# retir/Style-Big-GAN

Hardware: AMD Instinct MI355X
Metric: images/sec (G+D step) StyleGAN2-ADA 256x256 bf16 (higher is better)
Workload: dtype bf16; 1 GPU; configs/sg2ada.yaml @ 256x256: sg2_classic G (skip) + D (orig), softplus + R1(0.01)/4, idle Greg slot /16 (G lr x 16/17), global batch 64 = 1 rank(s) x 2 round(s) x batch_gpu 32 (the rounds of a phase evaluated in one pass, minibatch-std groups and loss those of the separate rounds), bf16 from 8x8 up (num_fp16_res 6; the reference recipe defaults to 4), conv_clamp 256, ADA off; global_batch=64, per_rank_batch=64, parallelism=dp1

## Files before the change

### include/sbg_hip.h

```cpp
#ifndef SBG_HIP_H
#define SBG_HIP_H

#include <stdint.h>

#ifdef __cplusplus
extern "C" {
#endif

typedef void* sbg_stream_t;

enum sbg_status {
    SBG_OK = 0,
    SBG_ERR_INVALID = 1,
    SBG_ERR_UNSUPPORTED = 2,
    SBG_ERR_LAUNCH = 3
};

enum sbg_dtype { SBG_F32 = 0, SBG_F16 = 1, SBG_BF16 = 2 };

enum sbg_act {
    SBG_ACT_LINEAR = 1, SBG_ACT_RELU = 2, SBG_ACT_LRELU = 3, SBG_ACT_TANH = 4, SBG_ACT_SIGMOID = 5,
    SBG_ACT_ELU = 6, SBG_ACT_SELU = 7, SBG_ACT_SOFTPLUS = 8, SBG_ACT_SWISH = 9
};

int         sbg_version(void);
const char* sbg_last_error(void);

int sbg_bias_act(const void* x, const void* b, const void* xref, const void* yref, const void* dy,
                 void* y, int dtype, int grad, int act, float alpha, float gain, float clamp,
                 int64_t sizeX, int sizeB, int64_t stepB, sbg_stream_t stream);

typedef struct sbg_upfirdn2d_params {
    const void*  x;
    const float* f;
    void*        y;
    int dtype;
    int upx, upy, downx, downy, padx0, pady0;
    int flip;
    float gain;
    int     inSize[4];      int64_t inStride[4];
    int     filterSize[2];  int     filterStride[2];
    int     outSize[4];     int64_t outStride[4];
    const float* oscale; const float* noise; int64_t noise_stride_n; const float* bias;
    int act; float alpha, act_gain, clamp;
    int     filter_exact16;
    const void* dact_y; float* dact_partial; int dact_act; float dact_alpha, dact_gain, dact_clamp;
    const float* post_scale;
} sbg_upfirdn2d_params;
int sbg_upfirdn2d_tail_supported(const sbg_upfirdn2d_params* p);
int64_t sbg_upfirdn2d_dact_rows(const sbg_upfirdn2d_params* p);
int sbg_upfirdn2d(const sbg_upfirdn2d_params* p, sbg_stream_t stream);

int sbg_upfirdn2d_separable_supported(int up, int down, int taps);
int sbg_upfirdn2d_separable(const float* x, const float* f, float* y, int M, int IH, int IW, int OH, int OW, int taps,
                            int up, int down, int padx0, int pady0, int flip, float gain, sbg_stream_t stream);

#define SBG_MAX_TAPS 16
typedef struct sbg_conv_params {
    const void* x; const void* w; void* y;
    const float* oscale;
    int xdtype, ydtype;
    int N, IH, IW, Cin, Cout, OH, OW;
    int64_t xs_n, xs_h, xs_w;
    int64_t ys_n, ys_h, ys_w;
    int64_t ws_slab, ws_co;
    int stride;
    int ntaps;
    int tap_dy[SBG_MAX_TAPS], tap_dx[SBG_MAX_TAPS], tap_slab[SBG_MAX_TAPS];
    int accumulate;
    const float* bias; const float* noise; int64_t noise_stride_n;
    int act; float alpha, gain, clamp;
    void* workspace; int ksplit;
    int nphase; int ph_ntaps[4], ph_oh[4], ph_ow[4]; int64_t ph_yoff[4];
} sbg_conv_params;
int64_t sbg_conv2d_igemm_workspace(const sbg_conv_params* p);
int     sbg_conv2d_igemm(const sbg_conv_params* p, sbg_stream_t stream);
typedef struct sbg_conv_launch_info {
    int dims[7]; double flops, bytes;
    int64_t grid_x; int grid_y, block, lds;
} sbg_conv_launch_info;
int     sbg_conv2d_igemm_plan(const sbg_conv_params* p, sbg_conv_launch_info* out, int max);


typedef struct sbg_wgrad_params {
    const void* a; const void* b; float* out; void* workspace;
    int dtype;
    int N, PH, PW, Ca, BH, BW, Cb;
    int64_t as_n, as_h, as_w;
    int64_t bs_n, bs_h, bs_w;
    int stride;
    int ntaps;
    int tap_dy[SBG_MAX_TAPS], tap_dx[SBG_MAX_TAPS];
    int accumulate;
} sbg_wgrad_params;
int64_t sbg_conv2d_wgrad_workspace(const sbg_wgrad_params* p);
int     sbg_conv2d_wgrad(const sbg_wgrad_params* p, sbg_stream_t stream);


int sbg_scale_nc(const void* x, const float* a, const float* z, void* y, int dtype, int layout,
                 int N, int C, int64_t HW, int64_t z_stride_n, sbg_stream_t stream);
int sbg_scale_shift_nc(const void* x, const float* a, const float* b, void* y, int dtype, int layout,
                       int N, int C, int64_t HW, sbg_stream_t stream);

int sbg_dot_hw_splits(int layout, int N, int C, int64_t HW);
int sbg_dot_hw(const void* u, const void* v, float* partial, int dtype, int layout,
               int N, int C, int64_t HW, sbg_stream_t stream);
int sbg_moments_hw(const void* x, float* r, int dtype, int N, int C, int64_t HW, sbg_stream_t stream);

typedef struct sbg_gg_problem {
    const float *a0, *b0, *a1, *b1;
    float* c; const float* bias; float* rowsum;
    int64_t a0_rs, a0_cs, b0_rs, b0_cs, a1_rs, a1_cs, b1_rs, b1_cs, c_rs, c_cs;
    int M, N, K0, K1, nterms;
    float alpha0, alpha1, bias_scale, rowsum_scale;
} sbg_gg_problem;
int sbg_grouped_gemm(const sbg_gg_problem* problems, int count, sbg_stream_t stream);

int sbg_dot_hw_scale_supported(int C);
int sbg_dot_hw_scale(const void* u, const void* v, const float* scale, void* y, float* partial, int dtype,
                     int N, int C, int64_t HW, sbg_stream_t stream);


int sbg_modconv_bwd_supported(int C);
int sbg_modconv_bwd(const void* dy, const void* y, const float* dcoef, const float* noise, const float* bias,
                    void* d2, float* partial, float* dnoise, int dtype, int N, int C, int64_t HW, int64_t noise_stride_n,
                    int act, float alpha, float gain, float clamp, sbg_stream_t stream);
int sbg_modconv_bwd_prescaled(const void* dy, const void* y, const float* prescale, const float* dcoef, const float* noise, const float* bias,
                              void* d2, float* partial, float* partial3, float* dnoise, int dtype, int N, int C, int64_t HW,
                              int64_t noise_stride_n, int act, float alpha, float gain, float clamp, sbg_stream_t stream);

int64_t sbg_sn_workspace(int rows, int cols);
int sbg_sn_power_iteration(const float* W, const float* u, float* v, float* u_new, float* sigma, void* workspace,
                           int rows, int cols, float eps, sbg_stream_t stream);

int64_t sbg_mbstd_workspace(int N, int C, int HW, int G, int F);
int sbg_mbstd_fwd(const float* x, float* y, void* workspace, int N, int C, int HW, int G, int F, sbg_stream_t stream);
int sbg_mbstd_bwd(const float* x, const float* dy, float* dx, int N, int C, int HW, int G, int F, sbg_stream_t stream);

int sbg_split_bf16_cat(const float* x, void* y, int64_t outer, int64_t C, int64_t inner, int nseg, const int* order, sbg_stream_t stream);
int sbg_split_bf16_cat_nd(const float* x, const int64_t* shape, const int64_t* xstrides, int cat_dim, void* y, int nseg, const int* order, sbg_stream_t stream);

int sbg_attention_supported(int Q, int M, int D, int DV);
int sbg_attention_fwd(const float* theta, const float* phi, const float* g, float* out, int N, int Q, int M, int D, int DV,
                      sbg_stream_t stream);
int sbg_attention_bwd_supported(int Q, int M, int D, int DV);
int64_t sbg_attention_bwd_workspace(int N, int Q);
int sbg_attention_bwd(const float* theta, const float* phi, const float* g, const float* dout, float* dtheta, float* dphi, float* dg,
                      void* workspace, int N, int Q, int M, int D, int DV, sbg_stream_t stream);

int sbg_pack_weight(const float* w, void* out, int out_dtype, int A, int B, int KH, int KW,
                    int64_t sA, int64_t sB, int64_t sKH, int64_t sKW, int Bp, float gain, float* w2, sbg_stream_t stream);
int sbg_unpack_wgrad(const float* dwp, int64_t dwp_tap_stride, int64_t dwp_row_stride, float* dw, const float* w, const float* dw2,
                     int A, int B, int KH, int KW, int64_t sA, int64_t sB, int64_t sKH, int64_t sKW, float gain, sbg_stream_t stream);

int sbg_demod_coefs(const float* styles, const float* w2, float* dcoefs, int N, int O, int I, float eps, sbg_stream_t stream);
int sbg_demod_coefs_bwd(const float* g, const float* dcoefs, const float* styles, const float* w2, float* dstyles, float* dw2,
                        int N, int O, int I, sbg_stream_t stream);

// ... 163 lines not shown
```

### style-big-gan_amd/_lib.py

```python
import ctypes
import os
import threading

import torch

_HERE = os.path.dirname(os.path.abspath(__file__))
LIB_PATH = os.environ.get("SBG_HIP_LIBRARY") or os.path.join(_HERE, "libsbg_hip.so")

SBG_F32, SBG_F16, SBG_BF16 = 0, 1, 2
SBG_MAX_TAPS = 16

_DTYPES = {torch.float32: SBG_F32, torch.float16: SBG_F16, torch.bfloat16: SBG_BF16}


def dtype_code(dtype):
    try:
        return _DTYPES[dtype]
    except KeyError:
        raise RuntimeError(f"style_big_gan_amd: unsupported dtype {dtype} (float32 / float16 / bfloat16 only)")


class UpfirdnParams(ctypes.Structure):
    _fields_ = [
        ("x", ctypes.c_void_p), ("f", ctypes.c_void_p), ("y", ctypes.c_void_p),
        ("dtype", ctypes.c_int),
        ("upx", ctypes.c_int), ("upy", ctypes.c_int), ("downx", ctypes.c_int), ("downy", ctypes.c_int),
        ("padx0", ctypes.c_int), ("pady0", ctypes.c_int),
        ("flip", ctypes.c_int), ("gain", ctypes.c_float),
        ("inSize", ctypes.c_int * 4), ("inStride", ctypes.c_int64 * 4),
        ("filterSize", ctypes.c_int * 2), ("filterStride", ctypes.c_int * 2),
        ("outSize", ctypes.c_int * 4), ("outStride", ctypes.c_int64 * 4),
        ("oscale", ctypes.c_void_p), ("noise", ctypes.c_void_p), ("noise_stride_n", ctypes.c_int64), ("bias", ctypes.c_void_p),
        ("act", ctypes.c_int), ("alpha", ctypes.c_float), ("act_gain", ctypes.c_float), ("clamp", ctypes.c_float),
        ("filter_exact16", ctypes.c_int),
        ("dact_y", ctypes.c_void_p), ("dact_partial", ctypes.c_void_p), ("dact_act", ctypes.c_int),
        ("dact_alpha", ctypes.c_float), ("dact_gain", ctypes.c_float), ("dact_clamp", ctypes.c_float),
        ("post_scale", ctypes.c_void_p),
    ]


class ConvParams(ctypes.Structure):
    _fields_ = [
        ("x", ctypes.c_void_p), ("w", ctypes.c_void_p), ("y", ctypes.c_void_p), ("oscale", ctypes.c_void_p),
        ("xdtype", ctypes.c_int), ("ydtype", ctypes.c_int),
        ("N", ctypes.c_int), ("IH", ctypes.c_int), ("IW", ctypes.c_int), ("Cin", ctypes.c_int), ("Cout", ctypes.c_int),
        ("OH", ctypes.c_int), ("OW", ctypes.c_int),
        ("xs_n", ctypes.c_int64), ("xs_h", ctypes.c_int64), ("xs_w", ctypes.c_int64),
        ("ys_n", ctypes.c_int64), ("ys_h", ctypes.c_int64), ("ys_w", ctypes.c_int64),
        ("ws_slab", ctypes.c_int64), ("ws_co", ctypes.c_int64),
        ("stride", ctypes.c_int), ("ntaps", ctypes.c_int),
        ("tap_dy", ctypes.c_int * SBG_MAX_TAPS), ("tap_dx", ctypes.c_int * SBG_MAX_TAPS), ("tap_slab", ctypes.c_int * SBG_MAX_TAPS),
        ("accumulate", ctypes.c_int),
        ("bias", ctypes.c_void_p), ("noise", ctypes.c_void_p), ("noise_stride_n", ctypes.c_int64),
        ("act", ctypes.c_int), ("alpha", ctypes.c_float), ("gain", ctypes.c_float), ("clamp", ctypes.c_float),
        ("workspace", ctypes.c_void_p), ("ksplit", ctypes.c_int),
        ("nphase", ctypes.c_int), ("ph_ntaps", ctypes.c_int * 4), ("ph_oh", ctypes.c_int * 4), ("ph_ow", ctypes.c_int * 4), ("ph_yoff", ctypes.c_int64 * 4),
    ]


class ConvLaunchInfo(ctypes.Structure):
    _fields_ = [("dims", ctypes.c_int * 7), ("flops", ctypes.c_double), ("bytes", ctypes.c_double),
                ("grid_x", ctypes.c_int64), ("grid_y", ctypes.c_int), ("block", ctypes.c_int), ("lds", ctypes.c_int)]


class WgradParams(ctypes.Structure):
    _fields_ = [
        ("a", ctypes.c_void_p), ("b", ctypes.c_void_p), ("out", ctypes.c_void_p), ("workspace", ctypes.c_void_p),
        ("dtype", ctypes.c_int),
        ("N", ctypes.c_int), ("PH", ctypes.c_int), ("PW", ctypes.c_int), ("Ca", ctypes.c_int),
        ("BH", ctypes.c_int), ("BW", ctypes.c_int), ("Cb", ctypes.c_int),
        ("as_n", ctypes.c_int64), ("as_h", ctypes.c_int64), ("as_w", ctypes.c_int64),
        ("bs_n", ctypes.c_int64), ("bs_h", ctypes.c_int64), ("bs_w", ctypes.c_int64),
        ("stride", ctypes.c_int), ("ntaps", ctypes.c_int),
        ("tap_dy", ctypes.c_int * SBG_MAX_TAPS), ("tap_dx", ctypes.c_int * SBG_MAX_TAPS),
        ("accumulate", ctypes.c_int),
    ]


class GridSampleParams(ctypes.Structure):
    _fields_ = [
        ("x", ctypes.c_void_p), ("grid", ctypes.c_void_p), ("theta", ctypes.c_void_p), ("dy", ctypes.c_void_p),
        ("y", ctypes.c_void_p), ("dx", ctypes.c_void_p), ("dgrid", ctypes.c_void_p),
        ("N", ctypes.c_int), ("C", ctypes.c_int), ("IH", ctypes.c_int), ("IW", ctypes.c_int), ("OH", ctypes.c_int), ("OW", ctypes.c_int),
        ("xs_n", ctypes.c_int64), ("xs_c", ctypes.c_int64), ("xs_h", ctypes.c_int64), ("xs_w", ctypes.c_int64),
        ("ys_n", ctypes.c_int64), ("ys_c", ctypes.c_int64), ("ys_h", ctypes.c_int64), ("ys_w", ctypes.c_int64),
        ("theta_host", ctypes.c_void_p),
    ]


class GgProblem(ctypes.Structure):
    _fields_ = [("a0", ctypes.c_void_p), ("b0", ctypes.c_void_p), ("a1", ctypes.c_void_p), ("b1", ctypes.c_void_p),
                ("c", ctypes.c_void_p), ("bias", ctypes.c_void_p), ("rowsum", ctypes.c_void_p),
                ("a0_rs", ctypes.c_int64), ("a0_cs", ctypes.c_int64), ("b0_rs", ctypes.c_int64), ("b0_cs", ctypes.c_int64),
                ("a1_rs", ctypes.c_int64), ("a1_cs", ctypes.c_int64), ("b1_rs", ctypes.c_int64), ("b1_cs", ctypes.c_int64),
                ("c_rs", ctypes.c_int64), ("c_cs", ctypes.c_int64),
                ("M", ctypes.c_int), ("N", ctypes.c_int), ("K0", ctypes.c_int), ("K1", ctypes.c_int), ("nterms", ctypes.c_int),
                ("alpha0", ctypes.c_float), ("alpha1", ctypes.c_float), ("bias_scale", ctypes.c_float), ("rowsum_scale", ctypes.c_float)]


class ProfRecord(ctypes.Structure):
    _fields_ = [("kind", ctypes.c_int), ("dims", ctypes.c_int * 7), ("flops", ctypes.c_double), ("bytes", ctypes.c_double),
                ("ms", ctypes.c_float), ("pad", ctypes.c_int)]


KERNEL_KINDS = {1: "bias_act", 2: "upfirdn2d", 3: "conv_igemm", 4: "conv_wgrad", 5: "wgrad_reduce", 6: "scale_nc", 7: "dot_hw", 9: "sn_power", 10: "attention",
                11: "grid_sample", 12: "filter1d", 13: "color", 14: "weight_prep", 15: "torgb", 16: "fromrgb", 17: "grouped_gemm", 18: "ppl",
                19: "projector", 20: "image_export", 21: "resample", 22: "pr", 23: "grad_finish", 24: "resident", 25: "diffaug", 26: "nn_u8", 27: "swd", 28: "spectrum",
                29: "msssim", 30: "directions", 31: "kmeans_u8", 32: "walk"}
WALK_VARIANTS = {0: "blend", 1: "sqdiff", 2: "merge"}
KMEANS_VARIANTS = {0: "accumulate", 1: "finish"}
DIRECTIONS_VARIANTS = {0: "mean", 1: "gram", 2: "merge", 3: "edit"}
MSSSIM_VARIANTS = {0: "level", 1: "down", 2: "merge"}
SWD_VARIANTS = {0: "pyr_down", 1: "pyr_lap", 2: "gather", 3: "moments", 4: "project", 5: "l1", 6: "merge"}
SPECTRUM_VARIANTS = {0: "rows", 1: "cols"}
NN_VARIANTS = {0: "norms", 1: "single", 2: "split", 3: "merge"}
RESIDENT_PATHS = {1: "dword", 2: "byte"}
PPL_VARIANTS = {0: "slerp", 1: "lerp", 2: "prep", 3: "dist"}
PROJ_VARIANTS = {0: "reg", 1: "reg_bwd", 2: "normalize", 3: "sqdist", 4: "sqdist_bwd"}
IMG_VARIANTS = {0: "quantize_tile", 1: "truncate_mix"}
QUANT_RULES = {"grid": 0, "clamp": 1}
RESAMPLE_VARIANTS = {0: "h", 1: "v"}
PR_VARIANTS = {0: "single", 1: "split", 2: "merge", 3: "norms"}
GRAD_FINISH_VARIANTS = {0: "sweep", 1: "merge"}
DIFFAUG_VARIANTS = {0: "sum", 1: "apply", 2: "adj_sum", 3: "adj_apply", 4: "single", 5: "adj_single"}
DIFFAUG_WORDS = 12
ATT_VARIANTS = {0: "single", 1: "stream", 2: "stream_stats", 3: "stream_dq", 4: "stream_dkv"}

_lib = None
_lock = threading.Lock()

_c = ctypes
SYMBOLS = [
    ("sbg_version", _c.c_int, []),
    ("sbg_last_error", _c.c_char_p, []),
    ("sbg_bias_act", _c.c_int, [_c.c_void_p] * 6 + [_c.c_int, _c.c_int, _c.c_int, _c.c_float, _c.c_float, _c.c_float,
                                                   _c.c_int64, _c.c_int, _c.c_int64, _c.c_void_p]),
    ("sbg_upfirdn2d_tail_supported", _c.c_int, [_c.POINTER(UpfirdnParams)]),
    ("sbg_upfirdn2d", _c.c_int, [_c.POINTER(UpfirdnParams), _c.c_void_p]),
    ("sbg_upfirdn2d_dact_rows", _c.c_int64, [_c.POINTER(UpfirdnParams)]),
    ("sbg_upfirdn2d_separable_supported", _c.c_int, [_c.c_int] * 3),
    ("sbg_upfirdn2d_separable", _c.c_int, [_c.c_void_p] * 3 + [_c.c_int] * 11 + [_c.c_float, _c.c_void_p]),
    ("sbg_conv2d_igemm_workspace", _c.c_int64, [_c.POINTER(ConvParams)]),
    ("sbg_conv2d_igemm", _c.c_int, [_c.POINTER(ConvParams), _c.c_void_p]),
    ("sbg_conv2d_igemm_plan", _c.c_int, [_c.POINTER(ConvParams), _c.POINTER(ConvLaunchInfo), _c.c_int]),
    ("sbg_conv2d_wgrad_workspace", _c.c_int64, [_c.POINTER(WgradParams)]),
    ("sbg_conv2d_wgrad", _c.c_int, [_c.POINTER(WgradParams), _c.c_void_p]),
    ("sbg_scale_nc", _c.c_int, [_c.c_void_p] * 4 + [_c.c_int, _c.c_int, _c.c_int, _c.c_int, _c.c_int64, _c.c_int64, _c.c_void_p]),
    ("sbg_scale_shift_nc", _c.c_int, [_c.c_void_p] * 4 + [_c.c_int, _c.c_int, _c.c_int, _c.c_int, _c.c_int64, _c.c_void_p]),
    ("sbg_sn_workspace", _c.c_int64, [_c.c_int, _c.c_int]),
    ("sbg_sn_power_iteration", _c.c_int, [_c.c_void_p] * 6 + [_c.c_int, _c.c_int, _c.c_float, _c.c_void_p]),
    ("sbg_mbstd_workspace", _c.c_int64, [_c.c_int] * 5),
    ("sbg_mbstd_fwd", _c.c_int, [_c.c_void_p] * 3 + [_c.c_int] * 5 + [_c.c_void_p]),
    ("sbg_mbstd_bwd", _c.c_int, [_c.c_void_p] * 3 + [_c.c_int] * 5 + [_c.c_void_p]),
    ("sbg_split_bf16_cat", _c.c_int, [_c.c_void_p, _c.c_void_p, _c.c_int64, _c.c_int64, _c.c_int64, _c.c_int, _c.POINTER(_c.c_int), _c.c_void_p]),
    ("sbg_split_bf16_cat_nd", _c.c_int, [_c.c_void_p, _c.POINTER(_c.c_int64), _c.POINTER(_c.c_int64), _c.c_int, _c.c_void_p, _c.c_int, _c.POINTER(_c.c_int), _c.c_void_p]),
    ("sbg_attention_supported", _c.c_int, [_c.c_int] * 4),
    ("sbg_attention_fwd", _c.c_int, [_c.c_void_p] * 4 + [_c.c_int] * 5 + [_c.c_void_p]),
    ("sbg_attention_bwd_supported", _c.c_int, [_c.c_int] * 4),
    ("sbg_attention_bwd_workspace", _c.c_int64, [_c.c_int, _c.c_int]),
    ("sbg_attention_bwd", _c.c_int, [_c.c_void_p] * 8 + [_c.c_int] * 5 + [_c.c_void_p]),
    ("sbg_dot_hw_splits", _c.c_int, [_c.c_int, _c.c_int, _c.c_int, _c.c_int64]),
    ("sbg_dot_hw", _c.c_int, [_c.c_void_p] * 3 + [_c.c_int, _c.c_int, _c.c_int, _c.c_int, _c.c_int64, _c.c_void_p]),
    ("sbg_moments_hw", _c.c_int, [_c.c_void_p, _c.c_void_p, _c.c_int, _c.c_int, _c.c_int, _c.c_int64, _c.c_void_p]),
    ("sbg_grouped_gemm", _c.c_int, [_c.c_void_p, _c.c_int, _c.c_void_p]),
    ("sbg_dot_hw_scale_supported", _c.c_int, [_c.c_int]),
    ("sbg_dot_hw_scale", _c.c_int, [_c.c_void_p] * 5 + [_c.c_int, _c.c_int, _c.c_int, _c.c_int64, _c.c_void_p]),
    ("sbg_modconv_bwd_supported", _c.c_int, [_c.c_int]),
    ("sbg_modconv_bwd", _c.c_int, [_c.c_void_p] * 8 + [_c.c_int, _c.c_int, _c.c_int, _c.c_int64, _c.c_int64, _c.c_int, _c.c_float, _c.c_float, _c.c_float, _c.c_void_p]),
    ("sbg_modconv_bwd_prescaled", _c.c_int, [_c.c_void_p] * 10 + [_c.c_int, _c.c_int, _c.c_int, _c.c_int64, _c.c_int64, _c.c_int, _c.c_float, _c.c_float, _c.c_float, _c.c_void_p]),
    ("sbg_pack_weight", _c.c_int, [_c.c_void_p, _c.c_void_p, _c.c_int, _c.c_int, _c.c_int, _c.c_int, _c.c_int] + [_c.c_int64] * 4
     + [_c.c_int, _c.c_float, _c.c_void_p, _c.c_void_p]),
    ("sbg_unpack_wgrad", _c.c_int, [_c.c_void_p, _c.c_int64, _c.c_int64, _c.c_void_p, _c.c_void_p, _c.c_void_p] + [_c.c_int] * 4
     + [_c.c_int64] * 4 + [_c.c_float, _c.c_void_p]),
    ("sbg_demod_coefs", _c.c_int, [_c.c_void_p] * 3 + [_c.c_int] * 3 + [_c.c_float, _c.c_void_p]),
    ("sbg_demod_coefs_bwd", _c.c_int, [_c.c_void_p] * 6 + [_c.c_int] * 3 + [_c.c_void_p]),
    ("sbg_torgb_supported", _c.c_int, [_c.c_int, _c.c_int]),
    ("sbg_torgb_bwd_blocks", _c.c_int, [_c.c_int, _c.c_int, _c.c_int64]),
    ("sbg_torgb_fwd", _c.c_int, [_c.c_void_p] * 4 + [_c.c_int] * 4 + [_c.c_int64, _c.c_float, _c.c_void_p]),
    ("sbg_torgb_bwd", _c.c_int, [_c.c_void_p] * 6 + [_c.c_int] * 4 + [_c.c_int64, _c.c_float, _c.c_void_p]),
    ("sbg_fromrgb_supported", _c.c_int, [_c.c_int] * 3),
    ("sbg_fromrgb_bwd_blocks", _c.c_int, [_c.c_int, _c.c_int64]),
    ("sbg_fromrgb_fwd", _c.c_int, [_c.c_void_p] * 4 + [_c.c_int] * 4 + [_c.c_int64, _c.c_int, _c.c_float, _c.c_float, _c.c_float, _c.c_void_p]),
    ("sbg_fromrgb_bwd", _c.c_int, [_c.c_void_p] * 6 + [_c.c_int] * 4 + [_c.c_int64, _c.c_int, _c.c_float, _c.c_float, _c.c_float, _c.c_void_p]),
    ("sbg_grid_sample2d", _c.c_int, [_c.POINTER(GridSampleParams), _c.c_void_p]),
    ("sbg_grid_sample2d_bwd", _c.c_int, [_c.POINTER(GridSampleParams), _c.c_void_p]),
    ("sbg_grid_sample2d_bwd_overwrites", _c.c_int, [_c.POINTER(GridSampleParams)]),
    ("sbg_color_transform", _c.c_int, [_c.c_void_p] * 3 + [_c.c_int, _c.c_int64, _c.c_void_p]),
    ("sbg_filter1d_batch", _c.c_int, [_c.c_void_p] * 3 + [_c.c_int] * 8 + [_c.c_void_p]),
    ("sbg_ppl_slerp_endpoints", _c.c_int, [_c.c_void_p] * 3 + [_c.c_float, _c.c_void_p, _c.c_int, _c.c_int, _c.c_void_p]),
    ("sbg_ppl_lerp_endpoints", _c.c_int, [_c.c_void_p] * 3 + [_c.c_float, _c.c_void_p, _c.c_int, _c.c_int64, _c.c_void_p]),
    ("sbg_ppl_prep_images", _c.c_int, [_c.c_void_p] * 2 + [_c.c_int] * 4 + [_c.c_int64] * 4 + [_c.c_int, _c.c_int, _c.c_void_p]),
    ("sbg_ppl_dist_workspace", _c.c_int64, [_c.c_int, _c.c_int64]),
    ("sbg_ppl_dist", _c.c_int, [_c.c_void_p] * 3 + [_c.c_int, _c.c_int64, _c.c_float, _c.c_void_p]),
    ("sbg_proj_noise_reg_workspace", _c.c_int64, [_c.c_void_p, _c.c_int]),
    ("sbg_proj_noise_reg", _c.c_int, [_c.c_void_p] * 2 + [_c.c_int] + [_c.c_void_p] * 4),
    ("sbg_proj_noise_reg_bwd", _c.c_int, [_c.c_void_p] * 3 + [_c.c_int] + [_c.c_void_p] * 4),
    ("sbg_proj_noise_normalize_workspace", _c.c_int64, [_c.c_void_p, _c.c_int]),
    ("sbg_proj_noise_normalize", _c.c_int, [_c.c_void_p] * 2 + [_c.c_int] + [_c.c_void_p] * 2),
    ("sbg_proj_sqdist_workspace", _c.c_int64, [_c.c_int64]),
    ("sbg_proj_sqdist", _c.c_int, [_c.c_void_p] * 4 + [_c.c_int64, _c.c_void_p]),
    ("sbg_proj_sqdist_bwd", _c.c_int, [_c.c_void_p] * 4 + [_c.c_int64, _c.c_void_p]),
    ("sbg_img_quantize_tile", _c.c_int, [_c.c_void_p] * 2 + [_c.c_int] * 4 + [_c.c_int64] * 4 + [_c.c_int] * 4 + [_c.c_float] * 2 + [_c.c_void_p]),
    ("sbg_ws_truncate_mix", _c.c_int, [_c.c_void_p] * 2 + [_c.c_float] + [_c.c_void_p] * 4 + [_c.c_int] * 5 + [_c.c_void_p]),
    ("sbg_u8_resample_h", _c.c_int, [_c.c_void_p, _c.c_int64, _c.c_int64] * 2 + [_c.c_int] * 5 + [_c.c_void_p] * 2 + [_c.c_int] * 3 + [_c.c_void_p]),
    ("sbg_u8_resample_v", _c.c_int, [_c.c_void_p, _c.c_int64, _c.c_int64] * 2 + [_c.c_int] * 4 + [_c.c_void_p] * 2 + [_c.c_int, _c.c_void_p]),
    ("sbg_knn_workspace", _c.c_int64, [_c.c_int] * 4),
    ("sbg_knn_kth_radius", _c.c_int, [_c.c_void_p] * 2 + [_c.c_int, _c.c_int, _c.c_int64, _c.c_int] + [_c.c_void_p] * 3),
    ("sbg_knn_in_manifold", _c.c_int, [_c.c_void_p] * 3 + [_c.c_int, _c.c_int, _c.c_int64] + [_c.c_void_p] * 3),
    ("sbg_knn_probe_workspace", _c.c_int64, [_c.c_int] * 2),
    ("sbg_knn_probe", _c.c_int, [_c.c_void_p] * 3 + [_c.c_int, _c.c_int, _c.c_int64] + [_c.c_void_p] * 4),
    ("sbg_knn_topk_workspace", _c.c_int64, [_c.c_int] * 3),
    ("sbg_knn_topk", _c.c_int, [_c.c_void_p] * 2 + [_c.c_int, _c.c_int, _c.c_int64, _c.c_int] + [_c.c_void_p] * 5),
    ("sbg_knn_realism_workspace", _c.c_int64, [_c.c_int] * 2),
    ("sbg_knn_realism", _c.c_int, [_c.c_void_p] * 3 + [_c.c_int, _c.c_int, _c.c_int64] + [_c.c_void_p] * 5),
    ("sbg_grad_finish_records", _c.c_int64, [_c.c_int64]),
    ("sbg_grad_finish_sweep", _c.c_int, [_c.c_void_p, _c.c_int64, _c.c_float, _c.c_void_p, _c.c_void_p]),
    ("sbg_grad_finish_merge", _c.c_int, [_c.c_void_p, _c.c_int64, _c.c_void_p, _c.c_void_p]),
    ("sbg_u8_gather_images", _c.c_int, [_c.c_void_p, _c.c_int64, _c.c_int, _c.c_int, _c.c_int, _c.c_void_p, _c.c_void_p, _c.c_int, _c.c_void_p, _c.c_int,
                                        _c.c_void_p, _c.c_void_p]),
    ("sbg_u8_nn_workspace", _c.c_int64, [_c.c_int] * 3),
    ("sbg_u8_nn_topk", _c.c_int, [_c.c_void_p] * 2 + [_c.c_int, _c.c_int, _c.c_int64, _c.c_int] + [_c.c_void_p] * 5),
    ("sbg_diffaug_workspace", _c.c_int64, [_c.c_int] * 4),
    ("sbg_diffaug_fwd", _c.c_int, [_c.c_void_p] * 4 + [_c.c_int] * 5 + [_c.c_void_p]),
    ("sbg_diffaug_adj", _c.c_int, [_c.c_void_p] * 4 + [_c.c_int] * 4 + [_c.c_void_p]),
    ("sbg_swd_pyr_down", _c.c_int, [_c.c_void_p] * 2 + [_c.c_int] * 3 + [_c.c_void_p]),
# ... 98 lines not shown
```

### style-big-gan_amd/csrc/conv_common.h

```cpp
#pragma once
#include "sbg_common.h"
#include <cstdlib>

#define SBG_OOB_OFFSET 0x80000000u

namespace sbgconv {

typedef __attribute__((address_space(3))) void* lds_void_ptr;

struct bf16_mfma { static constexpr int dtype = SBG_BF16; };
struct f16_mfma  { static constexpr int dtype = SBG_F16;  };

template <class MF> struct Mfma;
template <> struct Mfma<bf16_mfma> {
    static __device__ __forceinline__ float4_t run(short8_t a, short8_t b, float4_t c) {
        return __builtin_amdgcn_mfma_f32_16x16x32_bf16(__builtin_bit_cast(bf16x8_t, a), __builtin_bit_cast(bf16x8_t, b), c, 0, 0, 0);
    }
    static __device__ __forceinline__ unsigned short cvt(float v) { return f32_to_bf16_bits(v); }
};
template <> struct Mfma<f16_mfma> {
    static __device__ __forceinline__ float4_t run(short8_t a, short8_t b, float4_t c) {
        return __builtin_amdgcn_mfma_f32_16x16x32_f16(__builtin_bit_cast(f16x8_t, a), __builtin_bit_cast(f16x8_t, b), c, 0, 0, 0);
    }
    static __device__ __forceinline__ unsigned short cvt(float v) { return f32_to_f16_bits(v); }
};

struct ConvArgs {
    const unsigned short* x; const unsigned short* w; void* y; const float* oscale;
    const float* bias; const float* noise; int64_t noise_sn; int act; float alpha, gain, clamp;
    int ydtype;
    int N, IH, IW, Cin, Cout, OH, OW;
    int64_t xs_n, xs_h, xs_w, ys_n, ys_h, ys_w, ws_slab, ws_co;
    int stride, ntaps;
    int tap_dy[SBG_MAX_TAPS], tap_dx[SBG_MAX_TAPS], tap_slab[SBG_MAX_TAPS];
    int accumulate;
    int P;
    int ptiles, ctiles;
    int nphase, ph_rot_div;
    int ph_tap0[4], ph_ntaps[4], ph_OH[4], ph_OW[4], ph_P[4];
    int64_t ph_yoff[4];
    int ksplit;
    int64_t y_split_stride;
    int lds_params;
};

#define SBG_CONV_IS_PLAIN(a) (((a).act <= SBG_ACT_LINEAR) && (a).gain == 1.f && (a).clamp < 0.f && !(a).bias && !(a).noise && !(a).oscale)
static __host__ __device__ __forceinline__ bool conv_is_plain(const ConvArgs& a) { return SBG_CONV_IS_PLAIN(a); }
static inline bool conv_is_plain(const sbg_conv_params& q)
{
    return (q.act == 0 || q.act == SBG_ACT_LINEAR) && (q.gain == 1.f || q.gain == 0.f) && q.clamp < 0.f && !q.bias && !q.noise && !q.oscale;
}

template <auto Kern, class... Args>
static int launch_as(int kind, const char* who, int64_t nblk, unsigned grid_y, unsigned block, int lds, hipStream_t stream, double flops,
                     double bytes, std::initializer_list<int> dims, const Args&... args)
{
    if (nblk > INT32_MAX || nblk < 1) return sbg_fail(SBG_ERR_INVALID, "%s: grid too large", who);
    if (lds > 64 * 1024 && !SBG_RAISE_LDS_ONCE(Kern, lds))
        return sbg_fail(SBG_ERR_LAUNCH, "%s: cannot raise the dynamic LDS limit to %d bytes", who, lds);
    SbgProfScope prof(stream, kind, flops, bytes, dims);
    SBG_LAUNCH(Kern, dim3((unsigned)nblk, grid_y), dim3(block), lds, stream, args...);
    SBG_HIP_LAUNCH_CHECK();
    return SBG_OK;
}

enum ConvFamily { CONV_THIN, CONV_UP2, CONV_GATHER, CONV_HALO, CONV_K64, CONV_GENERIC };
struct ConvLaunch {
    ConvFamily family;
    int bc, bp;
    int64_t grid_x; unsigned grid_y, block; int lds;
    ConvArgs a;
    unsigned x_bytes, w_bytes;
    int pitch;
    int tiles_y, tiles_x, dymin, dxmin;
    double flops, bytes; int dims[7];
};
struct ConvPlan {
    int nlaunch; ConvLaunch launch[5];
    ConvArgs call;
    int ksplit; bool reduce_epi;
    int64_t workspace_bytes;
};

static inline void conv_prof(ConvLaunch& l, double macs, double outpix, int ntaps, int stride, int rows, int code)
{
    const ConvArgs& a = l.a;
    const double ys = a.ydtype == SBG_F32 ? 4.0 : 2.0;
    l.flops = 2.0 * macs * a.Cout * (double)a.Cin;
    l.bytes = 2.0 * a.N * a.IH * a.IW * (double)a.Cin + 2.0 * ntaps * a.Cout * (double)a.Cin + ys * outpix * (double)a.Cout * (a.accumulate ? 2 : 1);
    const int dims[7] = {(int)outpix, a.Cout, a.Cin, ntaps, stride, rows, code};
    for (int i = 0; i < 7; i++) l.dims[i] = dims[i];
}
static inline void conv_prof_phases(ConvLaunch& l, int code)
{
    const ConvArgs& a = l.a;
    double macs = (double)a.P * a.ntaps, outpix = a.P;
    if (a.nphase > 1) {
        macs = outpix = 0.0;
        for (int i = 0; i < a.nphase; i++) { macs += (double)a.ph_P[i] * a.ph_ntaps[i]; outpix += a.ph_P[i]; }
    }
    conv_prof(l, macs, outpix, a.ntaps, a.stride, a.OH, code);
}

template <auto Kern, class... Extra>
static int conv_launch(const ConvLaunch& l, hipStream_t stream, const Extra&... extra)
{
    const int* d = l.dims;
    return launch_as<Kern>(SBG_K_CONV_IGEMM, "conv2d_igemm", l.grid_x, l.grid_y, l.block, l.lds, stream, l.flops, l.bytes,
                           {d[0], d[1], d[2], d[3], d[4], d[5], d[6]}, l.a, extra...);
}

}

bool sbg_conv_thin_fit(sbgconv::ConvLaunch& l);
int  sbg_conv_thin_launch(const sbgconv::ConvLaunch& l, bool bf16, hipStream_t stream);
enum Up2Fit { UP2_OTHER_FORM, UP2_ORDERED, UP2_FITS };
Up2Fit sbg_conv_up2_fit(sbgconv::ConvLaunch& l, const sbg_conv_params& q, sbg_conv_params& border);
int    sbg_conv_up2_launch(const sbgconv::ConvLaunch& l, bool bf16, hipStream_t stream);
void sbg_conv_k64_fit(sbgconv::ConvLaunch& l);
int  sbg_conv_k64_launch(const sbgconv::ConvLaunch& l, bool bf16, hipStream_t stream);
int  sbg_conv_ksplit_reduce(const sbgconv::ConvArgs& call, const void* workspace, int ksplit, bool reduce_epi, hipStream_t stream);
```

### style-big-gan_amd/csrc/conv_device.h

```cpp
#pragma once
#include "conv_common.h"
#include "lds_asm.h"

namespace sbgconv {

static __device__ __forceinline__ int chmap(int R) { return (R & ~31) + 8 * ((R & 15) >> 2) + 4 * ((R >> 4) & 1) + (R & 3); }

template <int N> static __device__ __forceinline__ void wait_vmcnt_const() { asm volatile("s_waitcnt vmcnt(%0)" :: "n"(N) : "memory"); }

static __device__ __forceinline__ int xcd_tile_order(int bid, int nwg)
{
    const int q = nwg >> 3, r = nwg & 7, xcd = bid & 7, k = bid >> 3;
    return (xcd < r ? xcd * (q + 1) : r * (q + 1) + (xcd - r) * q) + k;
}

static __device__ __forceinline__ int dma_lrow(int lane)  { return lane >> 3; }
static __device__ __forceinline__ int dma_src_k(int lane, int lrow) { return ((lane & 7) ^ lrow) * 8; }

static __device__ __forceinline__ int frag_off(int fr, int fg) { return fr * 128 + ((fg ^ (fr & 7)) << 4); }

template <class MF, int TC, int TP>
static __device__ __forceinline__ void mma_step(float4_t (&acc)[TC][TP], const short8_t (&fa)[2][TC], const short8_t (&fb)[2][TP])
{
#pragma unroll
    for (int ks = 0; ks < 2; ks++)
#pragma unroll
        for (int i = 0; i < TC; i++)
#pragma unroll
            for (int j = 0; j < TP; j++) acc[i][j] = Mfma<MF>::run(fa[ks][i], fb[ks][j], acc[i][j]);
}

static __device__ __forceinline__ float tail(const ConvArgs& p, float u, int64_t si, float add)
{
    if (p.oscale) u *= p.oscale[si];
    u += add;
    if (p.act == SBG_ACT_LRELU) u = (u > 0.f) ? u : u * p.alpha;
    else if (p.act == SBG_ACT_RELU) u = (u > 0.f) ? u : 0.f;
    u *= p.gain;
    if (p.clamp >= 0.f) u = (u > -p.clamp && u < p.clamp) ? u : (u >= 0.f ? p.clamp : -p.clamp);
    return u;
}

typedef __attribute__((address_space(3))) const float lds_cfloat;
typedef __attribute__((address_space(3))) const float4_t lds_cfloat4;
struct LdsParams { lds_cfloat* base; int c; int tw; };
template <int TC, int TP, int YDT, bool PLAIN, bool NUNI, bool LP = false, class PixFn>
static __device__ __forceinline__ void conv_epilogue_fast(const ConvArgs& p, float4_t (&acc)[TC][TP], int cbase, int fg, PixFn pix, int64_t ybase,
                                                          const LdsParams* lp = nullptr, int y0 = 0, int x0 = 0)
{
    constexpr int TH2 = TC / 2;
    const float alpha = (p.act == SBG_ACT_LRELU) ? p.alpha : (p.act == SBG_ACT_RELU ? 0.f : 1.f);
    const float lsel = alpha <= 1.f ? __builtin_inff() : -__builtin_inff();
    const float cl = p.clamp >= 0.f ? p.clamp : __builtin_inff();
    const float gain = p.gain;
    const float* const dummy = reinterpret_cast<const float*>(p.x);
    const bool has_nz = !PLAIN && p.noise != nullptr, has_b = !PLAIN && p.bias != nullptr, has_s = !PLAIN && p.oscale != nullptr;
    int64_t yoff[TP]; float nz[TP]; bool ok[TP]; int nn[TP];
#pragma unroll
    for (int j = 0; j < TP; j++) {
        int n, oy, ox;
        ok[j] = pix(j, n, oy, ox);
        nn[j] = n;
        yoff[j] = ybase + (int64_t)blockIdx.y * p.y_split_stride + (int64_t)n * p.ys_n + (int64_t)oy * p.ys_h + (int64_t)ox * p.ys_w + cbase + 8 * fg;
        nz[j] = 0.f;
        if (!PLAIN) {
            if constexpr (LP) nz[j] = lp->base[(oy - y0) * lp->tw + (ox - x0)];
            else              nz[j] = *(has_nz ? p.noise + ((int64_t)n * p.noise_sn + (int64_t)oy * p.OW + ox) : dummy);
        }
    }
    float4_t b_lo[TH2], b_hi[TH2], s_lo[TH2], s_hi[TH2];
#pragma unroll
    for (int h = 0; h < TH2; h++) {
        b_lo[h] = b_hi[h] = float4_t{0.f, 0.f, 0.f, 0.f};
        s_lo[h] = s_hi[h] = float4_t{1.f, 1.f, 1.f, 1.f};
        if (!PLAIN) {
            if constexpr (LP) {
                lds_cfloat* b = lp->base + 256 + lp->c + 32 * h + 8 * fg;
                b_lo[h] = *(lds_cfloat4*)b; b_hi[h] = *(lds_cfloat4*)(b + 4);
                if (NUNI) { s_lo[h] = *(lds_cfloat4*)(b + 256); s_hi[h] = *(lds_cfloat4*)(b + 260); }
            } else {
            const float* b = has_b ? p.bias + cbase + 32 * h + 8 * fg : dummy;
            b_lo[h] = *reinterpret_cast<const float4_t*>(b); b_hi[h] = *reinterpret_cast<const float4_t*>(has_b ? b + 4 : dummy);
            if (NUNI) {
                const float* sc = has_s ? p.oscale + (int64_t)nn[0] * p.Cout + cbase + 32 * h + 8 * fg : dummy;
                s_lo[h] = *reinterpret_cast<const float4_t*>(sc); s_hi[h] = *reinterpret_cast<const float4_t*>(has_s ? sc + 4 : dummy);
            }
            }
        }
    }
    if (!PLAIN) {
#pragma unroll
        for (int j = 0; j < TP; j++) nz[j] = has_nz ? nz[j] : 0.f;
#pragma unroll
        for (int h = 0; h < TH2; h++) {
            if (!has_b) { b_lo[h] = float4_t{0.f, 0.f, 0.f, 0.f}; b_hi[h] = b_lo[h]; }
            if (!NUNI || !has_s) { s_lo[h] = float4_t{1.f, 1.f, 1.f, 1.f}; s_hi[h] = s_lo[h]; }
        }
    }
#pragma unroll
    for (int h = 0; h < TH2; h++) {
#pragma unroll
        for (int j = 0; j < TP; j++) {
            if (!ok[j]) continue;
            float4_t lo = acc[2 * h][j], hi = acc[2 * h + 1][j];
            if (!PLAIN) {
                float4_t sl = s_lo[h], sh = s_hi[h];
                if (!NUNI && has_s) {
                    const float* sc = p.oscale + (int64_t)nn[j] * p.Cout + cbase + 32 * h + 8 * fg;
                    sl = *reinterpret_cast<const float4_t*>(sc); sh = *reinterpret_cast<const float4_t*>(sc + 4);
                }
                lo = lo * sl + (nz[j] + b_lo[h]);
                hi = hi * sh + (nz[j] + b_hi[h]);
                const float4_t tl = lo * alpha, th = hi * alpha;
#pragma unroll
                for (int e = 0; e < 4; e++) { lo[e] = __builtin_amdgcn_fmed3f(lo[e], tl[e], lsel); hi[e] = __builtin_amdgcn_fmed3f(hi[e], th[e], lsel); }
                lo = lo * gain; hi = hi * gain;
#pragma unroll
                for (int e = 0; e < 4; e++) { lo[e] = __builtin_amdgcn_fmed3f(lo[e], -cl, cl); hi[e] = __builtin_amdgcn_fmed3f(hi[e], -cl, cl); }
            }
            if (YDT == SBG_F32) {
                float* dst = (float*)p.y + yoff[j] + 32 * h;
                if (p.accumulate) { lo += *reinterpret_cast<float4_t*>(dst); hi += *reinterpret_cast<float4_t*>(dst + 4); }
                *reinterpret_cast<float4_t*>(dst) = lo;
                *reinterpret_cast<float4_t*>(dst + 4) = hi;
            } else {
                short8_t o;
#pragma unroll
                for (int e = 0; e < 4; e++) { o[e] = (short)f32_to_bf16_bits(lo[e]); o[4 + e] = (short)f32_to_bf16_bits(hi[e]); }
                *reinterpret_cast<short8_t*>((unsigned short*)p.y + yoff[j] + 32 * h) = o;
            }
        }
    }
}


template <int TC, int TP, bool NUNI = false, class PixFn>
static __device__ __forceinline__ void conv_epilogue8(const ConvArgs& p, float4_t (&acc)[TC][TP], int cbase, int fg, PixFn pix, int64_t ybase = 0,
                                                      const LdsParams* lp = nullptr, int y0 = 0, int x0 = 0)
{
    constexpr int TH2 = TC / 2;
    const bool plain = conv_is_plain(p);
    const bool fast = (cbase + 16 * TC <= p.Cout) && ((p.Cout & 7) == 0) && ((((uintptr_t)p.y) & 15) == 0) && (((p.ys_n | p.ys_h | p.ys_w) & 7) == 0)
                      && ((((uintptr_t)p.oscale) & 15) == 0) && ((((uintptr_t)p.bias) & 15) == 0) && p.ydtype != SBG_F16;
    if (fast) {
        if (p.ydtype == SBG_BF16) {
            if (plain) conv_epilogue_fast<TC, TP, SBG_BF16, true, NUNI>(p, acc, cbase, fg, pix, ybase);
            else if (lp) conv_epilogue_fast<TC, TP, SBG_BF16, false, NUNI, true>(p, acc, cbase, fg, pix, ybase, lp, y0, x0);
            else       conv_epilogue_fast<TC, TP, SBG_BF16, false, NUNI>(p, acc, cbase, fg, pix, ybase);
        } else {
            if (plain) conv_epilogue_fast<TC, TP, SBG_F32, true, NUNI>(p, acc, cbase, fg, pix, ybase);
            else if (lp) conv_epilogue_fast<TC, TP, SBG_F32, false, NUNI, true>(p, acc, cbase, fg, pix, ybase, lp, y0, x0);
            else       conv_epilogue_fast<TC, TP, SBG_F32, false, NUNI>(p, acc, cbase, fg, pix, ybase);
        }
        return;
    }
    float bias8[TH2][8];
#pragma unroll
    for (int h = 0; h < TH2; h++) {
        const int co = cbase + 32 * h + 8 * fg;
#pragma unroll
        for (int e = 0; e < 8; e++) bias8[h][e] = (p.bias && co + e < p.Cout) ? p.bias[co + e] : 0.f;
    }
#pragma unroll
    for (int j = 0; j < TP; j++) {
        int n, oy, ox;
        if (!pix(j, n, oy, ox)) continue;
        const int64_t yoff = ybase + (int64_t)blockIdx.y * p.y_split_stride + (int64_t)n * p.ys_n + (int64_t)oy * p.ys_h + (int64_t)ox * p.ys_w;
        const float nz = (!plain && p.noise) ? p.noise[(int64_t)n * p.noise_sn + (int64_t)oy * p.OW + ox] : 0.f;
#pragma unroll
        for (int h = 0; h < TH2; h++) {
            const int co = cbase + 32 * h + 8 * fg;
            if (co >= p.Cout) continue;
            float v[8];
#pragma unroll
            for (int e = 0; e < 4; e++) { v[e] = acc[2 * h][j][e]; v[4 + e] = acc[2 * h + 1][j][e]; }
#pragma unroll 1
            for (int e = 0; e < 8; e++) {
                if (co + e >= p.Cout) break;
                float u = v[e];
                if (!plain) {
                    if (p.oscale) u *= p.oscale[(int64_t)n * p.Cout + co + e];
                    u += nz + bias8[h][e];
                    if (p.act == SBG_ACT_LRELU) u = (u > 0.f) ? u : u * p.alpha;
                    else if (p.act == SBG_ACT_RELU) u = (u > 0.f) ? u : 0.f;
                    u *= p.gain;
                    if (p.clamp >= 0.f) u = (u > -p.clamp && u < p.clamp) ? u : (u >= 0.f ? p.clamp : -p.clamp);
                }
                if (p.ydtype == SBG_F32) {
                    float* dst = (float*)p.y + yoff + co + e;
                    *dst = p.accumulate ? *dst + u : u;
                } else {
                    ((unsigned short*)p.y)[yoff + co + e] = (p.ydtype == SBG_BF16) ? f32_to_bf16_bits(u) : f32_to_f16_bits(u);
                }
            }
        }
    }
}

}
```

### style-big-gan_amd/csrc/conv_igemm.hip

```cpp
#include "conv_device.h"

using namespace sbgconv;

namespace {

static __device__ __forceinline__ int stage_row16(int lane) { return (lane & 7) | ((lane >> 5) << 3); }
static __device__ __forceinline__ int stage_kgrp(int lane)  { return (lane >> 3) & 3; }

template <int TC, int TP>
static __device__ __forceinline__ void conv_epilogue(const ConvArgs& p, float4_t (&acc)[TC][TP], int c0, int p0, int wc, int wp, int fr, int fg)
{
    float4_t bias4[TC];
    bool full4[TC];
#pragma unroll
    for (int i = 0; i < TC; i++) {
        const int co = c0 + wc + 16 * i + 4 * fg;
        full4[i] = (co + 4 <= p.Cout);
        bias4[i] = float4_t{0.f, 0.f, 0.f, 0.f};
        if (p.bias) {
#pragma unroll
            for (int e = 0; e < 4; e++) if (co + e < p.Cout) bias4[i][e] = p.bias[co + e];
        }
    }
    const bool plain = conv_is_plain(p);
// ... 125 lines not shown
        if (s + 1 < nsteps) issue_loads(s + 1);
        const unsigned char* sa = smem + buf * STAGE;
        const unsigned char* sb = sa + A_BYTES;
        short8_t fa[TC], fb[TP];
#pragma unroll
        for (int i = 0; i < TC; i++) fa[i] = *reinterpret_cast<const short8_t*>(sa + (fg * BC + wc + 16 * i + fr) * 16);
#pragma unroll
        for (int j = 0; j < TP; j++) fb[j] = *reinterpret_cast<const short8_t*>(sb + (fg * BP + wp + 16 * j + fr) * 16);
#pragma unroll
        for (int i = 0; i < TC; i++)
#pragma unroll
            for (int j = 0; j < TP; j++) acc[i][j] = Mfma<MF>::run(fa[i], fb[j], acc[i][j]);
        if (s + 1 < nsteps) write_stage(buf ^ 1);
        __syncthreads();
    }

    conv_epilogue<TC, TP>(p, acc, c0, p0, wc, wp, fr, fg);
}

template <class MF>
static int launch_generic(const ConvLaunch& l, hipStream_t stream)
{
    if (l.bc == 64) return conv_launch<conv_igemm_kernel<MF, 64, 256, 1, 4>>(l, stream);
    return conv_launch<conv_igemm_kernel<MF, 128, 128, 2, 2>>(l, stream);
}

static void fit_generic(ConvLaunch& l)
{
    ConvArgs& a = l.a;
    l.family = CONV_GENERIC; l.bc = a.Cout <= 64 ? 64 : 128; l.bp = a.Cout <= 64 ? 256 : 128;
    a.ptiles = (a.P + l.bp - 1) / l.bp;
    a.ctiles = (a.Cout + l.bc - 1) / l.bc;
    l.grid_x = (int64_t)a.ptiles * a.ctiles; l.grid_y = 1; l.block = 256; l.lds = 2 * (4 * l.bc * 16 + 4 * l.bp * 16);
    conv_prof_phases(l, l.bc * 1000 + l.bp);
}

constexpr int kPhaseMinTiles = 16;

int conv_validate(const sbg_conv_params* q)
{
    SBG_CHECK(q && q->x && q->w && q->y, "conv2d_igemm: null pointer");
    SBG_CHECK(q->xdtype == SBG_BF16 || q->xdtype == SBG_F16, "conv2d_igemm: x/w must be bf16 or f16 (fp32 inputs are split by the host)");
    SBG_CHECK(q->ydtype == SBG_F32 || q->ydtype == SBG_BF16 || q->ydtype == SBG_F16, "conv2d_igemm: bad output dtype");
    SBG_CHECK(q->N >= 0 && q->IH >= 1 && q->IW >= 1 && q->OH >= 1 && q->OW >= 1 && q->Cin >= 8 && q->Cout >= 1, "conv2d_igemm: bad sizes");
    SBG_CHECK((q->Cin % 8) == 0, "conv2d_igemm: Cin must be a multiple of 8 (pad on the host)");
    SBG_CHECK(q->ntaps >= 1 && q->ntaps <= SBG_MAX_TAPS, "conv2d_igemm: 1..%d taps", SBG_MAX_TAPS);
    SBG_CHECK(q->stride >= 1, "conv2d_igemm: stride must be >= 1");
    SBG_CHECK(!q->accumulate || q->ydtype == SBG_F32, "conv2d_igemm: accumulate needs an fp32 output");
    SBG_CHECK(q->ksplit >= 0, "conv2d_igemm: ksplit must be 0 (the library chooses), 1 (never) or a cap");
    SBG_CHECK(q->act == 0 || q->act == SBG_ACT_LINEAR || q->act == SBG_ACT_RELU || q->act == SBG_ACT_LRELU, "conv2d_igemm: fused activation must be linear, relu or lrelu");
    SBG_CHECK(sbg_aligned16(q->x) && sbg_aligned16(q->w), "conv2d_igemm: x and w must be 16-byte aligned");
    SBG_CHECK((q->xs_n % 8) == 0 && (q->xs_h % 8) == 0 && (q->xs_w % 8) == 0 && (q->ws_slab % 8) == 0 && (q->ws_co % 8) == 0,
              "conv2d_igemm: pixel / row strides must be multiples of 8 elements");
    const int64_t P = (int64_t)q->N * q->OH * q->OW;
    SBG_CHECK(P <= INT32_MAX, "conv2d_igemm: too many output pixels");
    if (P == 0) return SBG_OK;
    for (int t = 0; t < q->ntaps; t++) SBG_CHECK(q->tap_slab[t] >= 0, "conv2d_igemm: negative weight slab");
    if (q->nphase > 1) {
        SBG_CHECK(q->nphase <= 4, "conv2d_igemm: at most 4 phases");
        SBG_CHECK(conv_is_plain(*q) && (q->ksplit <= 1), "conv2d_igemm: phases exclude the fused epilogue and the K split");
        int t0 = 0;
        for (int i = 0; i < q->nphase; i++) {
            SBG_CHECK(q->ph_ntaps[i] >= 1 && q->ph_oh[i] >= 1 && q->ph_ow[i] >= 1, "conv2d_igemm: bad phase %d", i);
            t0 += q->ph_ntaps[i];
        }
        SBG_CHECK(t0 <= q->ntaps, "conv2d_igemm: phases use %d taps, %d given", t0, q->ntaps);
    }
    return SBG_OK;
}

void conv_fill(const sbg_conv_params& q, ConvArgs& a)
{
    a.x = (const unsigned short*)q.x; a.w = (const unsigned short*)q.w; a.y = q.y; a.oscale = q.oscale;
    a.bias = q.bias; a.noise = q.noise; a.noise_sn = q.noise_stride_n;
    a.act = q.act; a.alpha = q.alpha; a.gain = (q.act == 0 && q.gain == 0.f) ? 1.f : q.gain; a.clamp = (q.act == 0 && q.clamp == 0.f && q.gain == 0.f) ? -1.f : q.clamp;
    a.ydtype = q.ydtype;
    a.N = q.N; a.IH = q.IH; a.IW = q.IW; a.Cin = q.Cin; a.Cout = q.Cout; a.OH = q.OH; a.OW = q.OW;
    a.xs_n = q.xs_n; a.xs_h = q.xs_h; a.xs_w = q.xs_w; a.ys_n = q.ys_n; a.ys_h = q.ys_h; a.ys_w = q.ys_w;
    a.ws_slab = q.ws_slab; a.ws_co = q.ws_co;
    a.stride = q.stride; a.ntaps = q.ntaps;
    for (int t = 0; t < SBG_MAX_TAPS; t++) { a.tap_dy[t] = q.tap_dy[t]; a.tap_dx[t] = q.tap_dx[t]; a.tap_slab[t] = q.tap_slab[t]; }
    a.accumulate = q.accumulate;
    a.P = q.N * q.OH * q.OW; a.ptiles = a.ctiles = 0; a.lds_params = 0; a.ksplit = 1; a.y_split_stride = 0;
    a.nphase = q.nphase > 1 ? q.nphase : 1; a.ph_rot_div = 1;
    for (int i = 0, t0 = 0; i < 4; i++) {
        const bool on = q.nphase > 1 && i < q.nphase;
        a.ph_tap0[i] = on ? t0 : 0; a.ph_ntaps[i] = on ? q.ph_ntaps[i] : 0; a.ph_OH[i] = on ? q.ph_oh[i] : 0; a.ph_OW[i] = on ? q.ph_ow[i] : 0;
        a.ph_P[i] = on ? q.N * q.ph_oh[i] * q.ph_ow[i] : 0; a.ph_yoff[i] = on ? q.ph_yoff[i] : 0;
        if (on) t0 += q.ph_ntaps[i];
    }
}

int conv_ksplit(const sbg_conv_params& q, const ConvArgs& a, bool have_ws, bool& reduce_epi)
{
    const bool dense_y = a.ys_w == a.Cout && a.ys_h == (int64_t)a.OW * a.Cout && a.ys_n == (int64_t)a.OH * a.OW * a.Cout;
    const bool simple = a.ydtype == SBG_F32 && conv_is_plain(a);
    const bool epi_ok = !a.accumulate && (a.Cout & 7) == 0 && sbg_aligned16(a.y);
    reduce_epi = !simple;
    if (!have_ws || q.ksplit == 1 || a.Cout <= 64 || !dense_y || !(simple || epi_ok)) return 1;
    const int64_t tiles = (int64_t)((a.P + 127) / 128) * ((a.Cout + 127) / 128);
    const int ksteps = a.ntaps * ((a.Cin + 63) >> 6);
    if (tiles >= 128 || ksteps < 16) return 1;
    int k = (int)((256 + tiles - 1) / tiles);
    if (k > ksteps / 4) k = ksteps / 4;
    if (q.ksplit > 1 && k > q.ksplit) k = q.ksplit;
    return k < 2 ? 1 : k;
}

int push(ConvPlan& pl, const ConvLaunch& l)
{
    if (pl.nlaunch >= 5) return sbg_fail(SBG_ERR_INVALID, "conv2d_igemm: more than five launches");
    pl.launch[pl.nlaunch++] = l;
    return SBG_OK;
}

int conv_plan_add(const sbg_conv_params& q, bool have_ws, ConvPlan& pl)
{
    if ((int64_t)q.N * q.OH * q.OW == 0) return SBG_OK;
    ConvLaunch l = {};
    ConvArgs& a = l.a;
    conv_fill(q, a);
    if (pl.nlaunch == 0) pl.call = a;
    int maxslab = 0;
    for (int t = 0; t < q.ntaps; t++) if (q.tap_slab[t] > maxslab) maxslab = q.tap_slab[t];
    const int64_t x_bytes = 2 * ((int64_t)(q.N - 1) * q.xs_n + (int64_t)(q.IH - 1) * q.xs_h + (int64_t)(q.IW - 1) * q.xs_w + q.Cin);
    const int64_t w_bytes = 2 * ((int64_t)maxslab * q.ws_slab + (int64_t)(q.Cout - 1) * q.ws_co + q.Cin);
    const bool fwd_strides = q.xs_n >= 0 && q.xs_h >= 0 && q.xs_w >= 0 && q.ws_slab >= 0 && q.ws_co >= 0;
    const bool dma = fwd_strides && x_bytes < (int64_t)SBG_OOB_OFFSET && w_bytes < (int64_t)SBG_OOB_OFFSET;
    l.x_bytes = (unsigned)x_bytes; l.w_bytes = (unsigned)w_bytes;
    if (q.nphase > 1) {
        if (fwd_strides && sbg_conv_thin_fit(l)) return push(pl, l);
        if (dma && q.nphase == 4) {
            sbg_conv_params border;
            if (sbg_conv_up2_fit(l, q, border) == UP2_FITS) {
                const int rc = push(pl, l);
                return rc != SBG_OK || border.nphase == 0 ? rc : conv_plan_add(border, false, pl);
            }
        }
        int64_t ptot = 0;
        for (int i = 0; i < q.nphase; i++) ptot += a.ph_P[i];
        const int64_t tiles = ((ptot / q.nphase + 255) / 256) * q.nphase * ((q.Cout + 127) / 128);
        if (dma && q.Cout > 64 && tiles >= kPhaseMinTiles) { sbg_conv_k64_fit(l); return push(pl, l); }
        for (int i = 0; i < q.nphase; i++) {
            sbg_conv_params one = q;
            one.nphase = 0; one.ksplit = 1; one.OH = q.ph_oh[i]; one.OW = q.ph_ow[i]; one.ntaps = q.ph_ntaps[i];
            one.y = (char*)q.y + q.ph_yoff[i] * (q.ydtype == SBG_F32 ? 4 : 2);
            for (int t = 0; t < one.ntaps; t++) { one.tap_dy[t] = q.tap_dy[a.ph_tap0[i] + t]; one.tap_dx[t] = q.tap_dx[a.ph_tap0[i] + t]; one.tap_slab[t] = q.tap_slab[a.ph_tap0[i] + t]; }
            const int rc = conv_plan_add(one, false, pl);
            if (rc != SBG_OK) return rc;
        }
        return SBG_OK;
    }
    if (q.ksplit <= 1 && fwd_strides && sbg_conv_thin_fit(l)) return push(pl, l);
    if (!dma) { fit_generic(l); return push(pl, l); }
    const int k = conv_ksplit(q, a, have_ws, pl.reduce_epi);
    if (k > 1) {
        pl.ksplit = k; pl.workspace_bytes = (int64_t)k * a.P * a.Cout * (int64_t)sizeof(float);
        a.y = q.workspace; a.accumulate = 0; a.ksplit = k; a.y_split_stride = (int64_t)a.P * a.Cout;
        a.ydtype = SBG_F32; a.act = SBG_ACT_LINEAR; a.gain = 1.f; a.clamp = -1.f; a.bias = nullptr; a.noise = nullptr; a.oscale = nullptr;
    }
    sbg_conv_k64_fit(l);
    return push(pl, l);
}

int conv_plan(const sbg_conv_params* q, bool have_ws, ConvPlan& pl)
{
    const int rc = conv_validate(q);
    if (rc != SBG_OK) return rc;
    pl.nlaunch = 0; pl.ksplit = 1; pl.reduce_epi = false; pl.workspace_bytes = 0;
    return conv_plan_add(*q, have_ws, pl);
}

}

extern "C" int64_t sbg_conv2d_igemm_workspace(const sbg_conv_params* q)
{
    ConvPlan pl;
    return conv_plan(q, true, pl) == SBG_OK ? pl.workspace_bytes : -1;
}

extern "C" int sbg_conv2d_igemm_plan(const sbg_conv_params* q, sbg_conv_launch_info* out, int max)
{
    ConvPlan pl;
    if (conv_plan(q, q && q->workspace, pl) != SBG_OK) return -1;
    for (int i = 0; i < pl.nlaunch && i < max && out; i++) {
        const ConvLaunch& l = pl.launch[i];
        for (int d = 0; d < 7; d++) out[i].dims[d] = l.dims[d];
        out[i].flops = l.flops; out[i].bytes = l.bytes;
        out[i].grid_x = l.grid_x; out[i].grid_y = (int)l.grid_y; out[i].block = (int)l.block; out[i].lds = l.lds;
    }
    return pl.nlaunch;
}

extern "C" int sbg_conv2d_igemm(const sbg_conv_params* q, sbg_stream_t stream)
{
    ConvPlan pl;
    int rc = conv_plan(q, q && q->workspace, pl);
    if (rc != SBG_OK) return rc;
    SBG_CHECK(q->ksplit <= 1 || q->workspace != nullptr, "conv2d_igemm: ksplit > 1 needs a workspace");
    hipStream_t s = (hipStream_t)stream;
    const bool bf16 = q->xdtype == SBG_BF16;
    for (int i = 0; i < pl.nlaunch && rc == SBG_OK; i++) {
        const ConvLaunch& l = pl.launch[i];
        switch (l.family) {
        case CONV_THIN:    rc = sbg_conv_thin_launch(l, bf16, s); break;
        case CONV_UP2:     rc = sbg_conv_up2_launch(l, bf16, s); break;
        case CONV_GENERIC: rc = bf16 ? launch_generic<bf16_mfma>(l, s) : launch_generic<f16_mfma>(l, s); break;
        default:           rc = sbg_conv_k64_launch(l, bf16, s); break;
        }
    }
    return rc != SBG_OK || pl.ksplit == 1 ? rc : sbg_conv_ksplit_reduce(pl.call, q->workspace, pl.ksplit, pl.reduce_epi, s);
}
```

### style-big-gan_amd/csrc/conv_k64.hip

```cpp
#include "conv_device.h"
#include <type_traits>

using namespace sbgconv;

namespace {


template <class MF, int BC, int BP, int WGC, int WGP, int NSTAGE = 3>
__global__ __launch_bounds__(512, 2) void conv_k64_kernel(ConvArgs p, unsigned x_bytes, unsigned w_bytes)
{
    constexpr int NW = 8;
    static_assert(WGC * WGP == NW, "8 waves per workgroup");
    constexpr int WC = BC / WGC, WP = BP / WGP;
    constexpr int TC = WC / 16,  TP = WP / 16;
    static_assert(WC % 32 == 0 && WP % 16 == 0 && BC % 64 == 0 && BP % 64 == 0, "tile shape");
    constexpr int IA = BC / 64;
    constexpr int IB = BP / 64;
    constexpr int LEAD = NSTAGE - 1;
    static_assert(NSTAGE == 2 || NSTAGE == 3, "gather pipeline: one or two steps of loads in flight");
    constexpr int A_BYTES = BC * 128, B_BYTES = BP * 128, STAGE = A_BYTES + B_BYTES;

    extern __shared__ __attribute__((aligned(16))) unsigned char smem[];

    const int tid = threadIdx.x, lane = tid & 63;
    const int wave = __builtin_amdgcn_readfirstlane(tid >> 6);
    const bool grpY = wave >= 4;
    const int bid = xcd_tile_order(blockIdx.x, gridDim.x);
    const int c0 = (bid % p.ctiles) * BC, p0 = (bid / p.ctiles) * BP;

    __amdgpu_buffer_rsrc_t xr = __builtin_amdgcn_make_buffer_rsrc((void*)p.x, 0, (int)x_bytes, 0x00020000);
    __amdgpu_buffer_rsrc_t wr = __builtin_amdgcn_make_buffer_rsrc((void*)p.w, 0, (int)w_bytes, 0x00020000);

    const int lrow = dma_lrow(lane);
    const int src_k = dma_src_k(lane, lrow);
    unsigned a_base[IA];
#pragma unroll
    for (int i = 0; i < IA; i++) {
        const int co = c0 + chmap((wave * IA + i) * 8 + lrow);
        a_base[i] = (co < p.Cout) ? (unsigned)(co * (int)p.ws_co + src_k) * 2u : SBG_OOB_OFFSET;
    }
    const int kchunks = (p.Cin + 63) >> 6;
    const int nsteps_all = p.ntaps * kchunks;
    int nsteps = nsteps_all;
    const int tl = lane < p.ntaps ? lane : 0;
    const int tbl_dy = p.tap_dy[tl], tbl_dx = p.tap_dx[tl];
    const int tbl_wtap = p.tap_slab[tl] * (int)p.ws_slab * 2;

    auto issue_w = [&](int t, int chunk, int stage) {
        unsigned char* st = smem + stage * STAGE;
        const int wtap = __builtin_amdgcn_readlane(tbl_wtap, t) + chunk * 128;
        const bool ragged = chunk * 64 + 64 > p.Cin;
#pragma unroll
        for (int i = 0; i < IA; i++) {
            unsigned off = a_base[i];
            if (ragged) off = (chunk * 64 + src_k < p.Cin) ? off : SBG_OOB_OFFSET;
            __builtin_amdgcn_raw_ptr_buffer_load_lds(wr, (lds_void_ptr)(st + (wave * IA + i) * 1024), 16, off, wtap, 0, 0);
        }
    };

    const int wci = wave / WGP, wpi = wave % WGP;
    const int wc = wci * WC, wp = wpi * WP;
    const int fr = lane & 15, fg = lane >> 4;
    const int foff = frag_off(fr, fg);
    float4_t acc[TC][TP];
#pragma unroll
    for (int i = 0; i < TC; i++)
#pragma unroll
        for (int j = 0; j < TP; j++) acc[i][j] = float4_t{0.f, 0.f, 0.f, 0.f};
    short8_t fa[2][TC], fb[2][TP];

    auto read_a = [&](int stage) {
        const unsigned char* sa = smem + stage * STAGE + wc * 128;
#pragma unroll
        for (int ks = 0; ks < 2; ks++)
#pragma unroll
            for (int i = 0; i < TC; i++) fa[ks][i] = *reinterpret_cast<const short8_t*>(sa + i * 16 * 128 + (foff ^ (ks * 64)));
    };
    auto mma = [&]() {
#pragma unroll
        for (int ks = 0; ks < 2; ks++)
#pragma unroll
            for (int i = 0; i < TC; i++)
#pragma unroll
                for (int j = 0; j < TP; j++) acc[i][j] = Mfma<MF>::run(fa[ks][i], fb[ks][j], acc[i][j]);
    };


    {
        int b_iy0[IB], b_ix0[IB]; unsigned b_base[IB];
#pragma unroll
        for (int i = 0; i < IB; i++) {
// ... 92 lines not shown
                    x_off[i] = ok ? b_org[i] + shift : SBG_OOB_OFFSET;
                }
            }
        };
        auto issue_piece = [&](auto k_tag, int t, int chunk, int stg) {
            constexpr int k = decltype(k_tag)::value;
            unsigned char* st = smem + stg * STAGE;
            const bool ragged = chunk * 64 + 64 > p.Cin;
            if constexpr (k < IA) {
                const int wtap = __builtin_amdgcn_readlane(tbl_wtap, t) + chunk * 128 + (16 * (k & 1) + 4 * (k >> 1)) * (int)p.ws_co * 2;
                unsigned off = a_base[0];
                if (ragged) off = (chunk * 64 + src_k < p.Cin) ? off : SBG_OOB_OFFSET;
                __builtin_amdgcn_raw_ptr_buffer_load_lds(wr, (lds_void_ptr)(st + (wave * IA + k) * 1024), 16, off, wtap, 0, 0);
            } else {
                constexpr int i = k - IA;
                unsigned off = x_off[i];
                if (ragged) off = (chunk * 64 + src_k < p.Cin) ? off : SBG_OOB_OFFSET;
                __builtin_amdgcn_raw_ptr_buffer_load_lds(xr, (lds_void_ptr)(st + A_BYTES + (wave * IB + i) * 1024), 16, off, chunk * 128, 0, 0);
            }
        };
        auto issue_advance = [&]() {
            wstage ^= 1;
            if (++ic == kchunks) { ic = 0; it++; }
        };
        auto issue_all = [&]() {
            tap_prep(it);
            sbg_static_for<C>([&](auto k_tag) { issue_piece(k_tag, it, ic, wstage); });
            issue_advance();
        };
        constexpr int NG = 2 * TC, GPP = NG / C;
        static_assert(NG % C == 0, "pieces spread evenly over the MFMA groups");
        auto mma_issue = [&]() {
            tap_prep(it);
            sbg_static_for<NG>([&](auto q_tag) {
                constexpr int q = decltype(q_tag)::value, ks = q / TC, i = q % TC;
#pragma unroll
                for (int j = 0; j < TP; j++) acc[i][j] = Mfma<MF>::run(fa[ks][i], fb[ks][j], acc[i][j]);
                if constexpr ((q + 1) % GPP == 0) {
                    __builtin_amdgcn_sched_barrier(0);
                    issue_piece(std::integral_constant<int, (q + 1) / GPP - 1>{}, it, ic, wstage);
                    __builtin_amdgcn_sched_barrier(0);
                }
            });
            issue_advance();
        };
        if (nsteps > 0) issue_all();
        int stage = 0;
        if (!grpY) {
            for (int s = 0; s < nsteps; s++) {
                wait_vmcnt_const<0>();
                __builtin_amdgcn_s_barrier();
                read_a(stage); read_b(stage);
                if (s + 1 < nsteps) issue_all();
                __builtin_amdgcn_s_waitcnt(0xC07F);
                __builtin_amdgcn_s_barrier();
                __builtin_amdgcn_sched_barrier(0);
                mma();
                __builtin_amdgcn_sched_barrier(0);
                stage ^= 1;
            }
            __builtin_amdgcn_s_barrier();
        } else {
            if (nsteps > 1) { issue_all(); wait_vmcnt_const<C>(); } else wait_vmcnt_const<0>();
            __builtin_amdgcn_s_barrier();
            auto y_step = [&](auto more_tag) {
                constexpr bool more = decltype(more_tag)::value;
                __builtin_amdgcn_s_barrier();
                read_a(stage); read_b(stage);
                wait_vmcnt_const<0>();
                __builtin_amdgcn_s_waitcnt(0xC07F);
                __builtin_amdgcn_s_barrier();
                __builtin_amdgcn_sched_barrier(0);
                if constexpr (more) mma_issue(); else mma();
                __builtin_amdgcn_sched_barrier(0);
                stage ^= 1;
            };
            int s = 0;
            for (; s + 2 < nsteps; s++) y_step(std::true_type{});
            for (; s < nsteps; s++) y_step(std::false_type{});
        }
        }
    }

    conv_epilogue8<TC, TP>(p, acc, c0 + wc, fg, [&](int j, int& n, int& oy, int& ox) {
        const int pix = p0 + wp + 16 * j + fr;
        const int pp = pix < p.P ? pix : 0;
        ox = pp % p.OW; const int t = pp / p.OW; oy = t % p.OH; n = t / p.OH;
        return pix < p.P;
    });
}

template <class MF, int TH, int TW>
__global__ __launch_bounds__(768, 3) void conv_halo_ld_kernel(ConvArgs p, unsigned x_bytes, unsigned w_bytes)
{
    constexpr int BC = 128, BP = 256, WGP = 4;
    constexpr int WC = 64, WP = 64, TC = 4, TP = 4;
    static_assert(TH * TW == BP, "halo tile = TH x TW pixels");
    constexpr int NSTAGE = 4, STAGE = BC * 128;
    constexpr int PW = TW + 2, PH = TH + 2, NPIX = PW * PH;
    constexpr int HPIECES = (NPIX + 7) / 8, HALO_BYTES = HPIECES * 1024;
    constexpr int NT = 9, SEG = TW / 16;
    constexpr int WPIECES = BC / 8 / 2;
    constexpr int HPL = (HPIECES + 1) / 2;

    extern __shared__ __attribute__((aligned(16))) unsigned char smem[];
    unsigned char* const sH = smem + NSTAGE * STAGE;
    unsigned char* const sP = sH + 2 * HALO_BYTES;
    constexpr int PARAM_BYTES = 3072;

    const int tid = threadIdx.x, lane = tid & 63;
    const int wave = __builtin_amdgcn_readfirstlane(tid >> 6);
    const int bid = xcd_tile_order(blockIdx.x, gridDim.x);
    const int tiles_x = p.OW / TW, tiles_y = p.OH / TH;
    const int ntiles = p.ptiles * p.ctiles, G = gridDim.x;
    const int my_tiles = (ntiles - bid + G - 1) / G;
    const int kchunks = (p.Cin + 63) >> 6;
    const int nslices = my_tiles * kchunks;
    struct TileC { int c0, tn, y0, x0; };
    auto decode = [&](int tile) -> TileC {
        TileC r;
        const int ct_ = tile % p.ctiles; int pt_ = tile / p.ctiles;
        const int tx = pt_ % tiles_x; pt_ /= tiles_x;
        const int ty = pt_ % tiles_y;
        r.c0 = ct_ * BC; r.tn = pt_ / tiles_y; r.y0 = ty * TH; r.x0 = tx * TW;
        return r;
    };
    const TileC gstep = decode(G);
    auto advance = [&](TileC t_) -> TileC {
        t_.c0 += gstep.c0; int carry = t_.c0 >= p.ctiles * BC; t_.c0 -= carry ? p.ctiles * BC : 0;
        t_.x0 += gstep.x0 + (carry ? TW : 0); carry = t_.x0 >= tiles_x * TW; t_.x0 -= carry ? tiles_x * TW : 0;
        t_.y0 += gstep.y0 + (carry ? TH : 0); carry = t_.y0 >= tiles_y * TH; t_.y0 -= carry ? tiles_y * TH : 0;
        t_.tn += gstep.tn + carry;
        return t_;
    };
    const int lrow = dma_lrow(lane);
    const int src_k = dma_src_k(lane, lrow);

    if (wave >= 10) {
        const int lh = wave - 10;
        __amdgpu_buffer_rsrc_t xr = __builtin_amdgcn_make_buffer_rsrc((void*)p.x, 0, (int)x_bytes, 0x00020000);
        auto issue_params = [&](int t_, int buf) {
            const TileC pc = decode(t_);
            unsigned char* dst = sP + buf * PARAM_BYTES;
            if (p.noise) {
                __amdgpu_buffer_rsrc_t nr = __builtin_amdgcn_make_buffer_rsrc((void*)p.noise, 0, 0x7fffffff, 0x00020000);
                constexpr int LPR = TW / 4;
                const int r = lane / LPR, cx = (lane - r * LPR) * 4;
                const unsigned off = (unsigned)(pc.tn * (int)p.noise_sn + (pc.y0 + r) * p.OW + pc.x0 + cx) * 4u;
                __builtin_amdgcn_raw_ptr_buffer_load_lds(nr, (lds_void_ptr)dst, 16, off, 0, 0, 0);
            }
            const int co = pc.c0 + 4 * lane;
            const unsigned okm = 0u - (unsigned)((lane < 32) & (co < p.Cout));
            if (p.bias) {
                __amdgpu_buffer_rsrc_t br_ = __builtin_amdgcn_make_buffer_rsrc((void*)p.bias, 0, 0x7fffffff, 0x00020000);
                __builtin_amdgcn_raw_ptr_buffer_load_lds(br_, (lds_void_ptr)(dst + 1024), 16, (((unsigned)co * 4u) & okm) | (SBG_OOB_OFFSET & ~okm), 0, 0, 0);
            }
            if (p.oscale) {
                __amdgpu_buffer_rsrc_t sr = __builtin_amdgcn_make_buffer_rsrc((void*)p.oscale, 0, 0x7fffffff, 0x00020000);
                __builtin_amdgcn_raw_ptr_buffer_load_lds(sr, (lds_void_ptr)(dst + 2048), 16, (((unsigned)(pc.tn * p.Cout + co) * 4u) & okm) | (SBG_OOB_OFFSET & ~okm), 0, 0, 0);
            }
        };
        int rel[HPL]; unsigned ef[(HPL + 5) / 6];
#pragma unroll
        for (int w_ = 0; w_ < (HPL + 5) / 6; w_++) ef[w_] = 0;
#pragma unroll
        for (int i = 0; i < HPL; i++) {
            const int piece = lh * HPL + i, pp = piece * 8 + lrow;
            const int py = pp / PW, px = pp - py * PW;
            rel[i] = (py * (int)p.xs_h + px * (int)p.xs_w + src_k) * 2;
            const unsigned f = (unsigned)(py == 0) | ((unsigned)(py == PH - 1) << 1) | ((unsigned)(px == 0) << 2) | ((unsigned)(px == PW - 1) << 3)
                             | ((unsigned)((piece >= HPIECES) | (pp >= NPIX)) << 4);
            ef[i / 6] |= f << (5 * (i % 6));
        }
        auto issue_halo = [&](auto i_tag, int hbase, unsigned emask, bool kok, int buf) {
            constexpr int i = decltype(i_tag)::value;
// ... 52 lines not shown
                const int co = c0_ + chmap((lw * WPIECES + i) * 8 + lrow);
                a_base[i] = (co < p.Cout) ? (unsigned)(co * (int)p.ws_co + src_k) * 2u : SBG_OOB_OFFSET;
            }
        };
        int it = 0, ichunk = 0, itile = bid, istage = 0;
        weight_rows(decode(itile).c0);
        unsigned char* st = nullptr; unsigned kokm = 0, wtap = 0;
        auto issue_prep = [&]() {
            st = smem + istage * STAGE + lw * WPIECES * 1024;
            kokm = 0u - (unsigned)(ichunk * 64 + src_k < p.Cin);
            wtap = (unsigned)(__builtin_amdgcn_readlane(tbl_wtap, it) + ichunk * 128);
        };
        const bool whole_k = (p.Cin & 63) == 0;
        auto issue_part = [&](int lo, int hi) {
            if (whole_k) {
#pragma unroll
                for (int i = 0; i < WPIECES; i++)
                    if (i >= lo && i < hi) __builtin_amdgcn_raw_ptr_buffer_load_lds(wr, (lds_void_ptr)(st + i * 1024), 16, a_base[i], wtap, 0, 0);
                return;
            }
#pragma unroll
            for (int i = 0; i < WPIECES; i++) {
                if (i < lo || i >= hi) continue;
                const unsigned okm = kokm & (0u - (unsigned)(a_base[i] != SBG_OOB_OFFSET));
                const unsigned off = ((a_base[i] + wtap) & okm) | (SBG_OOB_OFFSET & ~okm);
                __builtin_amdgcn_raw_ptr_buffer_load_lds(wr, (lds_void_ptr)(st + i * 1024), 16, off, 0, 0, 0);
            }
        };
        auto issue_done = [&]() {
            istage = (istage + 1) & (NSTAGE - 1);
            if (++it == NT) {
                it = 0;
                if (++ichunk == kchunks) { ichunk = 0; itile += G; if (itile < ntiles) weight_rows(decode(itile).c0); }
            }
        };
        auto issue_next = [&]() { issue_prep(); issue_part(0, WPIECES); issue_done(); };
        constexpr bool split = false;
        const int S = nslices * NT;
        int issued = 0;
        for (; issued < 4 && issued < S; issued++) issue_next();
        for (int s = 0; s < S; s++) {
            const int newer = issued - 1 - s;
            if (newer >= 3) wait_vmcnt_const<3 * WPIECES>();
            else if (newer == 2) wait_vmcnt_const<2 * WPIECES>();
            else if (newer == 1) wait_vmcnt_const<1 * WPIECES>();
            else wait_vmcnt_const<0>();
            __builtin_amdgcn_s_barrier();
            const bool go = s >= 1 && issued < S;
            if (go) { issue_prep(); issue_part(0, split ? WPIECES / 2 : WPIECES); }
            __builtin_amdgcn_s_barrier();
            if (go) { if (split) issue_part(WPIECES / 2, WPIECES); issue_done(); issued++; }
            else if (s >= 1 && issued < S) issued++;
        }
        __builtin_amdgcn_s_barrier();
        return;
    }

    const bool grpY = wave >= 4;
    const int wci = wave >> 2, wpi = wave & 3;
    const int wc = wci * WC;
    const int fr = lane & 15, fg = lane >> 4;
    const int foff = frag_off(fr, fg);
    const int tl = lane < p.ntaps ? lane : 0;
    const int tbl_shift = p.tap_dy[tl] * PW + p.tap_dx[tl];
    float4_t acc[TC][TP];
#pragma unroll
    for (int i = 0; i < TC; i++)
#pragma unroll
        for (int j = 0; j < TP; j++) acc[i][j] = float4_t{0.f, 0.f, 0.f, 0.f};
    short8_t fa[2][TC], fb[2][TP];
    int seg_pp[TP];
#pragma unroll
    for (int j = 0; j < TP; j++) {
        const int sg = wpi * TP + j, r = sg / SEG, cseg = (sg - r * SEG) * 16;
        seg_pp[j] = (r + 1) * PW + cseg + fr + 1;
    }
    int stage = 0, par = 0, chunk = 0, tile = bid;
    TileC cur = decode(tile);
    bool pend = false;
    TileC done = cur;
    int tpar = 0, done_par = 0;
    auto epilogue = [&](const TileC& tc) __attribute__((always_inline)) {
        const LdsParams lp{(lds_cfloat*)(sP + done_par * PARAM_BYTES), wc, TW};
        conv_epilogue8<TC, TP, true>(p, acc, tc.c0 + wc, fg, [&](int j, int& n, int& oy, int& ox) {
            const int sg = wpi * TP + j, r = sg / SEG, cseg = (sg - r * SEG) * 16;
            n = tc.tn; oy = tc.y0 + r; ox = tc.x0 + cseg + fr;
            return true;
        }, 0, p.lds_params ? &lp : nullptr, tc.y0, tc.x0);
#pragma unroll
        for (int i = 0; i < TC; i++)
#pragma unroll
            for (int j = 0; j < TP; j++) acc[i][j] = float4_t{0.f, 0.f, 0.f, 0.f};
    };
    if (grpY) __builtin_amdgcn_s_barrier();
    for (int c = 0; c < nslices; c++) {
        const unsigned char* hb = sH + par * HALO_BYTES;
        sbg_static_for<NT>([&](auto tap_tag) {
            constexpr int t = decltype(tap_tag)::value;
            const int shift = __builtin_amdgcn_readlane(tbl_shift, t);
            const unsigned char* sa = smem + stage * STAGE + wc * 128;
            __builtin_amdgcn_s_barrier();
            if (t == 0 && pend) { epilogue(done); pend = false; }
#pragma unroll
            for (int ks = 0; ks < 2; ks++)
#pragma unroll
                for (int i = 0; i < TC; i++) fa[ks][i] = *reinterpret_cast<const short8_t*>(sa + i * 16 * 128 + (foff ^ (ks * 64)));
#pragma unroll
            for (int j = 0; j < TP; j++) {
                const int pp = seg_pp[j] + shift;
                const int o = pp * 128 + ((fg ^ (pp & 7)) << 4);
#pragma unroll
                for (int ks = 0; ks < 2; ks++) fb[ks][j] = *reinterpret_cast<const short8_t*>(hb + (o ^ (ks * 64)));
            }
            __builtin_amdgcn_s_waitcnt(0xC07F);
            __builtin_amdgcn_s_barrier();
            __builtin_amdgcn_sched_barrier(0);
            mma_step<MF>(acc, fa, fb);
            __builtin_amdgcn_sched_barrier(0);
            stage = (stage + 1) & (NSTAGE - 1);
        });
        par ^= 1;
        if (++chunk < kchunks) continue;
        done = cur; done_par = tpar; tpar ^= 1;
        if (grpY && p.lds_params) epilogue(done); else pend = true;
        chunk = 0; tile += G;
        if (tile < ntiles) cur = advance(cur);
    }
    if (pend) epilogue(done);
    if (!grpY) __builtin_amdgcn_s_barrier();
}

template <class MF>
__global__ __launch_bounds__(768, 3) void conv_gather_ld_kernel(ConvArgs p, unsigned x_bytes, unsigned w_bytes)
{
    constexpr int BC = 128, BP = 256, WGP = 4;
    constexpr int WC = 64, WP = 64, TC = 4, TP = 4;
    constexpr int NSTAGE = 3, A_BYTES = BC * 128, B_BYTES = BP * 128, STAGE = A_BYTES + B_BYTES;
    constexpr int WPIECES = BC / 8 / 2;
    constexpr int XPIECES = BP / 8 / 2;

    extern __shared__ __attribute__((aligned(16))) unsigned char smem[];
    const int tid = threadIdx.x, lane = tid & 63;
    const int wave = __builtin_amdgcn_readfirstlane(tid >> 6);
    const int bid = xcd_tile_order(blockIdx.x, gridDim.x);
    const int ntiles = p.ptiles * p.ctiles, G = gridDim.x;
    const int my_tiles = (ntiles - bid + G - 1) / G;
    const int kchunks = (p.Cin + 63) >> 6;
    auto tile_phase = [&](int tile) { const int r = tile / p.ctiles; return (r % p.nphase + (r / p.nphase) / p.ph_rot_div) % p.nphase; };
    int S = 0;
    for (int t_ = bid; t_ < ntiles; t_ += G) S += p.ph_ntaps[tile_phase(t_)] * kchunks;
    const int lrow = dma_lrow(lane);
    const int src_k = dma_src_k(lane, lrow);
    const int tl = lane < p.ntaps ? lane : 0;

    if (wave >= 8) {
        const bool xload = wave >= 10;
        const int lw = (wave - 8) & 1;
        __amdgpu_buffer_rsrc_t xr = __builtin_amdgcn_make_buffer_rsrc((void*)p.x, 0, (int)x_bytes, 0x00020000);
        __amdgpu_buffer_rsrc_t wr = __builtin_amdgcn_make_buffer_rsrc((void*)p.w, 0, (int)w_bytes, 0x00020000);
        const int tbl_dy = p.tap_dy[tl], tbl_dx = p.tap_dx[tl];
        const int tbl_wtap = p.tap_slab[tl] * (int)p.ws_slab * 2;
        unsigned a_base[WPIECES];
        int b_iy0[XPIECES], b_ix0[XPIECES]; unsigned b_base[XPIECES];
        int ph_t0 = 0, ph_nt = 1;
        auto tile_state = [&](int tile) {
            const int ph = tile_phase(tile);
            const int c0 = (tile % p.ctiles) * BC, p0 = (tile / p.ctiles / p.nphase) * BP;
            const int OW_ = p.ph_OW[ph], OH_ = p.ph_OH[ph], P_ = p.ph_P[ph];
            ph_t0 = p.ph_tap0[ph]; ph_nt = p.ph_ntaps[ph];
            if (!xload) {
#pragma unroll
// ... 54 lines not shown
        int issued = 0;
        for (; issued < NSTAGE && issued < S; issued++) issue_next();
        for (int s = 0; s < S; s++) {
            const int newer = issued - 1 - s;
            if (xload) {
                if (newer >= 2) wait_vmcnt_const<2 * XPIECES>(); else if (newer == 1) wait_vmcnt_const<XPIECES>(); else wait_vmcnt_const<0>();
            } else {
                if (newer >= 2) wait_vmcnt_const<2 * WPIECES>(); else if (newer == 1) wait_vmcnt_const<WPIECES>(); else wait_vmcnt_const<0>();
            }
            __builtin_amdgcn_s_barrier();
            const bool go = s >= 1 && issued < S;
            if (go) issue_part(split ? 0 : -1);
            __builtin_amdgcn_s_barrier();
            if (go) { if (split) issue_part(1); issue_done(); issued++; }
        }
        __builtin_amdgcn_s_barrier();
        return;
    }

    const bool grpY = wave >= 4;
    const int wci = wave >> 2, wpi = wave & 3;
    const int wc = wci * WC, wp = wpi * WP;
    const int fr = lane & 15, fg = lane >> 4;
    const int foff = frag_off(fr, fg);
    float4_t acc[TC][TP];
#pragma unroll
    for (int i = 0; i < TC; i++)
#pragma unroll
        for (int j = 0; j < TP; j++) acc[i][j] = float4_t{0.f, 0.f, 0.f, 0.f};
    short8_t fa[2][TC], fb[2][TP];
    int stage = 0, tile = bid, left = p.ph_ntaps[tile_phase(bid)] * kchunks;
    bool pend = false;
    int done_tile = tile;
    auto epilogue = [&](int t_) __attribute__((always_inline)) {
        const int ph = tile_phase(t_);
        const int c0 = (t_ % p.ctiles) * BC, p0 = (t_ / p.ctiles / p.nphase) * BP;
        const int OW_ = p.ph_OW[ph], OH_ = p.ph_OH[ph], P_ = p.ph_P[ph];
        conv_epilogue8<TC, TP>(p, acc, c0 + wc, fg, [&](int j, int& n, int& oy, int& ox) {
            const int pix = p0 + wp + 16 * j + fr;
            const int pp = pix < P_ ? pix : 0;
            ox = pp % OW_; const int t = pp / OW_; oy = t % OH_; n = t / OH_;
            return pix < P_;
        }, p.ph_yoff[ph]);
#pragma unroll
        for (int i = 0; i < TC; i++)
#pragma unroll
            for (int j = 0; j < TP; j++) acc[i][j] = float4_t{0.f, 0.f, 0.f, 0.f};
    };
    if (grpY) __builtin_amdgcn_s_barrier();
    for (int s = 0; s < S; s++) {
        const unsigned char* sa = smem + stage * STAGE + wc * 128;
        const unsigned char* sb = smem + stage * STAGE + A_BYTES + wp * 128;
        __builtin_amdgcn_s_barrier();
        if (pend) { epilogue(done_tile); pend = false; }
#pragma unroll
        for (int ks = 0; ks < 2; ks++)
#pragma unroll
            for (int i = 0; i < TC; i++) fa[ks][i] = *reinterpret_cast<const short8_t*>(sa + i * 16 * 128 + (foff ^ (ks * 64)));
#pragma unroll
        for (int ks = 0; ks < 2; ks++)
#pragma unroll
            for (int j = 0; j < TP; j++) fb[ks][j] = *reinterpret_cast<const short8_t*>(sb + j * 16 * 128 + (foff ^ (ks * 64)));
        __builtin_amdgcn_s_waitcnt(0xC07F);
        __builtin_amdgcn_s_barrier();
        __builtin_amdgcn_sched_barrier(0);
        mma_step<MF>(acc, fa, fb);
        __builtin_amdgcn_sched_barrier(0);
        stage = stage == NSTAGE - 1 ? 0 : stage + 1;
        if (--left == 0) { pend = true; done_tile = tile; tile += G; if (tile < ntiles) left = p.ph_ntaps[tile_phase(tile)] * kchunks; }
    }
    if (pend) epilogue(done_tile);
    if (!grpY) __builtin_amdgcn_s_barrier();
}

constexpr int kGatherLds = 3 * (128 * 128 + 256 * 128);
constexpr int halo_lds(int TH, int TW) { return 4 * 128 * 128 + 2 * (((TH + 2) * (TW + 2) + 7) / 8) * 1024 + 2 * 3072; }
constexpr int k64_lds(int BC, int BP, int NSTAGE) { return NSTAGE * (BC * 128 + BP * 128); }
static_assert(kGatherLds <= 160 * 1024 && halo_lds(8, 32) <= 160 * 1024 && halo_lds(16, 16) <= 160 * 1024 && k64_lds(256, 256, 2) <= 160 * 1024
              && k64_lds(128, 256, 3) <= 160 * 1024, "LDS budget");

template <class MF>
static int launch_leaf(const ConvLaunch& l, hipStream_t stream)
{
    if (l.family == CONV_GATHER) return conv_launch<conv_gather_ld_kernel<MF>>(l, stream, l.x_bytes, l.w_bytes);
    if (l.family == CONV_HALO)
        return l.bc == 8 ? conv_launch<conv_halo_ld_kernel<MF, 8, 32>>(l, stream, l.x_bytes, l.w_bytes)
                         : conv_launch<conv_halo_ld_kernel<MF, 16, 16>>(l, stream, l.x_bytes, l.w_bytes);
    if (l.bc == 64)  return conv_launch<conv_k64_kernel<MF, 64, 256, 1, 8>>(l, stream, l.x_bytes, l.w_bytes);
    if (l.bp == 128) return conv_launch<conv_k64_kernel<MF, 128, 128, 2, 4>>(l, stream, l.x_bytes, l.w_bytes);
    if (l.bc == 256) return conv_launch<conv_k64_kernel<MF, 256, 256, 2, 4, 2>>(l, stream, l.x_bytes, l.w_bytes);
    return conv_launch<conv_k64_kernel<MF, 128, 256, 2, 4>>(l, stream, l.x_bytes, l.w_bytes);
}

static int64_t persistent_grid(int64_t tiles) { return tiles <= INT32_MAX && tiles > sbg_cu_count() ? sbg_cu_count() : tiles; }

static void fit_gather(ConvLaunch& l)
{
    ConvArgs& a = l.a;
    a.ctiles = (a.Cout + 127) / 128;
    if (a.nphase <= 1) {
        a.nphase = 1; a.ph_tap0[0] = 0; a.ph_ntaps[0] = a.ntaps; a.ph_OH[0] = a.OH; a.ph_OW[0] = a.OW; a.ph_P[0] = a.P; a.ph_yoff[0] = 0;
    }
    int pmax = 0;
    for (int i = 0; i < a.nphase; i++) if (a.ph_P[i] > pmax) pmax = a.ph_P[i];
    a.ptiles = ((pmax + 255) / 256) * a.nphase;
    l.family = CONV_GATHER; l.bc = 128; l.bp = 256;
    l.grid_x = persistent_grid((int64_t)a.ptiles * a.ctiles); l.grid_y = 1; l.block = 768; l.lds = kGatherLds;
    a.ph_rot_div = (int)(l.grid_x / ((int64_t)a.ctiles * a.nphase)); if (a.ph_rot_div < 1) a.ph_rot_div = 1;
    conv_prof_phases(l, 4128256 + (a.nphase > 1 ? 1000000 * a.nphase : 0));
}

static void fit_halo(ConvLaunch& l, int TH, int TW)
{
    ConvArgs& a = l.a;
    {
        const bool plain = conv_is_plain(a);
        const bool fast = ((a.Cout & 7) == 0) && ((((uintptr_t)a.y) & 15) == 0) && (((a.ys_n | a.ys_h | a.ys_w) & 7) == 0)
                          && ((((uintptr_t)a.oscale) & 15) == 0) && ((((uintptr_t)a.bias) & 15) == 0) && a.ydtype != SBG_F16;
        const bool nz_ok = !a.noise || (((((uintptr_t)a.noise) & 15) == 0) && (a.noise_sn & 3) == 0 && (a.OW & 3) == 0
                                        && (int64_t)a.N * (a.noise_sn > 0 ? a.noise_sn : 0) + (int64_t)a.OH * a.OW < (1ll << 28));
        a.lds_params = !plain && fast && nz_ok && (int64_t)a.N * a.Cout < (1ll << 28);
    }
    a.ctiles = (a.Cout + 127) / 128;
    a.ptiles = a.N * (a.OH / TH) * (a.OW / TW);
    l.family = CONV_HALO; l.bc = TH; l.bp = TW;
    l.grid_x = persistent_grid((int64_t)a.ptiles * a.ctiles); l.grid_y = 1; l.block = 768; l.lds = halo_lds(TH, TW);
    conv_prof_phases(l, 3128256);
}

static void fit_tile(ConvLaunch& l, int BC, int BP, int NSTAGE = 3)
{
    ConvArgs& a = l.a;
    a.ctiles = (a.Cout + BC - 1) / BC;
    a.ptiles = (a.P + BP - 1) / BP;
    l.family = CONV_K64; l.bc = BC; l.bp = BP;
    l.grid_x = (int64_t)a.ptiles * a.ctiles; l.grid_y = (unsigned)(a.ksplit > 1 ? a.ksplit : 1); l.block = 512; l.lds = k64_lds(BC, BP, NSTAGE);
    conv_prof_phases(l, 1000000 + BC * 1000 + BP);
}

__global__ __launch_bounds__(256) void conv_ksplit_reduce_kernel(const float* ws, float* y, int64_t n, int ksplit, int accumulate)
{
    const int sub = threadIdx.x & 15;
    const int64_t step = (int64_t)gridDim.x * 16;
    for (int64_t i = (int64_t)blockIdx.x * 16 + (threadIdx.x >> 4); i < n; i += step) {
        float s = 0.f;
        for (int k = sub; k < ksplit; k += 16) s += ws[(int64_t)k * n + i];
        for (int m = 8; m >= 1; m >>= 1) s += __shfl_xor(s, m, 64);
        if (sub == 0) y[i] = accumulate ? y[i] + s : s;
    }
}

__global__ __launch_bounds__(256) void conv_ksplit_reduce_epi_kernel(const float* ws, ConvArgs p, int64_t n, int ksplit)
{
    const int64_t groups = n >> 3;
    const int hw = p.OH * p.OW;
    for (int64_t g = (int64_t)blockIdx.x * 256 + threadIdx.x; g < groups; g += (int64_t)gridDim.x * 256) {
        const int64_t i = g << 3;
        float acc[8] = {0.f, 0.f, 0.f, 0.f, 0.f, 0.f, 0.f, 0.f};
        for (int k = 0; k < ksplit; k++) {
            float v[8];
            Vec8<float>::ld(ws + (int64_t)k * n + i, v);
#pragma unroll
            for (int e = 0; e < 8; e++) acc[e] += v[e];
        }
        const int64_t pix = i / p.Cout; const int co = (int)(i - pix * p.Cout);
        const int img = (int)(pix / hw), pp = (int)(pix - (int64_t)img * hw);
// ... 51 lines not shown
```

### style-big-gan_amd/csrc/fromrgb.hip

```cpp
#include "sbg_common.h"

namespace {

constexpr int MAX_CI = 4;

struct FromArgs {
    const float* img; const float* w; const float* bias; const void* dy; const void* ysaved;
    void* y; float* dimg; float* partial;
    int N, Ci, Co; int64_t HW;
    int act; float alpha, gain, clamp;
    int blocks_per_n;
};

static __device__ __forceinline__ float act_fwd(float v, int act, float alpha)
{
    if (act == SBG_ACT_RELU) return fmaxf(v, 0.0f);
    if (act == SBG_ACT_LRELU) return v > 0.0f ? v : v * alpha;
    return v;
}
static __device__ __forceinline__ float act_grad_from_y(float y, int act, float alpha, float gain, float clamp)
{
    if (clamp >= 0.0f && !(fabsf(y) < clamp)) return 0.0f;
    if (act == SBG_ACT_RELU) return y > 0.0f ? gain : 0.0f;
    if (act == SBG_ACT_LRELU) return y > 0.0f ? gain : gain * alpha;
    return gain;
}

template <class T>
__global__ void __launch_bounds__(256) fromrgb_fwd_kernel(FromArgs p)
{
    __shared__ float4_t px[256];
    const int lpp = p.Co >> 3, ppw = 64 / lpp;
    const int n = blockIdx.x / p.blocks_per_n, blk = blockIdx.x % p.blocks_per_n;
    const int lane = threadIdx.x & 63, wave = threadIdx.x >> 6;
    const int cl = lane & (lpp - 1), pl = lane / lpp;
    float w[MAX_CI][8], b[8];
#pragma unroll
    for (int j = 0; j < 8; j++) {
        b[j] = p.bias ? p.bias[cl * 8 + j] : 0.0f;
#pragma unroll
        for (int c = 0; c < MAX_CI; c++) w[c][j] = c < p.Ci ? p.w[(int64_t)(cl * 8 + j) * p.Ci + c] : 0.0f;
    }
    const float* ib = p.img + (int64_t)n * p.Ci * p.HW;
    T* yb = (T*)p.y + (int64_t)n * p.HW * p.Co;
    for (int64_t chunk = (int64_t)blk * 256; chunk < p.HW; chunk += (int64_t)p.blocks_per_n * 256) {
        {
            const int64_t pix = chunk + threadIdx.x;
            float4_t v = {0.f, 0.f, 0.f, 0.f};
            if (pix < p.HW) {
#pragma unroll
                for (int c = 0; c < MAX_CI; c++)
                    if (c < p.Ci) v[c] = ib[(int64_t)c * p.HW + pix];
            }
            __syncthreads();
            px[threadIdx.x] = v;
            __syncthreads();
        }
        for (int q = 0; q < 64; q += ppw) {
            const int loc = wave * 64 + q + pl;
            const int64_t pix = chunk + loc;
            if (pix >= p.HW) continue;
            const float4_t v = px[loc];
            float o[8];
#pragma unroll
            for (int j = 0; j < 8; j++) {
                float a = b[j];
#pragma unroll
                for (int c = 0; c < MAX_CI; c++) a += v[c] * w[c][j];
                a = act_fwd(a, p.act, p.alpha) * p.gain;
                if (p.clamp >= 0.0f) a = fminf(fmaxf(a, -p.clamp), p.clamp);
                o[j] = a;
            }
            Vec8<T>::st(yb + pix * p.Co + cl * 8, o);
        }
    }
}

template <class T, int CI, bool DIMG>
__global__ void __launch_bounds__(256) fromrgb_bwd_kernel(FromArgs p)
{
    constexpr int RS = MAX_CI * 8 + 8 + 1;
    __shared__ float4_t px[256];
    extern __shared__ float red[];
    const int lpp = p.Co >> 3, ppw = 64 / lpp;
    const int n = blockIdx.x / p.blocks_per_n, blk = blockIdx.x % p.blocks_per_n;
    const int lane = threadIdx.x & 63, wave = threadIdx.x >> 6;
    const int cl = lane & (lpp - 1), pl = lane / lpp;
    float w[MAX_CI][8];
#pragma unroll
    for (int j = 0; j < 8; j++)
#pragma unroll
        for (int c = 0; c < MAX_CI; c++) w[c][j] = c < p.Ci ? p.w[(int64_t)(cl * 8 + j) * p.Ci + c] : 0.0f;
    float dw[MAX_CI][8], db[8];
#pragma unroll
    for (int j = 0; j < 8; j++) {
        db[j] = 0.0f;
#pragma unroll
        for (int c = 0; c < MAX_CI; c++) dw[c][j] = 0.0f;
    }
    const float* ib = p.img + (int64_t)n * p.Ci * p.HW;
    const T* dyb = (const T*)p.dy + (int64_t)n * p.HW * p.Co;
    const T* ysb = (const T*)p.ysaved + (int64_t)n * p.HW * p.Co;
    float* dib = DIMG ? p.dimg + (int64_t)n * p.Ci * p.HW : nullptr;
    const float gpos = p.gain, gneg = p.act == SBG_ACT_LRELU ? p.gain * p.alpha : (p.act == SBG_ACT_RELU ? 0.0f : p.gain);
    const float rail = p.clamp >= 0.0f ? p.clamp : __builtin_inff();
    for (int64_t chunk = (int64_t)blk * 256; chunk < p.HW; chunk += (int64_t)p.blocks_per_n * 256) {
        {
            const int64_t pix = chunk + threadIdx.x;
            float4_t v = {0.f, 0.f, 0.f, 0.f};
            if (pix < p.HW) {
#pragma unroll
                for (int c = 0; c < MAX_CI; c++)
                    if (c < p.Ci) v[c] = ib[(int64_t)c * p.HW + pix];
            }
            __syncthreads();
            px[threadIdx.x] = v;
            __syncthreads();
        }
        for (int q = 0; q < 64; q += ppw) {
            const int loc = wave * 64 + q + pl;
            const int64_t pix = chunk + loc;
            const bool ok = pix < p.HW;
            float g[8], yv[8];
            if (ok) {
                Vec8<T>::ld(dyb + pix * p.Co + cl * 8, g);
                Vec8<T>::ld(ysb + pix * p.Co + cl * 8, yv);
            }
            const float4_t v = px[loc & 255];
            float di[MAX_CI] = {0.f, 0.f, 0.f, 0.f};
#pragma unroll
            for (int j = 0; j < 8; j++) {
                const bool live = ok && (fabsf(yv[j]) < rail);
                const float d1 = live ? g[j] * (yv[j] > 0.0f ? gpos : gneg) : 0.0f;
                db[j] += d1;
#pragma unroll
                for (int c = 0; c < CI; c++) { dw[c][j] += d1 * v[c]; if (DIMG) di[c] += d1 * w[c][j]; }
            }
            if (DIMG) {
#pragma unroll
                for (int c = 0; c < CI; c++) {
                    float a = di[c];
                    for (int m = lpp >> 1; m >= 1; m >>= 1) a += __shfl_xor(a, m, 64);
                    if (ok && cl == (c & (lpp - 1)) && c < p.Ci) dib[(int64_t)c * p.HW + pix] = a;
                }
            }
        }
    }
#pragma unroll
    for (int j = 0; j < 8; j++) {
#pragma unroll
        for (int c = 0; c < MAX_CI; c++) {
            float a = c < CI ? dw[c][j] : 0.0f;
            for (int m = lpp; m < 64; m <<= 1) a += __shfl_xor(a, m, 64);
            if (pl == 0) red[(wave * lpp + cl) * RS + c * 8 + j] = a;
        }
        float a = db[j];
        for (int m = lpp; m < 64; m <<= 1) a += __shfl_xor(a, m, 64);
        if (pl == 0) red[(wave * lpp + cl) * RS + MAX_CI * 8 + j] = a;
    }
    __syncthreads();
    float* out = p.partial + ((int64_t)n * p.blocks_per_n + blk) * ((int64_t)p.Co * p.Ci + p.Co);
    for (int idx = threadIdx.x; idx < p.Co * (p.Ci + 1); idx += 256) {
        const bool is_b = idx >= p.Co * p.Ci;
        const int co = is_b ? idx - p.Co * p.Ci : idx / p.Ci, c = is_b ? 0 : idx % p.Ci;
        const int gq = co >> 3, j = co & 7;
        const int slot = is_b ? MAX_CI * 8 + j : c * 8 + j;
        float s = 0.0f;
        for (int wv = 0; wv < 4; wv++) s += red[(wv * lpp + gq) * RS + slot];
        out[idx] = s;
    }
}

static int check_shape(int N, int Ci, int Co, int64_t HW)
{
    const int lpp = Co >> 3;
    SBG_CHECK(N >= 1 && HW >= 1 && Ci >= 1 && Ci <= MAX_CI, "fromrgb: bad sizes (Cin <= %d)", MAX_CI);
    SBG_CHECK(Co >= 8 && Co <= 512 && (Co & 7) == 0 && (lpp & (lpp - 1)) == 0, "fromrgb: Cout must be 8 * 2^k <= 512");
    SBG_CHECK((int64_t)N * Co * HW <= INT32_MAX, "fromrgb: tensors are limited to INT_MAX elements");
    return 0;
}

static int blocks_for(int N, int64_t HW)
{
    int64_t want = (HW + 255) / 256;
    int64_t cap = (256 * 8 + N - 1) / N;
    if (want > cap) want = cap;
    if (want < 1) want = 1;
    return (int)want;
}

}

extern "C" int sbg_fromrgb_supported(int Ci, int Co, int act)
{
    const int lpp = Co >> 3;
    return (Ci >= 1 && Ci <= MAX_CI && Co >= 8 && Co <= 512 && (Co & 7) == 0 && (lpp & (lpp - 1)) == 0
            && (act == SBG_ACT_LINEAR || act == SBG_ACT_RELU || act == SBG_ACT_LRELU)) ? 1 : 0;
}

extern "C" int sbg_fromrgb_bwd_blocks(int N, int64_t HW) { return blocks_for(N, HW); }

extern "C" int sbg_fromrgb_fwd(const float* img, const float* w, const float* bias, void* y, int dtype, int N, int Ci, int Co, int64_t HW,
                               int act, float alpha, float gain, float clamp, sbg_stream_t stream_)
{
    SBG_CHECK(img && w && y, "fromrgb_fwd: null pointer");
    if (int rc = check_shape(N, Ci, Co, HW)) return rc;
    SBG_CHECK(sbg_fromrgb_supported(Ci, Co, act), "fromrgb_fwd: unsupported activation %d", act);
    SBG_CHECK(dtype == SBG_BF16 || dtype == SBG_F16, "fromrgb_fwd: 16-bit output only");
    FromArgs a = {};
    a.img = img; a.w = w; a.bias = bias; a.y = y; a.N = N; a.Ci = Ci; a.Co = Co; a.HW = HW; a.act = act; a.alpha = alpha; a.gain = gain; a.clamp = clamp;
    a.blocks_per_n = blocks_for(N, HW);
    hipStream_t stream = (hipStream_t)stream_;
    SbgProfScope prof(stream, SBG_K_FROMRGB, 2.0 * N * Co * (double)Ci * HW, (double)N * HW * (2.0 * Co + 4.0 * Ci), {N, Ci, Co, (int)HW, 0, 0, 0});
    dim3 grid((unsigned)(N * a.blocks_per_n)), block(256);
    if (dtype == SBG_BF16) SBG_LAUNCH(fromrgb_fwd_kernel<bf16_s>, grid, block, 0, stream, a);
    else                   SBG_LAUNCH(fromrgb_fwd_kernel<f16_s>, grid, block, 0, stream, a);
    SBG_HIP_LAUNCH_CHECK();
    return 0;
}

extern "C" int sbg_fromrgb_bwd(const float* img, const float* w, const void* dy, const void* y, float* dimg, float* partial, int dtype,
                               int N, int Ci, int Co, int64_t HW, int act, float alpha, float gain, float clamp, sbg_stream_t stream_)
{
    SBG_CHECK(img && w && dy && y && partial, "fromrgb_bwd: null pointer");
    if (int rc = check_shape(N, Ci, Co, HW)) return rc;
    SBG_CHECK(sbg_fromrgb_supported(Ci, Co, act), "fromrgb_bwd: unsupported activation %d", act);
    SBG_CHECK(dtype == SBG_BF16 || dtype == SBG_F16, "fromrgb_bwd: 16-bit activations only");
    FromArgs a = {};
    a.img = img; a.w = w; a.dy = dy; a.ysaved = y; a.dimg = dimg; a.partial = partial;
    a.N = N; a.Ci = Ci; a.Co = Co; a.HW = HW; a.act = act; a.alpha = alpha; a.gain = gain; a.clamp = clamp;
    a.blocks_per_n = blocks_for(N, HW);
    hipStream_t stream = (hipStream_t)stream_;
    SbgProfScope prof(stream, SBG_K_FROMRGB, 4.0 * N * Co * (double)Ci * HW, (double)N * HW * (4.0 * Co + 8.0 * Ci), {N, Ci, Co, (int)HW, 1, Ci == 3 ? 3 : MAX_CI, dimg ? 1 : 0});
    dim3 grid((unsigned)(N * a.blocks_per_n)), block(256);
    const int lds = 4 * (Co >> 3) * (MAX_CI * 8 + 8 + 1) * (int)sizeof(float);
#define SBG_FROMRGB_BWD(T_) do { \
        if (Ci == 3) { if (dimg) SBG_LAUNCH((fromrgb_bwd_kernel<T_, 3, true>), grid, block, lds, stream, a); else SBG_LAUNCH((fromrgb_bwd_kernel<T_, 3, false>), grid, block, lds, stream, a); } \
        else { if (dimg) SBG_LAUNCH((fromrgb_bwd_kernel<T_, MAX_CI, true>), grid, block, lds, stream, a); else SBG_LAUNCH((fromrgb_bwd_kernel<T_, MAX_CI, false>), grid, block, lds, stream, a); } } while (0)
    if (dtype == SBG_BF16) SBG_FROMRGB_BWD(bf16_s); else SBG_FROMRGB_BWD(f16_s);
#undef SBG_FROMRGB_BWD
    SBG_HIP_LAUNCH_CHECK();
    return 0;
}
```

### style-big-gan_amd/torch_utils/misc.py

```python
import contextlib
import re

import numpy as np
import torch


def assert_shape(tensor, ref_shape):
    if tensor.ndim != len(ref_shape):
        raise AssertionError(f"Wrong number of dimensions: got {tensor.ndim}, expected {len(ref_shape)}")
    for idx, (size, ref) in enumerate(zip(tensor.shape, ref_shape)):
        if ref is not None and int(size) != int(ref):
            raise AssertionError(f"Wrong size for dimension {idx}: got {size}, expected {ref}")


def profiled_function(fn):
    def wrapper(*args, **kwargs):
        with torch.autograd.profiler.record_function(fn.__name__):
            return fn(*args, **kwargs)
    wrapper.__name__ = fn.__name__
    return wrapper


class InfiniteSampler(torch.utils.data.Sampler):

# ... 6 lines not shown
    def __iter__(self):
        order = np.arange(len(self.dataset))
        rnd, window = None, 0
        if self.shuffle:
            rnd = np.random.RandomState(self.seed)
            rnd.shuffle(order)
            window = int(np.rint(order.size * self.window_size))
        idx = 0
        while True:
            i = idx % order.size
            if idx % self.num_replicas == self.rank:
                yield order[i]
            if window >= 2:
                j = (i - rnd.randint(window)) % order.size
                order[i], order[j] = order[j], order[i]
            idx += 1


def params_and_buffers(module):
    assert isinstance(module, torch.nn.Module)
    return list(module.parameters()) + list(module.buffers())


def named_params_and_buffers(module):
    assert isinstance(module, torch.nn.Module)
    return list(module.named_parameters()) + list(module.named_buffers())


def copy_params_and_buffers(src_module, dst_module, require_all=False):
    src = dict(named_params_and_buffers(src_module))
    for name, tensor in named_params_and_buffers(dst_module):
        assert (name in src) or (not require_all)
        if name in src:
            tensor.copy_(src[name].detach()).requires_grad_(tensor.requires_grad)


@contextlib.contextmanager
def ddp_sync(module, sync):
    assert isinstance(module, torch.nn.Module)
    if sync or not hasattr(module, "no_sync"):
        yield
    else:
        with module.no_sync():
            yield


def check_ddp_consistency(module, ignore_regex=None):
    assert isinstance(module, torch.nn.Module)
    for name, tensor in named_params_and_buffers(module):
        fullname = type(module).__name__ + "." + name
        if ignore_regex is not None and re.fullmatch(ignore_regex, fullname):
            continue
        tensor = tensor.detach()
        other = tensor.clone()
        torch.distributed.broadcast(tensor=other, src=0)
        assert (torch.nan_to_num(tensor) == torch.nan_to_num(other)).all(), fullname


class _Cat0(torch.autograd.Function):

    @staticmethod
    def forward(ctx, *tensors):
        ctx.sizes = [t.shape[0] for t in tensors]
        first = tensors[0]
        fmt = torch.channels_last if (first.ndim == 4 and first.is_contiguous(memory_format=torch.channels_last) and not first.is_contiguous()) else torch.contiguous_format
        out = torch.empty([sum(ctx.sizes), *first.shape[1:]], dtype=first.dtype, device=first.device, memory_format=fmt)
        i = 0
        for t in tensors:
            out.narrow(0, i, t.shape[0]).copy_(t)
            i += t.shape[0]
        return out

    @staticmethod
    def backward(ctx, dout):
        return tuple(dout.split(ctx.sizes))


def cat0(tensors):
    tensors = list(tensors)
    if len(tensors) == 1:
        return tensors[0]
    if any(t.dtype != tensors[0].dtype or t.shape[1:] != tensors[0].shape[1:] for t in tensors) or tensors[0].device.type != 'cuda':
        return torch.cat(tensors)
    return _Cat0.apply(*tensors)
```

### style-big-gan_amd/torch_utils/ops/conv2d_gradfix.py

```python
import contextlib
import ctypes
import typing
import weakref

import numpy as np
import torch

from ... import _lib
from . import bias_act
from ._tail import Tail

enabled = False
weight_gradients_disabled = False


@contextlib.contextmanager
def no_weight_gradients():
    global weight_gradients_disabled
    old = weight_gradients_disabled
    weight_gradients_disabled = True
    try:
        yield
    finally:
        weight_gradients_disabled = old
# ... 85 lines not shown
    if x_cat_dim == 1:
        a = a.contiguous(memory_format=torch.channels_last)
    return [(a, b)]



_pack_cache = {}
_ptr_epoch = {}


def _on_optimizer_step(optimizer, args, kwargs):
    for group in optimizer.param_groups:
        for q in group["params"]:
            if isinstance(q, torch.Tensor) and q.device.type == "cuda":
                k = q.data_ptr()
                _ptr_epoch[k] = _ptr_epoch.get(k, 0) + 1


from torch.optim.optimizer import register_optimizer_step_post_hook as _register_step_hook
_register_step_hook(_on_optimizer_step)


def invalidate_packed_weights():
    _pack_cache.clear()


def is_mixed(x, w):
    return w.dtype == torch.float32 and x.dtype in (torch.bfloat16, torch.float16)


def _packed_weight(w, rows_dim, dtype, bp, gain):
    assert w.dtype == torch.float32 and w.ndim == 4 and rows_dim in (0, 1)
    a_dim, b_dim = rows_dim, 1 - rows_dim
    A, B, kh, kw = w.shape[a_dim], w.shape[b_dim], w.shape[2], w.shape[3]
    base = w._base if w._base is not None else w
    cacheable = isinstance(base, torch.nn.Parameter)
    key = None
    if cacheable:
        key = (base.data_ptr(), w.storage_offset(), tuple(w.shape), tuple(w.stride()), rows_dim, dtype, bp, float(gain))
        hit = _pack_cache.get(key)
        stamp = (base._version, _ptr_epoch.get(base.data_ptr(), 0))
        if hit is not None and hit[0]() is base and hit[1] == stamp:
            return hit[2], hit[3]
    out = torch.empty([kh * kw, A, bp], dtype=dtype, device=w.device)
    w2 = torch.empty([A, B], dtype=torch.float32, device=w.device) if rows_dim == 0 else None
    wd = w.detach()
    _lib.check(_lib.load().sbg_pack_weight(wd.data_ptr(), out.data_ptr(), _lib.dtype_code(dtype), A, B, kh, kw, wd.stride(a_dim), wd.stride(b_dim),
                                           wd.stride(2), wd.stride(3), bp, float(gain), _lib.ptr(w2), _lib.stream_ptr(w.device)), "sbg_pack_weight")
    if cacheable:
        if len(_pack_cache) > 256:
            for k in [k for k, v in _pack_cache.items() if v[0]() is None]:
                del _pack_cache[k]
            if len(_pack_cache) > 2048:
                _pack_cache.clear()
        _pack_cache[key] = (weakref.ref(base), (base._version, _ptr_epoch.get(base.data_ptr(), 0)), out, w2)
    return out, w2


def _unpack_wgrad(out, ca, cb, wshape, wstride, rows_dim, gain, w=None, dw2=None):
    dev = out.device if out is not None else w.device
    dw = torch.empty_strided(wshape, wstride, dtype=torch.float32, device=dev)
    a_dim, b_dim = rows_dim, 1 - rows_dim
    assert wshape[a_dim] == ca and wshape[b_dim] == cb
    _lib.check(_lib.load().sbg_unpack_wgrad(_lib.ptr(out), out.stride(0) if out is not None else 0, out.stride(1) if out is not None else 0,
                                            dw.data_ptr(), _lib.ptr(w), _lib.ptr(dw2), ca, cb, wshape[2], wshape[3],
                                            wstride[a_dim], wstride[b_dim], wstride[2], wstride[3], float(gain), _lib.stream_ptr(dev)), "sbg_unpack_wgrad")
    return dw


def _conv_params(x, wp, y, y_step):
    p = _lib.ConvParams()
    n, cin, ih, iw = x.shape
    assert wp.shape[2] == cin and x.stride(1) == 1 and y.stride(1) == 1 and wp.is_contiguous() and x.dtype == wp.dtype
    p.x, p.w, p.y = x.data_ptr(), wp.data_ptr(), y.data_ptr()
    p.xdtype, p.ydtype = _lib.dtype_code(x.dtype), _lib.dtype_code(y.dtype)
    p.N, p.IH, p.IW, p.Cin, p.Cout = n, ih, iw, cin, wp.shape[1]
    p.xs_n, p.xs_h, p.xs_w = x.stride(0), x.stride(2), x.stride(3)
    p.ys_n, p.ys_h, p.ys_w = y.stride(0), y.stride(2) * y_step[0], y.stride(3) * y_step[1]
    p.ws_slab, p.ws_co = wp.stride(0), wp.stride(1)
    p.act, p.alpha, p.gain, p.clamp = 1, 0.0, 1.0, -1.0
    return p


def _igemm(x, wp, y, taps, stride, oh, ow, y_off=(0, 0), y_step=(1, 1), oscale=None, accumulate=False, epi=None):
    lib = _lib.load()
    p = _conv_params(x, wp, y, y_step)
    p.y = y.data_ptr() + (y_off[0] * y.stride(2) + y_off[1] * y.stride(3)) * y.element_size()
    p.oscale = oscale.data_ptr() if oscale is not None else None
    p.OH, p.OW = oh, ow
    p.stride, p.ntaps = stride, len(taps)
    assert 1 <= len(taps) <= _lib.SBG_MAX_TAPS
    for i, (dy, dx, slab) in enumerate(taps):
        p.tap_dy[i], p.tap_dx[i], p.tap_slab[i] = dy, dx, slab
    p.accumulate = int(accumulate)
    if epi is not None:
        assert not accumulate and y_step == (1, 1) and epi.act.fused and epi.post is None
        osc32, nz32, p.noise_stride_n, b32, _ = epi.operands(x.shape[0], wp.shape[1], oh, ow)
        if osc32 is not None:
            p.oscale = osc32.data_ptr()
        p.noise, p.bias = _lib.ptr(nz32), _lib.ptr(b32)
        p.act, p.alpha, p.gain, p.clamp = epi.act.code, epi.act.alpha, epi.act.gain, epi.act.clamp
    nbytes = lib.sbg_conv2d_igemm_workspace(p)
    if nbytes < 0:
        _lib.check(1, "sbg_conv2d_igemm_workspace")
    ws = torch.empty([nbytes // 4], dtype=torch.float32, device=x.device) if nbytes > 0 else None
    p.workspace = ws.data_ptr() if ws is not None else None
    _lib.check(lib.sbg_conv2d_igemm(p, _lib.stream_ptr(x.device)), "sbg_conv2d_igemm")


def _igemm_phases(x, wp, y, phases, s):
    lib = _lib.load()
    p = _conv_params(x, wp, y, (s, s))
    p.OH, p.OW = max(ph[2] for ph in phases), max(ph[3] for ph in phases)
    p.stride = 1
    t = 0
    for i, (a, b, goh, gow, taps) in enumerate(phases):
        p.ph_ntaps[i], p.ph_oh[i], p.ph_ow[i] = len(taps), goh, gow
        p.ph_yoff[i] = a * y.stride(2) + b * y.stride(3)
        for dy, dx, slab in taps:
            p.tap_dy[t], p.tap_dx[t], p.tap_slab[t] = dy, dx, slab
            t += 1
    p.ntaps, p.nphase = t, len(phases)
    _lib.check(lib.sbg_conv2d_igemm(p, _lib.stream_ptr(x.device)), "sbg_conv2d_igemm")


def _launch_groups(taps):
    m = _lib.SBG_MAX_TAPS
    return [taps[i:i + m] for i in range(0, len(taps), m)]


def epilogue_fusable(x):
    return x.dtype in (torch.bfloat16, torch.float16)


def _conv_forward(x, w, stride, padding, epi=None, wgain=1.0):
    n, cin, ih, iw = x.shape
    cout, cin_w, kh, kw = w.shape
    mixed = is_mixed(x, w)
    assert cin == cin_w and (x.dtype == w.dtype or mixed) and (mixed or wgain == 1.0)
    (sh, sw), (ph, pw) = stride, padding
    assert sh == sw, "conv2d: only square strides are implemented"
    oh = (ih + 2 * ph - kh) // sh + 1
    ow = (iw + 2 * pw - kw) // sw + 1
    assert oh >= 1 and ow >= 1
    xp = _pad_channels(x)
    taps = [(i - ph, j - pw, i * kw + j) for i in range(kh) for j in range(kw)]
    if mixed:
        passes = [(xp, _packed_weight(w, 0, x.dtype, xp.shape[1], wgain)[0])]
    else:
        wpk = w.permute(2, 3, 0, 1).reshape(kh * kw, cout, cin)
        if xp.shape[1] != cin:
            wpk = torch.nn.functional.pad(wpk, (0, xp.shape[1] - cin))
        passes = _mfma_operands(xp, wpk, 1, 2, b_dense=True)
    multi = len(passes) > 1 or len(taps) > _lib.SBG_MAX_TAPS
    y = torch.empty([n, cout, oh, ow], dtype=torch.float32 if multi else x.dtype, device=x.device, memory_format=torch.channels_last)
    assert epi is None or (not multi)
    first = True
    for xa, wa in passes:
        wa = wa.contiguous()
        for grp in _launch_groups(taps):
            _igemm(xa, wa, y, grp, sh, oh, ow, accumulate=not first, epi=epi)
            first = False
    return y.to(x.dtype) if y.dtype != x.dtype else y


def _conv_transpose_forward(x, w, stride, padding, output_padding, wgain=1.0):
    n, cin, ih, iw = x.shape
    cin_w, cout, kh, kw = w.shape
    mixed = is_mixed(x, w)
    assert cin == cin_w and (x.dtype == w.dtype or mixed) and (mixed or wgain == 1.0)
    (sh, sw), (ph, pw), (oph, opw) = stride, padding, output_padding
    assert sh == sw, "conv_transpose2d: only square strides are implemented"
    s = sh
    oh = (ih - 1) * s - 2 * ph + kh + oph
    ow = (iw - 1) * s - 2 * pw + kw + opw
    assert oh >= 1 and ow >= 1
    xp = _pad_channels(x)
    if mixed:
        passes = [(xp, _packed_weight(w, 1, x.dtype, xp.shape[1], wgain)[0])]
    else:
        wpk = w.permute(2, 3, 1, 0).reshape(kh * kw, cout, cin)
        if xp.shape[1] != cin:
            wpk = torch.nn.functional.pad(wpk, (0, xp.shape[1] - cin))
        passes = _mfma_operands(xp, wpk, 1, 2, b_dense=True)
    phases = []
    need_zero = False
    for a in range(s):
        for b in range(s):
            goh, gow = (oh - a + s - 1) // s, (ow - b + s - 1) // s
            if goh <= 0 or gow <= 0:
                continue
            taps = [((a + ph - i) // s, (b + pw - j) // s, i * kw + j)
                    for i in range(kh) if (a + ph - i) % s == 0
                    for j in range(kw) if (b + pw - j) % s == 0]
            if not taps:
                need_zero = True
                continue
            phases.append((a, b, goh, gow, taps))
    multi = len(passes) > 1 or any(len(t) > _lib.SBG_MAX_TAPS for *_, t in phases)
    y = torch.empty([n, cout, oh, ow], dtype=torch.float32 if multi else x.dtype, device=x.device, memory_format=torch.channels_last)
    if need_zero:
        y.zero_()
    first = True
    if (not multi and 2 <= len(phases) <= 4 and sum(len(t) for *_, t in phases) <= _lib.SBG_MAX_TAPS):
        xa, wa = passes[0]
        _igemm_phases(xa, wa.contiguous(), y, phases, s)
        return y
    for xa, wa in passes:
        wa = wa.contiguous()
        for a, b, goh, gow, taps in phases:
            for gi, grp in enumerate(_launch_groups(taps)):
                _igemm(xa, wa, y, grp, 1, goh, gow, y_off=(a, b), y_step=(s, s), accumulate=(not first) or gi > 0)
        first = False
    return y.to(x.dtype) if y.dtype != x.dtype else y


def _wgrad(a, b, stride, taps):
    lib = _lib.load()
    assert a.dtype == b.dtype and a.shape[0] == b.shape[0]
    ca, cb = a.shape[1], b.shape[1]
    pw = a.shape[3]
    if (len(taps) == 9 and stride in (1, 2) and pw in (8, 16)
            and all(taps[t] == (taps[0][0] + t // 3, taps[0][1] + t % 3) for t in range(9))):
        a = torch.nn.functional.pad(a, (0, 32 - pw))
    ap, bp = _pad_channels(a), _pad_channels(b)
    cap, cbp = ap.shape[1], bp.shape[1]
    out = torch.empty([len(taps), cap, cbp], dtype=torch.float32, device=a.device)
    first = True
    for aa, bb in _mfma_operands(ap, bp, 0, 0):
        aa, bb = _cl(aa), _cl(bb)
        for g0 in range(0, len(taps), _lib.SBG_MAX_TAPS):
            grp = taps[g0:g0 + _lib.SBG_MAX_TAPS]
            p = _lib.WgradParams()
            p.a, p.b, p.out = aa.data_ptr(), bb.data_ptr(), out[g0:].data_ptr()
            p.dtype = _lib.dtype_code(aa.dtype)
            p.N, p.PH, p.PW, p.Ca = aa.shape[0], aa.shape[2], aa.shape[3], cap
            p.BH, p.BW, p.Cb = bb.shape[2], bb.shape[3], cbp
            p.as_n, p.as_h, p.as_w = aa.stride(0), aa.stride(2), aa.stride(3)
            p.bs_n, p.bs_h, p.bs_w = bb.stride(0), bb.stride(2), bb.stride(3)
            p.stride, p.ntaps = stride, len(grp)
            for i, (dy, dx) in enumerate(grp):
                p.tap_dy[i], p.tap_dx[i] = dy, dx
            p.accumulate = int(not first)
            nbytes = lib.sbg_conv2d_wgrad_workspace(p)
            if nbytes < 0:
                _lib.check(1, "sbg_conv2d_wgrad_workspace")
            ws = torch.empty([max(nbytes, 4) // 4], dtype=torch.float32, device=a.device) if nbytes > 0 else None
            p.workspace = ws.data_ptr() if ws is not None else None
            _lib.check(lib.sbg_conv2d_wgrad(p, _lib.stream_ptr(a.device)), "sbg_conv2d_wgrad")
        first = False
    return out[:, :ca, :cb]



class ConvCfg(typing.NamedTuple):
    transpose: bool
    stride: tuple
    padding: tuple
    output_padding: tuple = (0, 0)
    wgain: float = 1.0

    @classmethod
    def make(cls, transpose, stride=1, padding=0, output_padding=0, wgain=1.0):
        return cls(bool(transpose), _pair(stride), _pair(padding), _pair(output_padding), float(wgain))

    def adjoint(self, x_hw, dy_hw, k_hw):
        op = (0, 0)
        if not self.transpose:
            op = tuple(x_hw[i] - (dy_hw[i] - 1) * self.stride[i] - (1 - 2 * self.padding[i]) - (k_hw[i] - 1) for i in range(2))
        return self._replace(transpose=not self.transpose, output_padding=op)


class _Conv(torch.autograd.Function):

    @staticmethod
    def forward(ctx, x, w, cfg):
        _lib.require_cuda(x, "conv2d")
        if x.dtype != w.dtype and not is_mixed(x, w):
            raise RuntimeError(f"conv2d: input ({x.dtype}) and weight ({w.dtype}) must have the same dtype (or an fp32 weight with 16-bit input)")
        if not cfg.transpose:
            y = _conv_forward(x, w, cfg.stride, cfg.padding, wgain=cfg.wgain)
        else:
            y = _conv_transpose_forward(x, w, cfg.stride, cfg.padding, cfg.output_padding, wgain=cfg.wgain)
        ctx.save_for_backward(x, w)
        ctx.cfg = cfg
        return y

    @staticmethod
    def backward(ctx, dy):
        x, w = ctx.saved_tensors
        dx = dw = None
        if ctx.needs_input_grad[0]:
            if dy.dtype != x.dtype:
                dy = dy.to(x.dtype)
            dx = _Conv.apply(dy, w, ctx.cfg.adjoint(x.shape[2:], dy.shape[2:], w.shape[2:]))
            assert dx.shape == x.shape
        if ctx.needs_input_grad[1] and not weight_gradients_disabled:
            dw = _ConvWgrad.apply(dy, x, ctx.cfg, tuple(w.shape), wmeta_of(x, w))
        return dx, dw, None
# ... 72 lines not shown
```

### style-big-gan_amd/torch_utils/ops/conv2d_resample.py

```python
import torch

from . import bias_act
from . import conv2d_gradfix
from . import conv_bias_act
from . import modulate
from . import upfirdn2d
from .upfirdn2d import _get_filter_size, _parse_padding


def _conv(x, w, stride=1, padding=0, groups=1, transpose=False, flip_weight=True, tail=None, wgain=1.0):
    if not flip_weight:
        w = w.flip([2, 3])
    if tail is not None and not transpose and conv_bias_act.fusable(x, w, tail.act.name, groups):
        return conv_bias_act.conv2d_bias_act(x, w, tail.bias, stride, padding, *tail.act, wgain=wgain)
    fn = conv2d_gradfix.conv_transpose2d if transpose else conv2d_gradfix.conv2d
    y = fn(x, w, stride=stride, padding=padding, groups=groups, wgain=wgain)
    return _tail(y, tail)


def _tail(y, tail):
    if tail is None:
        return y
    b = tail.bias
    if b is not None and b.dtype != y.dtype:
        b = b.to(y.dtype)
    return bias_act._BiasAct.apply(y, b, bias_act._Cfg(tail.act))


def lowpass_padding(f, down, padding):
    fw, fh = _get_filter_size(f)
    px0, px1, py0, py1 = _parse_padding(padding)
    return [px0 + (fw - down + 1) // 2, px1 + (fw - down) // 2, py0 + (fh - down + 1) // 2, py1 + (fh - down) // 2]


def conv2d_resample(x, w, f=None, up=1, down=1, padding=0, groups=1, flip_weight=True, flip_filter=False, bias_act_tail=None, fir_tail=None,
                    wgain=1.0, prefiltered=False):
    tail = bias_act_tail
    assert isinstance(x, torch.Tensor) and x.ndim == 4
    assert isinstance(w, torch.Tensor) and w.ndim == 4 and (w.dtype == x.dtype or conv2d_gradfix.is_mixed(x, w))
    assert wgain == 1.0 or conv2d_gradfix.is_mixed(x, w)
    assert f is None or (isinstance(f, torch.Tensor) and f.ndim in [1, 2] and f.dtype == torch.float32)
    assert isinstance(up, int) and up >= 1 and isinstance(down, int) and down >= 1
    assert isinstance(groups, int) and groups >= 1
    assert not prefiltered or (up == 1 and down > 1 and w.shape[2] > 1)
    cout, cin_g, kh, kw = [int(s) for s in w.shape]
    fw, fh = _get_filter_size(f)
    px0, px1, py0, py1 = _parse_padding(padding)

    if up > 1:
        px0 += (fw + up - 1) // 2; px1 += (fw - up) // 2
        py0 += (fh + up - 1) // 2; py1 += (fh - up) // 2
    if down > 1:
        px0 += (fw - down + 1) // 2; px1 += (fw - down) // 2
        py0 += (fh - down + 1) // 2; py1 += (fh - down) // 2
    pad4 = [px0, px1, py0, py1]
    pointwise = (kh == 1 and kw == 1)

    if pointwise and down > 1 and up == 1:
        x = upfirdn2d.upfirdn2d(x, f, down=down, padding=pad4, flip_filter=flip_filter)
        return _conv(x, w, groups=groups, flip_weight=flip_weight, tail=tail, wgain=wgain)

    if pointwise and up > 1 and down == 1:
        x = _conv(x, w, groups=groups, flip_weight=flip_weight, wgain=wgain)
        return _tail(upfirdn2d.upfirdn2d(x, f, up=up, padding=pad4, gain=up ** 2, flip_filter=flip_filter), tail)

    if down > 1 and up == 1:
        if not prefiltered:
            x = upfirdn2d.upfirdn2d(x, f, padding=pad4, flip_filter=flip_filter)
        return _conv(x, w, stride=down, groups=groups, flip_weight=flip_weight, tail=tail, wgain=wgain)

    if up > 1:
        if groups == 1:
            wt = w.transpose(0, 1)
        else:
            wt = w.reshape(groups, cout // groups, cin_g, kh, kw).transpose(1, 2).reshape(groups * cin_g, cout // groups, kh, kw)
        px0 -= kw - 1; px1 -= kw - up
        py0 -= kh - 1; py1 -= kh - up
        pxt = max(min(-px0, -px1), 0)
        pyt = max(min(-py0, -py1), 0)
        x = _conv(x, wt, stride=up, padding=[pyt, pxt], groups=groups, transpose=True, flip_weight=(not flip_weight), wgain=wgain)
        fpad = [px0 + pxt, px1 + pxt, py0 + pyt, py1 + pyt]
        if fir_tail is not None and down == 1 and upfirdn2d.fir_tail_supported(x, f, fpad, flip_filter):
            return upfirdn2d.fir_bias_act(x, f, fpad, up ** 2, fir_tail.oscale, fir_tail.noise, fir_tail.bias, *fir_tail.act, flip_filter=flip_filter,
                                          post_scale=fir_tail.post)
        x = upfirdn2d.upfirdn2d(x, f, padding=fpad, gain=up ** 2, flip_filter=flip_filter)
        if fir_tail is not None:
            if fir_tail.oscale is not None:
                x = modulate.scale_nc(x, fir_tail.oscale, fir_tail.noise)
            elif fir_tail.noise is not None:
                x = x + fir_tail.noise.to(x.dtype)
            x = _tail(x, fir_tail)
            return x if fir_tail.post is None else modulate.scale_nc(x, fir_tail.post)
        if down > 1:
            x = upfirdn2d.upfirdn2d(x, f, down=down, flip_filter=flip_filter)
        return _tail(x, tail)

    if px0 == px1 and py0 == py1 and px0 >= 0 and py0 >= 0:
        return _conv(x, w, padding=[py0, px0], groups=groups, flip_weight=flip_weight, tail=tail, wgain=wgain)

    x = upfirdn2d.upfirdn2d(x, (f if up > 1 else None), up=up, padding=pad4, gain=up ** 2, flip_filter=flip_filter)
    x = _conv(x, w, groups=groups, flip_weight=flip_weight, wgain=wgain)
    if down > 1:
        x = upfirdn2d.upfirdn2d(x, f, down=down, flip_filter=flip_filter)
    return _tail(x, tail)
```

### style-big-gan_amd/torch_utils/ops/conv_bias_act.py

```python
import torch

from . import bias_act as _ba
from . import conv2d_gradfix as _cg
from . import upfirdn2d as _up
from ._tail import Act, Tail

first_order = False


def _act_backward(act, dy, y, want_db):
    if act.trivial:
        return dy, None
    bcfg = _ba._Cfg(act, 1)
    fused = _ba._grad_and_bias_sum(dy, y, bcfg) if want_db else None
    return fused if fused is not None else (_ba._BiasActGrad.apply(dy, None, None, y, bcfg, torch.channels_last), None)


def _backward_from_dy(ctx, x, w, d1, db_fused, needs):
    dx = dw = db = None
    if needs[0]:
        dx = _cg._Conv.apply(d1, w, ctx.ccfg.adjoint(x.shape[2:], d1.shape[2:], w.shape[2:]))
    if needs[1] and not _cg.weight_gradients_disabled:
        dw = _cg._ConvWgrad.apply(d1, x, ctx.ccfg, tuple(w.shape), _cg.wmeta_of(x, w))
    if ctx.has_bias and needs[2]:
        db = (db_fused if db_fused is not None else _ba._sum_to_bias(d1, 1)).to(ctx.b_dtype)
    return dx, dw, db


def _forward(ctx, x, w, b, ccfg, act):
    y = _cg._conv_forward(x, w, ccfg.stride, ccfg.padding, epi=Tail(act, bias=b), wgain=ccfg.wgain)
    ctx.ccfg, ctx.act = ccfg, act
    ctx.has_bias = b is not None
    ctx.b_dtype = b.dtype if b is not None else None
    return y


class _ConvBiasAct(torch.autograd.Function):

    @staticmethod
    def forward(ctx, x, w, b, ccfg, act):
        y = _forward(ctx, x, w, b, ccfg, act)
        ctx.save_for_backward(x, w, y)
        return y

    @staticmethod
    def backward(ctx, dy):
        x, w, y = ctx.saved_tensors
        d1, db_fused = _act_backward(ctx.act, dy.contiguous(memory_format=torch.channels_last), y, ctx.has_bias and ctx.needs_input_grad[2])
        return (*_backward_from_dy(ctx, x, w, d1, db_fused, ctx.needs_input_grad), None, None)


class _ConvBiasActFir(torch.autograd.Function):

    @staticmethod
    def forward(ctx, x, w, b, f, ccfg, act, fcfg):
        y = _forward(ctx, x, w, b, ccfg, act)
        out = _up._launch(y, f, *fcfg)
        ctx.save_for_backward(x, w, y, f)
        ctx.fcfg = fcfg
        return out

    @staticmethod
    def backward(ctx, dout):
        if torch.is_grad_enabled():
            raise RuntimeError("conv_bias_act_fir: first-order only; leave torch_utils.ops.conv_bias_act.first_order = False for graphs that are differentiated twice")
        x, w, y, f = ctx.saved_tensors
        fused = _up.fir_transposed_dact(dout, f, ctx.fcfg, y.shape[2:], y, *ctx.act)
        if fused is not None:
            d1, db_fused = fused
        else:
            gcfg = ctx.fcfg.adjoint(y.shape[2:], dout.shape[2:], f)
            dy = _up._Upfirdn2d.apply(dout.to(y.dtype), f, gcfg).contiguous(memory_format=torch.channels_last)
            d1, db_fused = _act_backward(ctx.act, dy, y, True)
        return (*_backward_from_dy(ctx, x, w, d1, db_fused, ctx.needs_input_grad), None, None, None, None)


def fir_fusable(x, w, act, f, groups=1):
    return (first_order and fusable(x, w, act, groups) and x.dtype in (torch.bfloat16, torch.float16) and w.shape[0] % 64 == 0
            and f is not None and f.ndim == 2 and tuple(f.shape) == (4, 4) and x.shape[2] >= 16 and _up._taps_exact(f, x.dtype))


def conv2d_bias_act_fir(x, w, b, f, fpad, stride=1, padding=0, act="linear", alpha=None, gain=None, clamp=None, wgain=1.0, flip_filter=False, fgain=1.0):
    fcfg = _up.FirCfg(1, 1, 1, 1, *_up._parse_padding(fpad), bool(flip_filter), float(fgain))
    return _ConvBiasActFir.apply(x, w, b, f, _cg.ConvCfg.make(False, stride, padding, wgain=wgain), Act.make(act, alpha, gain, clamp), fcfg)


def fusable(x, w, act, groups=1):
    return (groups == 1 and x.device.type == "cuda" and _cg.epilogue_fusable(x) and Act(act).fused
            and (x.dtype == w.dtype or _cg.is_mixed(x, w)))


def conv2d_bias_act(x, w, b=None, stride=1, padding=0, act="linear", alpha=None, gain=None, clamp=None, wgain=1.0):
    return _ConvBiasAct.apply(x, w, b, _cg.ConvCfg.make(False, stride, padding, wgain=wgain), Act.make(act, alpha, gain, clamp))
```

### style-big-gan_amd/torch_utils/ops/fromrgb.py

```python
import torch

from ... import _lib
from .bias_act import Act

enabled = False


def usable(img, weight, act, out_dtype):
    return (enabled and img.device.type == "cuda" and img.dtype == torch.float32 and img.ndim == 4 and out_dtype in (torch.bfloat16, torch.float16)
            and weight.ndim == 4 and weight.shape[2] == 1 and weight.shape[3] == 1 and Act(act).fused
            and bool(_lib.load().sbg_fromrgb_supported(weight.shape[1], weight.shape[0], Act(act).code)))


class _FromRGB(torch.autograd.Function):

    @staticmethod
    def forward(ctx, img, w, bias, act, out_dtype):
        n, ci, h, wd = img.shape
        co = w.shape[0]
        ic = img.contiguous()
        wc = w.detach().to(torch.float32).contiguous()
        bc = bias.detach().to(torch.float32).contiguous() if bias is not None else None
        y = torch.empty([n, co, h, wd], dtype=out_dtype, device=img.device, memory_format=torch.channels_last)
        _lib.check(_lib.load().sbg_fromrgb_fwd(ic.data_ptr(), wc.data_ptr(), _lib.ptr(bc), y.data_ptr(), _lib.dtype_code(out_dtype), n, ci, co, h * wd,
                                               act.code, act.alpha, act.gain, act.clamp, _lib.stream_ptr(img.device)), "sbg_fromrgb_fwd")
        ctx.save_for_backward(ic, wc, y)
        ctx.act, ctx.has_bias = act, bias is not None
        ctx.dtypes = (w.dtype, bias.dtype if bias is not None else None)
        return y

    @staticmethod
    def backward(ctx, dy):
        ic, wc, y = ctx.saved_tensors
        act = ctx.act
        if torch.is_grad_enabled():
            raise RuntimeError("fromrgb: first-order only; set torch_utils.ops.fromrgb.enabled = False for double backward (R1, gradient penalty)")
        lib = _lib.load()
        n, ci, h, wd = ic.shape
        co = wc.shape[0]
        dyc = dy.to(y.dtype).contiguous(memory_format=torch.channels_last)
        dimg = torch.empty_like(ic) if ctx.needs_input_grad[0] else None
        nb = lib.sbg_fromrgb_bwd_blocks(n, h * wd)
        part = torch.empty([n * nb, co * ci + co], dtype=torch.float32, device=ic.device)
        _lib.check(lib.sbg_fromrgb_bwd(ic.data_ptr(), wc.data_ptr(), dyc.data_ptr(), y.data_ptr(), _lib.ptr(dimg), part.data_ptr(), _lib.dtype_code(y.dtype),
                                       n, ci, co, h * wd, act.code, act.alpha, act.gain, act.clamp, _lib.stream_ptr(ic.device)), "sbg_fromrgb_bwd")
        sums = part.sum(0)
        dw = sums[:co * ci].reshape(co, ci).to(ctx.dtypes[0]) if ctx.needs_input_grad[1] else None
        db = sums[co * ci:].to(ctx.dtypes[1]) if (ctx.has_bias and ctx.needs_input_grad[2]) else None
        return dimg, dw, db, None, None


def fromrgb(img, weight, bias, weight_gain, act, gain=None, clamp=None, out_dtype=torch.bfloat16):
    w2d = weight.reshape(weight.shape[0], weight.shape[1]) * weight_gain
    return _FromRGB.apply(img, w2d, bias, Act.make(act, gain=gain, clamp=clamp), out_dtype)
```

### style-big-gan_amd/train_parts/discriminators.py

```python
import numpy as np
import torch

from .. import utils
from ..torch_utils import misc
from ..torch_utils.ops import conv2d_gradfix, conv_bias_act, fromrgb, upfirdn2d
from . import generators as _g
from .generators import Conv2dLayer, FullyConnectedLayer, MappingNetwork

discriminators = utils.ClassRegistry()


def _attention_module(channels):
    from ..biggan.layers import Attention
    return Attention(channels)


class DiscriminatorBlock(torch.nn.Module):
    def __init__(self,
        in_channels         = None,
        tmp_channels        = None,
        out_channels        = None,
        resolution          = None,
        img_channels        = None,
        first_layer_idx     = None,
        architecture        = 'resnet',
        attention           = False,
        activation          = 'lrelu',
        resample_filter     = (1,3,3,1),
        conv_clamp          = None,
        use_fp16            = False,
        fp16_channels_last  = False,
        freeze_layers       = 0,
    ):
        assert None not in (in_channels, tmp_channels, out_channels, resolution, img_channels, first_layer_idx)
        assert in_channels in [0, tmp_channels]
        assert architecture in ['orig', 'skip', 'resnet']
        super().__init__()
        self.in_channels = in_channels
        self.resolution = resolution
        self.img_channels = img_channels
        self.first_layer_idx = first_layer_idx
        self.architecture = architecture
        self.use_fp16 = use_fp16
        self.channels_last = bool(use_fp16)
        self.register_buffer('resample_filter', upfirdn2d.setup_filter(list(resample_filter)))
        self.attention = _attention_module(out_channels) if attention else None

        self.num_layers = 0

        def next_trainable():
            trainable = (self.first_layer_idx + self.num_layers) >= freeze_layers
            self.num_layers += 1
            return trainable

        common = dict(activation=activation, conv_clamp=conv_clamp, channels_last=self.channels_last)
        if in_channels == 0 or architecture == 'skip':
            self.fromrgb = Conv2dLayer(img_channels, tmp_channels, kernel_size=1, trainable=next_trainable(), **common)
        self.conv0 = Conv2dLayer(tmp_channels, tmp_channels, kernel_size=3, trainable=next_trainable(), **common)
        self.conv1 = Conv2dLayer(tmp_channels, out_channels, kernel_size=3, down=2, trainable=next_trainable(),
                                 resample_filter=resample_filter, **common)
        if architecture == 'resnet':
            self.skip = Conv2dLayer(tmp_channels, out_channels, kernel_size=1, bias=False, down=2, trainable=next_trainable(),
                                    resample_filter=resample_filter, channels_last=self.channels_last)

    def forward(self, x, img, force_fp32=False):
        reduced = self.use_fp16 and not force_fp32
        dtype = _g.LOW_PRECISION if reduced else torch.float32
        fmt = torch.channels_last if reduced else torch.contiguous_format

        if x is not None:
            misc.assert_shape(x, [None, self.in_channels, self.resolution, self.resolution])
            x = x.to(dtype=dtype, memory_format=fmt)

        if self.in_channels == 0 or self.architecture == 'skip':
            misc.assert_shape(img, [None, self.img_channels, self.resolution, self.resolution])
            fr = self.fromrgb
            if (self.architecture != 'skip' and fr.up == 1 and fr.down == 1 and fromrgb.usable(img, fr.weight, fr.activation, dtype)):
                y = fromrgb.fromrgb(img, fr.weight, fr.bias, fr.weight_gain, fr.activation, gain=fr.act_gain, clamp=fr.conv_clamp, out_dtype=dtype)
            else:
                img = img.to(dtype=dtype, memory_format=fmt)
                y = self.fromrgb(img)
            x = x + y if x is not None else y
            img = upfirdn2d.downsample2d(img, self.resample_filter) if self.architecture == 'skip' else None

        residual = self.architecture == 'resnet'
        shortcut = self.skip(x, gain=np.sqrt(0.5)) if residual else None
        c0, c1 = self.conv0, self.conv1
        g1 = np.sqrt(0.5) if residual else 1
        if (conv_bias_act.first_order and x.device.type == 'cuda' and conv2d_gradfix.is_mixed(x, c0.weight) and c0.up == 1 and c0.down == 1 and c1.up == 1
                and c1.down == 2 and c1.weight.shape[2] > 1 and conv_bias_act.fir_fusable(x, c0.weight, c0.activation, c1.resample_filter)):
            x = c1(c0(x, then_lowpass_of=c1), gain=g1, prefiltered=True)
        else:
            x = c1(c0(x), gain=g1)
        if residual:
            x = shortcut + x
        if self.attention is not None:
            x = self.attention(x.to(torch.float32)).to(dtype)
        assert x.dtype == dtype
        return x, img


class MinibatchStdLayer(torch.nn.Module):

    def __init__(self, group_size, num_channels=1):
        super().__init__()
        self.group_size = group_size
        self.num_channels = num_channels

    def forward(self, x):
        N, C, H, W = x.shape
        G = min(int(self.group_size), N) if self.group_size is not None else N
        F = self.num_channels
        if x.device.type == 'cuda' and x.dtype == torch.float32 and x.is_contiguous() and N % G == 0 and C % F == 0:
            return _MinibatchStd.apply(x, G, F)
        return _minibatch_std_composite(x, G, F)


def _minibatch_std_composite(x, G, F):
    N, C, H, W = x.shape
    c = C // F
    y = x.reshape(G, -1, F, c, H, W)
    y = y - y.mean(dim=0)
    y = y.square().mean(dim=0)
    y = (y + 1e-8).sqrt()
    y = y.mean(dim=[2, 3, 4])
    y = y.reshape(-1, F, 1, 1)
    y = y.repeat(G, 1, H, W)
    return torch.cat([x, y], dim=1)


class _MinibatchStd(torch.autograd.Function):
    @staticmethod
    def forward(ctx, x, G, F):
        from .. import _lib
        N, C, H, W = x.shape
        y = torch.empty([N, C + F, H, W], dtype=torch.float32, device=x.device)
        lib = _lib.load()
        ws = torch.empty([max(lib.sbg_mbstd_workspace(N, C, H * W, G, F), 4) // 4], dtype=torch.float32, device=x.device)
        _lib.check(lib.sbg_mbstd_fwd(_lib.ptr(x), _lib.ptr(y), _lib.ptr(ws), N, C, H * W, G, F, _lib.stream_ptr(x.device)), "sbg_mbstd_fwd")
        ctx.save_for_backward(x)
        ctx.cfg = (G, F)
        return y

    @staticmethod
    def backward(ctx, dy):
        (x,) = ctx.saved_tensors
        G, F = ctx.cfg
        if torch.is_grad_enabled():
            with torch.enable_grad():
                xx = x if x.requires_grad else x.detach().requires_grad_(True)
                (dx,) = torch.autograd.grad(_minibatch_std_composite(xx, G, F), xx, dy, create_graph=True)
            return dx, None, None
        from .. import _lib
        N, C, H, W = x.shape
        dyc = dy.contiguous()
        dx = torch.empty_like(x)
        _lib.check(_lib.load().sbg_mbstd_bwd(_lib.ptr(x), _lib.ptr(dyc), _lib.ptr(dx), N, C, H * W, G, F, _lib.stream_ptr(x.device)), "sbg_mbstd_bwd")
        return dx, None, None


class DiscriminatorEpilogue(torch.nn.Module):
    def __init__(self,
        in_channels         = None,
        cmap_dim            = None,
        resolution          = None,
        img_channels        = None,
        architecture        = 'resnet',
        mbstd_group_size    = 4,
        mbstd_num_channels  = 1,
        activation          = 'lrelu',
        conv_clamp          = None,
    ):
        assert None not in (in_channels, cmap_dim, resolution, img_channels)
        assert architecture in ['orig', 'skip', 'resnet']
        super().__init__()
        self.in_channels = in_channels
# ... 251 lines not shown
```

### style-big-gan_amd/train_parts/generators.py

```python
import numpy as np
import torch

from .. import utils
from ..torch_utils import misc
from ..torch_utils.ops import bias_act, conv2d_gradfix, conv2d_resample, conv_bias_act, grouped_gemm, modconv, modulate, torgb, upfirdn2d
from ..torch_utils.ops._tail import Tail

generators = utils.ClassRegistry()

LOW_PRECISION = torch.bfloat16
import os as _os
style_bank_enabled = _os.environ.get('SBG_STYLE_BANK', '1') != '0'
premodulate = _os.environ.get('SBG_PREMODULATE', '1') != '0'


def set_low_precision(dtype):
    global LOW_PRECISION
    assert dtype in (torch.bfloat16, torch.float16)
    LOW_PRECISION = dtype


def low_precision():
    return LOW_PRECISION

# ... 79 lines not shown

def _zero(like):
    key = (like.device, like.dtype)
    z = _zero_cache.get(key)
    if z is None:
        z = _zero_cache[key] = torch.zeros([1], device=like.device, dtype=like.dtype)
    return z


class _ScaledLinear(torch.autograd.Function):

    @staticmethod
    def forward(ctx, x, w, b, alpha):
        ctx.save_for_backward(x, w)
        ctx.alpha = alpha
        ctx.has_bias = b is not None
        if b is not None:
            return torch.addmm(b.unsqueeze(0), x, w.t(), alpha=alpha)
        return torch.addmm(_zero(x), x, w.t(), beta=0, alpha=alpha)

    @staticmethod
    def backward(ctx, g):
        x, w = ctx.saved_tensors
        alpha = ctx.alpha
        dx = dw = db = None
        if torch.is_grad_enabled():
            if ctx.needs_input_grad[0]:
                dx = g.mm(w) * alpha
            if ctx.needs_input_grad[1]:
                dw = g.t().mm(x) * alpha
        else:
            if ctx.needs_input_grad[0]:
                dx = torch.addmm(_zero(g), g, w, beta=0, alpha=alpha)
            if ctx.needs_input_grad[1]:
                dw = torch.addmm(_zero(g), g.t(), x, beta=0, alpha=alpha)
        if ctx.has_bias and ctx.needs_input_grad[2]:
            db = g.sum(0)
        return dx, dw, db, None


def _scaled_linear(x, w, b, alpha):
    if x.ndim != 2 or x.device.type != 'cuda':
        y = x.matmul(w.t()) * alpha
        return y if b is None else y + b
    return _ScaledLinear.apply(x, w, b, alpha)


class Conv2dLayer(torch.nn.Module):
    def __init__(self,
        in_channels,
        out_channels,
        kernel_size,
        bias            = True,
        activation      = 'linear',
        up              = 1,
        down            = 1,
        resample_filter = [1,3,3,1],
        conv_clamp      = None,
        channels_last   = False,
        trainable       = True,
    ):
        super().__init__()
        self.activation = activation
        self.up = up
        self.down = down
        self.conv_clamp = conv_clamp
        self.register_buffer('resample_filter', upfirdn2d.setup_filter(resample_filter))
        self.padding = kernel_size // 2
        self.weight_gain = 1 / np.sqrt(in_channels * (kernel_size ** 2))
        self.act_gain = bias_act.activation_funcs[activation].def_gain
        fmt = torch.channels_last if channels_last else torch.contiguous_format
        weight = torch.randn([out_channels, in_channels, kernel_size, kernel_size]).to(memory_format=fmt)
        bias = torch.zeros([out_channels]) if bias else None
        if trainable:
            self.weight = torch.nn.Parameter(weight)
            self.bias = torch.nn.Parameter(bias) if bias is not None else None
        else:
            self.register_buffer('weight', weight)
            if bias is not None:
                self.register_buffer('bias', bias)
            else:
                self.bias = None

    def forward(self, x, gain=1, prefiltered=False, then_lowpass_of=None):
        b = self.bias
        clamp = self.conv_clamp * gain if self.conv_clamp is not None else None
        if then_lowpass_of is not None:
            nxt = then_lowpass_of
            assert self.up == 1 and self.down == 1 and nxt.up == 1 and nxt.down > 1
            return conv_bias_act.conv2d_bias_act_fir(x, self.weight, b, nxt.resample_filter, conv2d_resample.lowpass_padding(nxt.resample_filter, nxt.down, nxt.padding),
                                                     padding=self.padding, act=self.activation, gain=self.act_gain * gain, clamp=clamp, wgain=self.weight_gain)
        tail = Tail.make(self.activation, gain=self.act_gain * gain, clamp=clamp, bias=b)
        if conv2d_gradfix.is_mixed(x, self.weight) and x.device.type == 'cuda':
            return conv2d_resample.conv2d_resample(x=x, w=self.weight, f=self.resample_filter, up=self.up, down=self.down, padding=self.padding,
                                                   flip_weight=(self.up == 1), bias_act_tail=tail, wgain=self.weight_gain, prefiltered=prefiltered)
        w = self.weight * self.weight_gain
        return conv2d_resample.conv2d_resample(x=x, w=w.to(x.dtype), f=self.resample_filter, up=self.up, down=self.down,
                                               padding=self.padding, flip_weight=(self.up == 1), bias_act_tail=tail, prefiltered=prefiltered)


class MappingNetwork(torch.nn.Module):
    def __init__(self,
        z_dim           = None,
        c_dim           = None,
        w_dim           = None,
        num_ws          = None,
        num_layers      = 8,
        embed_features  = None,
        layer_features  = None,
        activation      = 'lrelu',
        lr_multiplier   = 0.01,
        w_avg_beta      = 0.995,
    ):
        assert z_dim is not None and c_dim is not None and w_dim is not None
        super().__init__()
        self.z_dim, self.c_dim, self.w_dim = z_dim, c_dim, w_dim
        self.num_ws, self.num_layers, self.w_avg_beta = num_ws, num_layers, w_avg_beta
        if embed_features is None:
            embed_features = w_dim
        if c_dim == 0:
            embed_features = 0
        if layer_features is None:
            layer_features = w_dim
        widths = [z_dim + embed_features] + [layer_features] * (num_layers - 1) + [w_dim]
        if c_dim > 0:
            self.embed = FullyConnectedLayer(c_dim, embed_features)
        for idx in range(num_layers):
            setattr(self, f'fc{idx}', FullyConnectedLayer(widths[idx], widths[idx + 1], activation=activation, lr_multiplier=lr_multiplier))
        if num_ws is not None and w_avg_beta is not None:
            self.register_buffer('w_avg', torch.zeros([w_dim]))

    def forward(self, z, c, truncation_psi=1, truncation_cutoff=None, skip_w_avg_update=False):
        parts = []
        if self.z_dim > 0:
            misc.assert_shape(z, [None, self.z_dim])
            parts.append(normalize_2nd_moment(z.to(torch.float32)))
        if self.c_dim > 0:
            misc.assert_shape(c, [None, self.c_dim])
            parts.append(normalize_2nd_moment(self.embed(c.to(torch.float32))))
        w = parts[0] if len(parts) == 1 else torch.cat(parts, dim=1)
        for idx in range(self.num_layers):
            w = getattr(self, f'fc{idx}')(w)
        track = self.w_avg_beta is not None and self.training and not skip_w_avg_update
        if track:
            for part in w.detach().chunk(max(int(getattr(self, 'w_avg_rounds', 1)), 1)):
                self.w_avg.copy_(torch.lerp(part.mean(dim=0), self.w_avg, self.w_avg_beta))
        if self.num_ws is not None:
            w = w.unsqueeze(1).repeat([1, self.num_ws, 1])
        if truncation_psi == 1:
            return w
        assert self.w_avg_beta is not None
        if self.num_ws is None or truncation_cutoff is None:
            return torch.lerp(self.w_avg, w, truncation_psi)
        w[:, :truncation_cutoff] = torch.lerp(self.w_avg, w[:, :truncation_cutoff], truncation_psi)
        return w


class SynthesisLayer(torch.nn.Module):
    def __init__(self,
        in_channels     = None,
        out_channels    = None,
        w_dim           = None,
        resolution      = None,
        kernel_size     = 3,
        up              = 1,
        use_noise       = True,
        activation      = 'lrelu',
        resample_filter = (1,3,3,1),
        conv_clamp      = None,
        channels_last   = False,
    ):
        assert None not in (in_channels, out_channels, w_dim, resolution)
        super().__init__()
        self.resolution = resolution
        self.up = up
        self.use_noise = use_noise
        self.activation = activation
        self.conv_clamp = conv_clamp
# ... 471 lines not shown
```

Before: 632.7 img/s.

## Fuse producer's lrelu backward and bias-grad sums into consumer conv dgrad epilogue

The discriminator's input-gradient conv can now carry the previous layer's leaky-ReLU/clamp backward tail in its epilogue. It reads the producer's saved output, applies the activation derivative, writes the pre-activation gradient and emits per-tile bias-gradient partials. A handle attached to the producer output (conv or fromRGB) lets that layer skip its own activation backward pass and one read-write of the gradient tensor. The cost is extra kernel template variants, an extra epilogue load, and a rounding step that must match the unfused path. It also adds handle bookkeeping that relies on the tensor having a single consumer.

```diff
diff --git a/include/sbg_hip.h b/include/sbg_hip.h
--- a/include/sbg_hip.h
+++ b/include/sbg_hip.h
@@ -72,8 +72,10 @@
     int act; float alpha, gain, clamp;
     void* workspace; int ksplit;
     int nphase; int ph_ntaps[4], ph_oh[4], ph_ow[4]; int64_t ph_yoff[4];
+    const void* dact_y; float* dact_partial; int dact_act; float dact_alpha, dact_gain, dact_clamp;
 } sbg_conv_params;
 int64_t sbg_conv2d_igemm_workspace(const sbg_conv_params* p);
+int64_t sbg_conv2d_igemm_dact_rows(const sbg_conv_params* p);
 int     sbg_conv2d_igemm(const sbg_conv_params* p, sbg_stream_t stream);
 typedef struct sbg_conv_launch_info {
     int dims[7]; double flops, bytes;
diff --git a/style-big-gan_amd/_lib.py b/style-big-gan_amd/_lib.py
--- a/style-big-gan_amd/_lib.py
+++ b/style-big-gan_amd/_lib.py
@@ -55,6 +55,8 @@
         ("act", ctypes.c_int), ("alpha", ctypes.c_float), ("gain", ctypes.c_float), ("clamp", ctypes.c_float),
         ("workspace", ctypes.c_void_p), ("ksplit", ctypes.c_int),
         ("nphase", ctypes.c_int), ("ph_ntaps", ctypes.c_int * 4), ("ph_oh", ctypes.c_int * 4), ("ph_ow", ctypes.c_int * 4), ("ph_yoff", ctypes.c_int64 * 4),
+        ("dact_y", ctypes.c_void_p), ("dact_partial", ctypes.c_void_p), ("dact_act", ctypes.c_int),
+        ("dact_alpha", ctypes.c_float), ("dact_gain", ctypes.c_float), ("dact_clamp", ctypes.c_float),
     ]
 
 
@@ -141,6 +143,7 @@
     ("sbg_upfirdn2d_separable_supported", _c.c_int, [_c.c_int] * 3),
     ("sbg_upfirdn2d_separable", _c.c_int, [_c.c_void_p] * 3 + [_c.c_int] * 11 + [_c.c_float, _c.c_void_p]),
     ("sbg_conv2d_igemm_workspace", _c.c_int64, [_c.POINTER(ConvParams)]),
+    ("sbg_conv2d_igemm_dact_rows", _c.c_int64, [_c.POINTER(ConvParams)]),
     ("sbg_conv2d_igemm", _c.c_int, [_c.POINTER(ConvParams), _c.c_void_p]),
     ("sbg_conv2d_igemm_plan", _c.c_int, [_c.POINTER(ConvParams), _c.POINTER(ConvLaunchInfo), _c.c_int]),
     ("sbg_conv2d_wgrad_workspace", _c.c_int64, [_c.POINTER(WgradParams)]),
diff --git a/style-big-gan_amd/csrc/conv_common.h b/style-big-gan_amd/csrc/conv_common.h
--- a/style-big-gan_amd/csrc/conv_common.h
+++ b/style-big-gan_amd/csrc/conv_common.h
@@ -42,6 +42,7 @@
     int ksplit;
     int64_t y_split_stride;
     int lds_params;
+    const unsigned short* dact_y; float* dact_partial; float dact_alpha, dact_gain, dact_clamp;
 };
 
 #define SBG_CONV_IS_PLAIN(a) (((a).act <= SBG_ACT_LINEAR) && (a).gain == 1.f && (a).clamp < 0.f && !(a).bias && !(a).noise && !(a).oscale)
@@ -80,6 +81,7 @@
     ConvArgs call;
     int ksplit; bool reduce_epi;
     int64_t workspace_bytes;
+    int64_t dact_rows;
 };
 
 static inline void conv_prof(ConvLaunch& l, double macs, double outpix, int ntaps, int stride, int rows, int code)
diff --git a/style-big-gan_amd/csrc/conv_device.h b/style-big-gan_amd/csrc/conv_device.h
--- a/style-big-gan_amd/csrc/conv_device.h
+++ b/style-big-gan_amd/csrc/conv_device.h
@@ -41,13 +41,17 @@
     return u;
 }
 
+template <int DT> static __device__ __forceinline__ unsigned short to16(float v) { return DT == SBG_F16 ? f32_to_f16_bits(v) : f32_to_bf16_bits(v); }
+template <int DT> static __device__ __forceinline__ float from16(unsigned short b) { return DT == SBG_F16 ? f16_bits_to_f32(b) : bf16_bits_to_f32(b); }
+
 typedef __attribute__((address_space(3))) const float lds_cfloat;
 typedef __attribute__((address_space(3))) const float4_t lds_cfloat4;
 struct LdsParams { lds_cfloat* base; int c; int tw; };
-template <int TC, int TP, int YDT, bool PLAIN, bool NUNI, bool LP = false, class PixFn>
+template <int TC, int TP, int YDT, bool PLAIN, bool NUNI, bool LP = false, bool DACT = false, class PixFn>
 static __device__ __forceinline__ void conv_epilogue_fast(const ConvArgs& p, float4_t (&acc)[TC][TP], int cbase, int fg, PixFn pix, int64_t ybase,
-                                                          const LdsParams* lp = nullptr, int y0 = 0, int x0 = 0)
-{
+                                                          const LdsParams* lp = nullptr, int y0 = 0, int x0 = 0, int prow = 0)
+{
+    static_assert(!DACT || (PLAIN && !LP && YDT != SBG_F32), "the backward tail rides on plain 16-bit launches");
     constexpr int TH2 = TC / 2;
     const float alpha = (p.act == SBG_ACT_LRELU) ? p.alpha : (p.act == SBG_ACT_RELU ? 0.f : 1.f);
     const float lsel = alpha <= 1.f ? __builtin_inff() : -__builtin_inff();
@@ -55,6 +59,9 @@
     const float gain = p.gain;
     const float* const dummy = reinterpret_cast<const float*>(p.x);
     const bool has_nz = !PLAIN && p.noise != nullptr, has_b = !PLAIN && p.bias != nullptr, has_s = !PLAIN && p.oscale != nullptr;
+    const bool dsum = DACT && p.dact_partial != nullptr, d_always = DACT && !dsum && p.dact_clamp < 0.f;
+    const float d_pos = dsum ? p.dact_gain : 1.f, d_neg = dsum ? p.dact_gain * p.dact_alpha : p.dact_alpha, d_g2 = dsum ? 1.f : p.dact_gain;
+    const float d_cl = p.dact_clamp >= 0.f ? p.dact_clamp : __builtin_inff();
     int64_t yoff[TP]; float nz[TP]; bool ok[TP]; int nn[TP];
 #pragma unroll
     for (int j = 0; j < TP; j++) {
@@ -66,6 +73,16 @@
         if (!PLAIN) {
             if constexpr (LP) nz[j] = lp->base[(oy - y0) * lp->tw + (ox - x0)];
             else              nz[j] = *(has_nz ? p.noise + ((int64_t)n * p.noise_sn + (int64_t)oy * p.OW + ox) : dummy);
+        }
+    }
+    short8_t ysv[DACT ? TH2 : 1][DACT ? TP : 1];
+    float4_t sum_lo[DACT ? TH2 : 1], sum_hi[DACT ? TH2 : 1];
+    if constexpr (DACT) {
+#pragma unroll
+        for (int h = 0; h < TH2; h++) {
+            sum_lo[h] = sum_hi[h] = float4_t{0.f, 0.f, 0.f, 0.f};
+#pragma unroll
+            for (int j = 0; j < TP; j++) ysv[h][j] = *reinterpret_cast<const short8_t*>(p.dact_y + yoff[j] + 32 * h);
         }
     }
     float4_t b_lo[TH2], b_hi[TH2], s_lo[TH2], s_hi[TH2];
@@ -123,6 +140,19 @@
                 if (p.accumulate) { lo += *reinterpret_cast<float4_t*>(dst); hi += *reinterpret_cast<float4_t*>(dst + 4); }
                 *reinterpret_cast<float4_t*>(dst) = lo;
                 *reinterpret_cast<float4_t*>(dst + 4) = hi;
+            } else if constexpr (DACT) {
+                short8_t o;
+                const short8_t ys = ysv[h][j];
+#pragma unroll
+                for (int e = 0; e < 8; e++) {
+                    const float dx = from16<YDT>(to16<YDT>(e < 4 ? lo[e & 3] : hi[e & 3]));
+                    const float yv = from16<YDT>((unsigned short)ys[e]);
+                    const float v = (dx * (yv > 0.f ? d_pos : d_neg)) * d_g2;
+                    const unsigned short r = to16<YDT>((d_always || (yv > -d_cl && yv < d_cl)) ? v : 0.f);
+                    o[e] = (short)r;
+                    if (dsum) { if (e < 4) sum_lo[h][e & 3] += from16<YDT>(r); else sum_hi[h][e & 3] += from16<YDT>(r); }
+                }
+                *reinterpret_cast<short8_t*>((unsigned short*)p.y + yoff[j] + 32 * h) = o;
             } else {
                 short8_t o;
 #pragma unroll
@@ -131,8 +161,32 @@
             }
         }
     }
-}
-
+    if constexpr (DACT) {
+        if (dsum) {
+            float* const row = p.dact_partial + (int64_t)prow * p.Cout + cbase + 8 * fg;
+#pragma unroll
+            for (int h = 0; h < TH2; h++) {
+                float4_t a = sum_lo[h], b = sum_hi[h];
+#pragma unroll
+                for (int m = 1; m < 16; m <<= 1)
+#pragma unroll
+                    for (int e = 0; e < 4; e++) { a[e] += __shfl_xor(a[e], m, 64); b[e] += __shfl_xor(b[e], m, 64); }
+                if ((threadIdx.x & 15) == 0) {
+                    *reinterpret_cast<float4_t*>(row + 32 * h) = a;
+                    *reinterpret_cast<float4_t*>(row + 32 * h + 4) = b;
+                }
+            }
+        }
+    }
+}
+
+
+template <int TC, int TP, bool NUNI = false, class PixFn>
+static __device__ __forceinline__ void conv_epilogue_dact(const ConvArgs& p, float4_t (&acc)[TC][TP], int cbase, int fg, PixFn pix, int prow)
+{
+    if (p.ydtype == SBG_BF16) conv_epilogue_fast<TC, TP, SBG_BF16, true, NUNI, false, true>(p, acc, cbase, fg, pix, 0, nullptr, 0, 0, prow);
+    else                      conv_epilogue_fast<TC, TP, SBG_F16, true, NUNI, false, true>(p, acc, cbase, fg, pix, 0, nullptr, 0, 0, prow);
+}
 
 template <int TC, int TP, bool NUNI = false, class PixFn>
 static __device__ __forceinline__ void conv_epilogue8(const ConvArgs& p, float4_t (&acc)[TC][TP], int cbase, int fg, PixFn pix, int64_t ybase = 0,
diff --git a/style-big-gan_amd/csrc/conv_igemm.hip b/style-big-gan_amd/csrc/conv_igemm.hip
--- a/style-big-gan_amd/csrc/conv_igemm.hip
+++ b/style-big-gan_amd/csrc/conv_igemm.hip
@@ -231,6 +231,7 @@
     for (int t = 0; t < SBG_MAX_TAPS; t++) { a.tap_dy[t] = q.tap_dy[t]; a.tap_dx[t] = q.tap_dx[t]; a.tap_slab[t] = q.tap_slab[t]; }
     a.accumulate = q.accumulate;
     a.P = q.N * q.OH * q.OW; a.ptiles = a.ctiles = 0; a.lds_params = 0; a.ksplit = 1; a.y_split_stride = 0;
+    a.dact_y = nullptr; a.dact_partial = nullptr; a.dact_alpha = 0.f; a.dact_gain = 1.f; a.dact_clamp = -1.f;
     a.nphase = q.nphase > 1 ? q.nphase : 1; a.ph_rot_div = 1;
     for (int i = 0, t0 = 0; i < 4; i++) {
         const bool on = q.nphase > 1 && i < q.nphase;
@@ -312,12 +313,31 @@
     return push(pl, l);
 }
 
+void conv_plan_dact(const sbg_conv_params& q, ConvPlan& pl)
+{
+    if (pl.nlaunch != 1 || pl.ksplit != 1 || q.nphase > 1) return;
+    ConvLaunch& l = pl.launch[0];
+    ConvArgs& a = l.a;
+    const bool halo = l.family == CONV_HALO, tile = l.family == CONV_K64 && l.bc <= 128;
+    if (!halo && !tile) return;
+    const int bc = halo ? 128 : l.bc, pixel_waves = (tile && l.bc == 64) ? 8 : 4;
+    if (!conv_is_plain(a) || a.accumulate || a.ydtype != q.xdtype || (a.Cout % bc) != 0) return;
+    if (!sbg_aligned16(a.y) || !sbg_aligned16(q.dact_y) || ((a.ys_n | a.ys_h | a.ys_w) & 7) != 0) return;
+    if (q.dact_act != SBG_ACT_LRELU || !(q.dact_gain > 0.f)) return;
+    a.dact_y = (const unsigned short*)q.dact_y; a.dact_partial = q.dact_partial;
+    a.dact_alpha = q.dact_alpha; a.dact_gain = q.dact_gain; a.dact_clamp = q.dact_clamp;
+    l.bytes += 2.0 * l.dims[0] * (double)a.Cout;
+    pl.dact_rows = (int64_t)a.ptiles * pixel_waves;
+}
+
 int conv_plan(const sbg_conv_params* q, bool have_ws, ConvPlan& pl)
 {
-    const int rc = conv_validate(q);
+    int rc = conv_validate(q);
     if (rc != SBG_OK) return rc;
-    pl.nlaunch = 0; pl.ksplit = 1; pl.reduce_epi = false; pl.workspace_bytes = 0;
-    return conv_plan_add(*q, have_ws, pl);
+    pl.nlaunch = 0; pl.ksplit = 1; pl.reduce_epi = false; pl.workspace_bytes = 0; pl.dact_rows = -1;
+    rc = conv_plan_add(*q, have_ws, pl);
+    if (rc == SBG_OK && q->dact_y) conv_plan_dact(*q, pl);
+    return rc;
 }
 
 }
@@ -326,6 +346,12 @@
 {
     ConvPlan pl;
     return conv_plan(q, true, pl) == SBG_OK ? pl.workspace_bytes : -1;
+}
+
+extern "C" int64_t sbg_conv2d_igemm_dact_rows(const sbg_conv_params* q)
+{
+    ConvPlan pl;
+    return (q && q->dact_y && conv_plan(q, true, pl) == SBG_OK) ? pl.dact_rows : -1;
 }
 
 extern "C" int sbg_conv2d_igemm_plan(const sbg_conv_params* q, sbg_conv_launch_info* out, int max)
@@ -347,6 +373,7 @@
     int rc = conv_plan(q, q && q->workspace, pl);
     if (rc != SBG_OK) return rc;
     SBG_CHECK(q->ksplit <= 1 || q->workspace != nullptr, "conv2d_igemm: ksplit > 1 needs a workspace");
+    SBG_CHECK(!q->dact_y || (pl.dact_rows > 0 && sbg_conv2d_igemm_dact_rows(q) == pl.dact_rows), "conv2d_igemm: this call cannot carry the backward tail (ask sbg_conv2d_igemm_dact_rows first)");
     hipStream_t s = (hipStream_t)stream;
     const bool bf16 = q->xdtype == SBG_BF16;
     for (int i = 0; i < pl.nlaunch && rc == SBG_OK; i++) {
diff --git a/style-big-gan_amd/csrc/conv_k64.hip b/style-big-gan_amd/csrc/conv_k64.hip
--- a/style-big-gan_amd/csrc/conv_k64.hip
+++ b/style-big-gan_amd/csrc/conv_k64.hip
@@ -6,7 +6,7 @@
 namespace {
 
 
-template <class MF, int BC, int BP, int WGC, int WGP, int NSTAGE = 3>
+template <class MF, int BC, int BP, int WGC, int WGP, int NSTAGE = 3, bool DACT = false>
 __global__ __launch_bounds__(512, 2) void conv_k64_kernel(ConvArgs p, unsigned x_bytes, unsigned w_bytes)
 {
     constexpr int NW = 8;
@@ -265,15 +265,17 @@
         }
     }
 
-    conv_epilogue8<TC, TP>(p, acc, c0 + wc, fg, [&](int j, int& n, int& oy, int& ox) {
+    auto pixel = [&](int j, int& n, int& oy, int& ox) {
         const int pix = p0 + wp + 16 * j + fr;
         const int pp = pix < p.P ? pix : 0;
         ox = pp % p.OW; const int t = pp / p.OW; oy = t % p.OH; n = t / p.OH;
         return pix < p.P;
-    });
-}
-
-template <class MF, int TH, int TW>
+    };
+    if constexpr (DACT) conv_epilogue_dact<TC, TP>(p, acc, c0 + wc, fg, pixel, (bid / p.ctiles) * WGP + wpi);
+    else                conv_epilogue8<TC, TP>(p, acc, c0 + wc, fg, pixel);
+}
+
+template <class MF, int TH, int TW, bool DACT = false>
 __global__ __launch_bounds__(768, 3) void conv_halo_ld_kernel(ConvArgs p, unsigned x_bytes, unsigned w_bytes)
 {
     constexpr int BC = 128, BP = 256, WGP = 4;
@@ -492,11 +494,15 @@
     int tpar = 0, done_par = 0;
     auto epilogue = [&](const TileC& tc) __attribute__((always_inline)) {
         const LdsParams lp{(lds_cfloat*)(sP + done_par * PARAM_BYTES), wc, TW};
-        conv_epilogue8<TC, TP, true>(p, acc, tc.c0 + wc, fg, [&](int j, int& n, int& oy, int& ox) {
+        auto pixel = [&](int j, int& n, int& oy, int& ox) {
             const int sg = wpi * TP + j, r = sg / SEG, cseg = (sg - r * SEG) * 16;
             n = tc.tn; oy = tc.y0 + r; ox = tc.x0 + cseg + fr;
             return true;
-        }, 0, p.lds_params ? &lp : nullptr, tc.y0, tc.x0);
+        };
+        if constexpr (DACT)
+            conv_epilogue_dact<TC, TP, true>(p, acc, tc.c0 + wc, fg, pixel, ((tc.tn * tiles_y + tc.y0 / TH) * tiles_x + tc.x0 / TW) * WGP + wpi);
+        else
+            conv_epilogue8<TC, TP, true>(p, acc, tc.c0 + wc, fg, pixel, 0, p.lds_params ? &lp : nullptr, tc.y0, tc.x0);
 #pragma unroll
         for (int i = 0; i < TC; i++)
 #pragma unroll
@@ -717,6 +723,15 @@
 template <class MF>
 static int launch_leaf(const ConvLaunch& l, hipStream_t stream)
 {
+    if (l.a.dact_y) {
+        if (l.family == CONV_HALO)
+            return l.bc == 8 ? conv_launch<conv_halo_ld_kernel<MF, 8, 32, true>>(l, stream, l.x_bytes, l.w_bytes)
+                             : conv_launch<conv_halo_ld_kernel<MF, 16, 16, true>>(l, stream, l.x_bytes, l.w_bytes);
+        if (l.family != CONV_K64 || l.bc > 128) return sbg_fail(SBG_ERR_INVALID, "conv2d_igemm: no kernel carries the backward tail for this launch");
+        if (l.bc == 64)  return conv_launch<conv_k64_kernel<MF, 64, 256, 1, 8, 3, true>>(l, stream, l.x_bytes, l.w_bytes);
+        if (l.bp == 128) return conv_launch<conv_k64_kernel<MF, 128, 128, 2, 4, 3, true>>(l, stream, l.x_bytes, l.w_bytes);
+        return conv_launch<conv_k64_kernel<MF, 128, 256, 2, 4, 3, true>>(l, stream, l.x_bytes, l.w_bytes);
+    }
     if (l.family == CONV_GATHER) return conv_launch<conv_gather_ld_kernel<MF>>(l, stream, l.x_bytes, l.w_bytes);
     if (l.family == CONV_HALO)
         return l.bc == 8 ? conv_launch<conv_halo_ld_kernel<MF, 8, 32>>(l, stream, l.x_bytes, l.w_bytes)
diff --git a/style-big-gan_amd/csrc/fromrgb.hip b/style-big-gan_amd/csrc/fromrgb.hip
--- a/style-big-gan_amd/csrc/fromrgb.hip
+++ b/style-big-gan_amd/csrc/fromrgb.hip
@@ -76,7 +76,7 @@
     }
 }
 
-template <class T, int CI, bool DIMG>
+template <class T, int CI, bool DIMG, bool PRE = false>
 __global__ void __launch_bounds__(256) fromrgb_bwd_kernel(FromArgs p)
 {
     constexpr int RS = MAX_CI * 8 + 8 + 1;
@@ -124,14 +124,14 @@
             float g[8], yv[8];
             if (ok) {
                 Vec8<T>::ld(dyb + pix * p.Co + cl * 8, g);
-                Vec8<T>::ld(ysb + pix * p.Co + cl * 8, yv);
+                if (!PRE) Vec8<T>::ld(ysb + pix * p.Co + cl * 8, yv);
             }
             const float4_t v = px[loc & 255];
             float di[MAX_CI] = {0.f, 0.f, 0.f, 0.f};
 #pragma unroll
             for (int j = 0; j < 8; j++) {
-                const bool live = ok && (fabsf(yv[j]) < rail);
-                const float d1 = live ? g[j] * (yv[j] > 0.0f ? gpos : gneg) : 0.0f;
+                const bool live = ok && (PRE || fabsf(yv[j]) < rail);
+                const float d1 = live ? (PRE ? g[j] : g[j] * (yv[j] > 0.0f ? gpos : gneg)) : 0.0f;
                 db[j] += d1;
 #pragma unroll
                 for (int c = 0; c < CI; c++) { dw[c][j] += d1 * v[c]; if (DIMG) di[c] += d1 * w[c][j]; }
@@ -222,7 +222,7 @@
 extern "C" int sbg_fromrgb_bwd(const float* img, const float* w, const void* dy, const void* y, float* dimg, float* partial, int dtype,
                                int N, int Ci, int Co, int64_t HW, int act, float alpha, float gain, float clamp, sbg_stream_t stream_)
 {
-    SBG_CHECK(img && w && dy && y && partial, "fromrgb_bwd: null pointer");
+    SBG_CHECK(img && w && dy && partial, "fromrgb_bwd: null pointer");
     if (int rc = check_shape(N, Ci, Co, HW)) return rc;
     SBG_CHECK(sbg_fromrgb_supported(Ci, Co, act), "fromrgb_bwd: unsupported activation %d", act);
     SBG_CHECK(dtype == SBG_BF16 || dtype == SBG_F16, "fromrgb_bwd: 16-bit activations only");
@@ -231,13 +231,17 @@
     a.N = N; a.Ci = Ci; a.Co = Co; a.HW = HW; a.act = act; a.alpha = alpha; a.gain = gain; a.clamp = clamp;
     a.blocks_per_n = blocks_for(N, HW);
     hipStream_t stream = (hipStream_t)stream_;
-    SbgProfScope prof(stream, SBG_K_FROMRGB, 4.0 * N * Co * (double)Ci * HW, (double)N * HW * (4.0 * Co + 8.0 * Ci), {N, Ci, Co, (int)HW, 1, Ci == 3 ? 3 : MAX_CI, dimg ? 1 : 0});
+    SbgProfScope prof(stream, SBG_K_FROMRGB, 4.0 * N * Co * (double)Ci * HW, (double)N * HW * ((y ? 4.0 : 2.0) * Co + 8.0 * Ci), {N, Ci, Co, (int)HW, 1, Ci == 3 ? 3 : MAX_CI, (dimg ? 1 : 0) + (y ? 0 : 2)});
     dim3 grid((unsigned)(N * a.blocks_per_n)), block(256);
     const int lds = 4 * (Co >> 3) * (MAX_CI * 8 + 8 + 1) * (int)sizeof(float);
+#define SBG_FROMRGB_BWD_(T_, CI_, PRE_) do { \
+        if (dimg) SBG_LAUNCH((fromrgb_bwd_kernel<T_, CI_, true, PRE_>), grid, block, lds, stream, a); \
+        else      SBG_LAUNCH((fromrgb_bwd_kernel<T_, CI_, false, PRE_>), grid, block, lds, stream, a); } while (0)
 #define SBG_FROMRGB_BWD(T_) do { \
-        if (Ci == 3) { if (dimg) SBG_LAUNCH((fromrgb_bwd_kernel<T_, 3, true>), grid, block, lds, stream, a); else SBG_LAUNCH((fromrgb_bwd_kernel<T_, 3, false>), grid, block, lds, stream, a); } \
-        else { if (dimg) SBG_LAUNCH((fromrgb_bwd_kernel<T_, MAX_CI, true>), grid, block, lds, stream, a); else SBG_LAUNCH((fromrgb_bwd_kernel<T_, MAX_CI, false>), grid, block, lds, stream, a); } } while (0)
+        if (Ci == 3) { if (y) SBG_FROMRGB_BWD_(T_, 3, false); else SBG_FROMRGB_BWD_(T_, 3, true); } \
+        else         { if (y) SBG_FROMRGB_BWD_(T_, MAX_CI, false); else SBG_FROMRGB_BWD_(T_, MAX_CI, true); } } while (0)
     if (dtype == SBG_BF16) SBG_FROMRGB_BWD(bf16_s); else SBG_FROMRGB_BWD(f16_s);
+#undef SBG_FROMRGB_BWD_
 #undef SBG_FROMRGB_BWD
     SBG_HIP_LAUNCH_CHECK();
     return 0;
diff --git a/style-big-gan_amd/torch_utils/misc.py b/style-big-gan_amd/torch_utils/misc.py
--- a/style-big-gan_amd/torch_utils/misc.py
+++ b/style-big-gan_amd/torch_utils/misc.py
@@ -112,4 +112,9 @@
         return tensors[0]
     if any(t.dtype != tensors[0].dtype or t.shape[1:] != tensors[0].shape[1:] for t in tensors) or tensors[0].device.type != 'cuda':
         return torch.cat(tensors)
-    return _Cat0.apply(*tensors)
+    out = _Cat0.apply(*tensors)
+    from .ops import conv_bias_act
+    handle = conv_bias_act.DactHandle.of_cat(tensors)
+    if handle is not None:
+        out._sbg_dact = handle
+    return out
diff --git a/style-big-gan_amd/torch_utils/ops/conv2d_gradfix.py b/style-big-gan_amd/torch_utils/ops/conv2d_gradfix.py
--- a/style-big-gan_amd/torch_utils/ops/conv2d_gradfix.py
+++ b/style-big-gan_amd/torch_utils/ops/conv2d_gradfix.py
@@ -191,7 +191,7 @@
     return p
 
 
-def _igemm(x, wp, y, taps, stride, oh, ow, y_off=(0, 0), y_step=(1, 1), oscale=None, accumulate=False, epi=None):
+def _igemm(x, wp, y, taps, stride, oh, ow, y_off=(0, 0), y_step=(1, 1), oscale=None, accumulate=False, epi=None, dact=None):
     lib = _lib.load()
     p = _conv_params(x, wp, y, y_step)
     p.y = y.data_ptr() + (y_off[0] * y.stride(2) + y_off[1] * y.stride(3)) * y.element_size()
@@ -209,6 +209,19 @@
             p.oscale = osc32.data_ptr()
         p.noise, p.bias = _lib.ptr(nz32), _lib.ptr(b32)
         p.act, p.alpha, p.gain, p.clamp = epi.act.code, epi.act.alpha, epi.act.gain, epi.act.clamp
+    if dact is not None:
+        ys, act, want_db = dact
+        assert epi is None and not accumulate and y_off == (0, 0) and y_step == (1, 1)
+        if ys.shape != y.shape or ys.dtype != y.dtype or ys.stride() != y.stride() or not act.fused:
+            return False
+        p.dact_y, p.dact_act, p.dact_alpha, p.dact_gain, p.dact_clamp = ys.data_ptr(), act.code, act.alpha, act.gain, act.clamp
+        rows = int(lib.sbg_conv2d_igemm_dact_rows(p))
+        if rows <= 0:
+            return False
+        part = torch.empty([rows, wp.shape[1]], dtype=torch.float32, device=x.device) if want_db else None
+        p.dact_partial = _lib.ptr(part)
+        _lib.check(lib.sbg_conv2d_igemm(p, _lib.stream_ptr(x.device)), "sbg_conv2d_igemm")
+        return part if want_db else True
     nbytes = lib.sbg_conv2d_igemm_workspace(p)
     if nbytes < 0:
         _lib.check(1, "sbg_conv2d_igemm_workspace")
@@ -324,6 +337,28 @@
     return y.to(x.dtype) if y.dtype != x.dtype else y
 
 
+def conv_transpose_dact(x, w, cfg, y_saved, act, want_db):
+    if (not cfg.transpose or cfg.stride != (1, 1) or cfg.output_padding != (0, 0) or x.device.type != "cuda"
+            or x.dtype not in (torch.bfloat16, torch.float16) or x.dtype != y_saved.dtype or x.numel() == 0):
+        return None
+    n, cin, ih, iw = x.shape
+    cin_w, cout, kh, kw = w.shape
+    mixed = is_mixed(x, w)
+    if cin != cin_w or cin % 8 != 0 or kh * kw > _lib.SBG_MAX_TAPS or not (mixed or x.dtype == w.dtype):
+        return None
+    ph, pw = cfg.padding
+    oh, ow = ih - 1 - 2 * ph + kh, iw - 1 - 2 * pw + kw
+    if (n, cout, oh, ow) != tuple(y_saved.shape):
+        return None
+    wa = _packed_weight(w, 1, x.dtype, cin, cfg.wgain)[0] if mixed else w.permute(2, 3, 1, 0).reshape(kh * kw, cout, cin)
+    taps = [(ph - i, pw - j, i * kw + j) for i in range(kh) for j in range(kw)]
+    y = torch.empty([n, cout, oh, ow], dtype=x.dtype, device=x.device, memory_format=torch.channels_last)
+    done = _igemm(_cl(x), wa.contiguous(), y, taps, 1, oh, ow, dact=(y_saved, act, want_db))
+    if done is False:
+        return None
+    return y, (done if want_db else None)
+
+
 def _wgrad(a, b, stride, taps):
     lib = _lib.load()
     assert a.dtype == b.dtype and a.shape[0] == b.shape[0]
diff --git a/style-big-gan_amd/torch_utils/ops/conv2d_resample.py b/style-big-gan_amd/torch_utils/ops/conv2d_resample.py
--- a/style-big-gan_amd/torch_utils/ops/conv2d_resample.py
+++ b/style-big-gan_amd/torch_utils/ops/conv2d_resample.py
@@ -8,11 +8,11 @@
 from .upfirdn2d import _get_filter_size, _parse_padding
 
 
-def _conv(x, w, stride=1, padding=0, groups=1, transpose=False, flip_weight=True, tail=None, wgain=1.0):
+def _conv(x, w, stride=1, padding=0, groups=1, transpose=False, flip_weight=True, tail=None, wgain=1.0, x_dact=None):
     if not flip_weight:
         w = w.flip([2, 3])
     if tail is not None and not transpose and conv_bias_act.fusable(x, w, tail.act.name, groups):
-        return conv_bias_act.conv2d_bias_act(x, w, tail.bias, stride, padding, *tail.act, wgain=wgain)
+        return conv_bias_act.conv2d_bias_act(x, w, tail.bias, stride, padding, *tail.act, wgain=wgain, x_dact=x_dact)
     fn = conv2d_gradfix.conv_transpose2d if transpose else conv2d_gradfix.conv2d
     y = fn(x, w, stride=stride, padding=padding, groups=groups, wgain=wgain)
     return _tail(y, tail)
@@ -34,7 +34,7 @@
 
 
 def conv2d_resample(x, w, f=None, up=1, down=1, padding=0, groups=1, flip_weight=True, flip_filter=False, bias_act_tail=None, fir_tail=None,
-                    wgain=1.0, prefiltered=False):
+                    wgain=1.0, prefiltered=False, x_dact=None):
     tail = bias_act_tail
     assert isinstance(x, torch.Tensor) and x.ndim == 4
     assert isinstance(w, torch.Tensor) and w.ndim == 4 and (w.dtype == x.dtype or conv2d_gradfix.is_mixed(x, w))
@@ -96,7 +96,7 @@
         return _tail(x, tail)
 
     if px0 == px1 and py0 == py1 and px0 >= 0 and py0 >= 0:
-        return _conv(x, w, padding=[py0, px0], groups=groups, flip_weight=flip_weight, tail=tail, wgain=wgain)
+        return _conv(x, w, padding=[py0, px0], groups=groups, flip_weight=flip_weight, tail=tail, wgain=wgain, x_dact=x_dact)
 
     x = upfirdn2d.upfirdn2d(x, (f if up > 1 else None), up=up, padding=pad4, gain=up ** 2, flip_filter=flip_filter)
     x = _conv(x, w, groups=groups, flip_weight=flip_weight, wgain=wgain)
diff --git a/style-big-gan_amd/torch_utils/ops/conv_bias_act.py b/style-big-gan_amd/torch_utils/ops/conv_bias_act.py
--- a/style-big-gan_amd/torch_utils/ops/conv_bias_act.py
+++ b/style-big-gan_amd/torch_utils/ops/conv_bias_act.py
@@ -1,11 +1,70 @@
+import os
+
 import torch
 
+from ... import _lib
 from . import bias_act as _ba
 from . import conv2d_gradfix as _cg
 from . import upfirdn2d as _up
 from ._tail import Act, Tail
 
 first_order = False
+
+fuse_d_dact = os.environ.get("SBG_FUSE_D_DACT", "1") != "0"
+
+
+class DactHandle:
+    __slots__ = ("act", "want_db", "result", "parts", "pending", "whole")
+
+    def __init__(self, act, want_db):
+        self.act, self.want_db, self.result, self.parts, self.pending, self.whole = act, bool(want_db), None, 0, 0, None
+
+    @classmethod
+    def of_cat(cls, tensors):
+        hs = [getattr(t, "_sbg_dact", None) for t in tensors]
+        if any(h is None or h.parts or h.act != hs[0].act for h in hs):
+            return None
+        whole, first = cls(hs[0].act, any(h.want_db for h in hs)), 0
+        whole.parts = len(hs)
+        for h, t in zip(hs, tensors):
+            h.whole, first = (whole, first), first + t.shape[0]
+        return whole
+
+    def hand_over(self, d1, w, adj, x):
+        if not (first_order and fuse_d_dact) or torch.is_grad_enabled() or self.act.name != "lrelu" or d1.dtype != x.dtype:
+            return None
+        sums = self.want_db and x.shape[1] > 1 and bool(_lib.load().sbg_modconv_bwd_supported(x.shape[1]))
+        if self.parts and (x.shape[2] * x.shape[3]) % 256 != 0:
+            sums = False
+        out = _cg.conv_transpose_dact(d1, w, adj, x, self.act, sums)
+        if out is None:
+            return None
+        dx, rows = out
+        self.result, self.pending = (dx.data_ptr(), tuple(dx.shape), rows), self.parts
+        return dx
+
+    def take(self, dy, y, who):
+        res, first, self.result = self.result, 0, None
+        if res is None and self.whole is not None and self.whole[0].result is not None:
+            whole, first = self.whole
+            res, whole.pending = whole.result, whole.pending - 1
+            if whole.pending <= 0:
+                whole.result = None
+        if res is None:
+            return None
+        ptr, shape, rows = res
+        n = dy.shape[0]
+        if (dy.data_ptr() != ptr + first * dy.stride(0) * dy.element_size() or tuple(dy.shape[1:]) != shape[1:] or first + n > shape[0]
+                or dy.shape != y.shape or dy.dtype != y.dtype or dy.stride() != y.stride()):
+            raise RuntimeError(f"{who}: the consumer handed over the activation gradient, but the incoming gradient is another tensor -- "
+                               "the output must have exactly that one consumer (DactHandle)")
+        db = None
+        if rows is not None and n == shape[0]:
+            db = rows.sum(0)
+        elif rows is not None:
+            per = rows.shape[0] // shape[0]
+            db = rows[first * per:(first + n) * per].sum(0)
+        return dy, db
 
 
 def _act_backward(act, dy, y, want_db):
@@ -19,7 +78,10 @@
 def _backward_from_dy(ctx, x, w, d1, db_fused, needs):
     dx = dw = db = None
     if needs[0]:
-        dx = _cg._Conv.apply(d1, w, ctx.ccfg.adjoint(x.shape[2:], d1.shape[2:], w.shape[2:]))
+        adj = ctx.ccfg.adjoint(x.shape[2:], d1.shape[2:], w.shape[2:])
+        dx = ctx.x_dact.hand_over(d1, w, adj, x) if ctx.x_dact is not None else None
+        if dx is None:
+            dx = _cg._Conv.apply(d1, w, adj)
     if needs[1] and not _cg.weight_gradients_disabled:
         dw = _cg._ConvWgrad.apply(d1, x, ctx.ccfg, tuple(w.shape), _cg.wmeta_of(x, w))
     if ctx.has_bias and needs[2]:
@@ -38,26 +100,33 @@
 class _ConvBiasAct(torch.autograd.Function):
 
     @staticmethod
-    def forward(ctx, x, w, b, ccfg, act):
+    def forward(ctx, x, w, b, ccfg, act, x_dact=None, dact=None):
         y = _forward(ctx, x, w, b, ccfg, act)
         ctx.save_for_backward(x, w, y)
+        ctx.x_dact, ctx.dact = x_dact, dact
+        if dact is not None:
+            dact.want_db = ctx.has_bias and ctx.needs_input_grad[2]
         return y
 
     @staticmethod
     def backward(ctx, dy):
         x, w, y = ctx.saved_tensors
-        d1, db_fused = _act_backward(ctx.act, dy.contiguous(memory_format=torch.channels_last), y, ctx.has_bias and ctx.needs_input_grad[2])
-        return (*_backward_from_dy(ctx, x, w, d1, db_fused, ctx.needs_input_grad), None, None)
+        handed = ctx.dact.take(dy, y, "conv_bias_act") if ctx.dact is not None else None
+        if handed is not None:
+            d1, db_fused = handed
+        else:
+            d1, db_fused = _act_backward(ctx.act, dy.contiguous(memory_format=torch.channels_last), y, ctx.has_bias and ctx.needs_input_grad[2])
+        return (*_backward_from_dy(ctx, x, w, d1, db_fused, ctx.needs_input_grad), None, None, None, None)
 
 
 class _ConvBiasActFir(torch.autograd.Function):
 
     @staticmethod
-    def forward(ctx, x, w, b, f, ccfg, act, fcfg):
+    def forward(ctx, x, w, b, f, ccfg, act, fcfg, x_dact=None):
         y = _forward(ctx, x, w, b, ccfg, act)
         out = _up._launch(y, f, *fcfg)
         ctx.save_for_backward(x, w, y, f)
-        ctx.fcfg = fcfg
+        ctx.fcfg, ctx.x_dact = fcfg, x_dact
         return out
 
     @staticmethod
@@ -72,7 +141,7 @@
             gcfg = ctx.fcfg.adjoint(y.shape[2:], dout.shape[2:], f)
             dy = _up._Upfirdn2d.apply(dout.to(y.dtype), f, gcfg).contiguous(memory_format=torch.channels_last)
             d1, db_fused = _act_backward(ctx.act, dy, y, True)
-        return (*_backward_from_dy(ctx, x, w, d1, db_fused, ctx.needs_input_grad), None, None, None, None)
+        return (*_backward_from_dy(ctx, x, w, d1, db_fused, ctx.needs_input_grad), None, None, None, None, None)
 
 
 def fir_fusable(x, w, act, f, groups=1):
@@ -80,9 +149,10 @@
             and f is not None and f.ndim == 2 and tuple(f.shape) == (4, 4) and x.shape[2] >= 16 and _up._taps_exact(f, x.dtype))
 
 
-def conv2d_bias_act_fir(x, w, b, f, fpad, stride=1, padding=0, act="linear", alpha=None, gain=None, clamp=None, wgain=1.0, flip_filter=False, fgain=1.0):
+def conv2d_bias_act_fir(x, w, b, f, fpad, stride=1, padding=0, act="linear", alpha=None, gain=None, clamp=None, wgain=1.0, flip_filter=False, fgain=1.0,
+                        x_dact=None):
     fcfg = _up.FirCfg(1, 1, 1, 1, *_up._parse_padding(fpad), bool(flip_filter), float(fgain))
-    return _ConvBiasActFir.apply(x, w, b, f, _cg.ConvCfg.make(False, stride, padding, wgain=wgain), Act.make(act, alpha, gain, clamp), fcfg)
+    return _ConvBiasActFir.apply(x, w, b, f, _cg.ConvCfg.make(False, stride, padding, wgain=wgain), Act.make(act, alpha, gain, clamp), fcfg, x_dact)
 
 
 def fusable(x, w, act, groups=1):
@@ -90,5 +160,14 @@
             and (x.dtype == w.dtype or _cg.is_mixed(x, w)))
 
 
-def conv2d_bias_act(x, w, b=None, stride=1, padding=0, act="linear", alpha=None, gain=None, clamp=None, wgain=1.0):
-    return _ConvBiasAct.apply(x, w, b, _cg.ConvCfg.make(False, stride, padding, wgain=wgain), Act.make(act, alpha, gain, clamp))
+def conv2d_bias_act(x, w, b=None, stride=1, padding=0, act="linear", alpha=None, gain=None, clamp=None, wgain=1.0, x_dact=None):
+    a = Act.make(act, alpha, gain, clamp)
+    handle = DactHandle(a, False) if first_order and fuse_d_dact and a.name == "lrelu" else None
+    y = _ConvBiasAct.apply(x, w, b, _cg.ConvCfg.make(False, stride, padding, wgain=wgain), a, x_dact, handle)
+    if handle is not None:
+        y._sbg_dact = handle
+    return y
+
+
+def sole_input_handle(x):
+    return getattr(x, "_sbg_dact", None) if first_order and fuse_d_dact else None
diff --git a/style-big-gan_amd/torch_utils/ops/fromrgb.py b/style-big-gan_amd/torch_utils/ops/fromrgb.py
--- a/style-big-gan_amd/torch_utils/ops/fromrgb.py
+++ b/style-big-gan_amd/torch_utils/ops/fromrgb.py
@@ -15,7 +15,7 @@
 class _FromRGB(torch.autograd.Function):
 
     @staticmethod
-    def forward(ctx, img, w, bias, act, out_dtype):
+    def forward(ctx, img, w, bias, act, out_dtype, dact=None):
         n, ci, h, wd = img.shape
         co = w.shape[0]
         ic = img.contiguous()
@@ -25,7 +25,7 @@
         _lib.check(_lib.load().sbg_fromrgb_fwd(ic.data_ptr(), wc.data_ptr(), _lib.ptr(bc), y.data_ptr(), _lib.dtype_code(out_dtype), n, ci, co, h * wd,
                                                act.code, act.alpha, act.gain, act.clamp, _lib.stream_ptr(img.device)), "sbg_fromrgb_fwd")
         ctx.save_for_backward(ic, wc, y)
-        ctx.act, ctx.has_bias = act, bias is not None
+        ctx.act, ctx.has_bias, ctx.dact = act, bias is not None, dact
         ctx.dtypes = (w.dtype, bias.dtype if bias is not None else None)
         return y
 
@@ -38,18 +38,25 @@
         lib = _lib.load()
         n, ci, h, wd = ic.shape
         co = wc.shape[0]
+        handed = ctx.dact.take(dy, y, "fromrgb") if ctx.dact is not None else None
         dyc = dy.to(y.dtype).contiguous(memory_format=torch.channels_last)
         dimg = torch.empty_like(ic) if ctx.needs_input_grad[0] else None
         nb = lib.sbg_fromrgb_bwd_blocks(n, h * wd)
         part = torch.empty([n * nb, co * ci + co], dtype=torch.float32, device=ic.device)
-        _lib.check(lib.sbg_fromrgb_bwd(ic.data_ptr(), wc.data_ptr(), dyc.data_ptr(), y.data_ptr(), _lib.ptr(dimg), part.data_ptr(), _lib.dtype_code(y.dtype),
+        _lib.check(lib.sbg_fromrgb_bwd(ic.data_ptr(), wc.data_ptr(), dyc.data_ptr(), None if handed is not None else y.data_ptr(), _lib.ptr(dimg), part.data_ptr(), _lib.dtype_code(y.dtype),
                                        n, ci, co, h * wd, act.code, act.alpha, act.gain, act.clamp, _lib.stream_ptr(ic.device)), "sbg_fromrgb_bwd")
         sums = part.sum(0)
         dw = sums[:co * ci].reshape(co, ci).to(ctx.dtypes[0]) if ctx.needs_input_grad[1] else None
         db = sums[co * ci:].to(ctx.dtypes[1]) if (ctx.has_bias and ctx.needs_input_grad[2]) else None
-        return dimg, dw, db, None, None
+        return dimg, dw, db, None, None, None
 
 
 def fromrgb(img, weight, bias, weight_gain, act, gain=None, clamp=None, out_dtype=torch.bfloat16):
+    from . import conv_bias_act as _cba
     w2d = weight.reshape(weight.shape[0], weight.shape[1]) * weight_gain
-    return _FromRGB.apply(img, w2d, bias, Act.make(act, gain=gain, clamp=clamp), out_dtype)
+    a = Act.make(act, gain=gain, clamp=clamp)
+    handle = _cba.DactHandle(a, False) if _cba.first_order and _cba.fuse_d_dact and a.name == "lrelu" else None
+    y = _FromRGB.apply(img, w2d, bias, a, out_dtype, handle)
+    if handle is not None:
+        y._sbg_dact = handle
+    return y
diff --git a/style-big-gan_amd/train_parts/discriminators.py b/style-big-gan_amd/train_parts/discriminators.py
--- a/style-big-gan_amd/train_parts/discriminators.py
+++ b/style-big-gan_amd/train_parts/discriminators.py
@@ -87,11 +87,12 @@
         shortcut = self.skip(x, gain=np.sqrt(0.5)) if residual else None
         c0, c1 = self.conv0, self.conv1
         g1 = np.sqrt(0.5) if residual else 1
+        x_dact = conv_bias_act.sole_input_handle(x) if self.architecture == 'orig' else None
         if (conv_bias_act.first_order and x.device.type == 'cuda' and conv2d_gradfix.is_mixed(x, c0.weight) and c0.up == 1 and c0.down == 1 and c1.up == 1
                 and c1.down == 2 and c1.weight.shape[2] > 1 and conv_bias_act.fir_fusable(x, c0.weight, c0.activation, c1.resample_filter)):
-            x = c1(c0(x, then_lowpass_of=c1), gain=g1, prefiltered=True)
+            x = c1(c0(x, then_lowpass_of=c1, x_dact=x_dact), gain=g1, prefiltered=True)
         else:
-            x = c1(c0(x), gain=g1)
+            x = c1(c0(x, x_dact=x_dact), gain=g1)
         if residual:
             x = shortcut + x
         if self.attention is not None:
diff --git a/style-big-gan_amd/train_parts/generators.py b/style-big-gan_amd/train_parts/generators.py
--- a/style-big-gan_amd/train_parts/generators.py
+++ b/style-big-gan_amd/train_parts/generators.py
@@ -185,18 +185,20 @@
             else:
                 self.bias = None
 
-    def forward(self, x, gain=1, prefiltered=False, then_lowpass_of=None):
+    def forward(self, x, gain=1, prefiltered=False, then_lowpass_of=None, x_dact=None):
         b = self.bias
         clamp = self.conv_clamp * gain if self.conv_clamp is not None else None
         if then_lowpass_of is not None:
             nxt = then_lowpass_of
             assert self.up == 1 and self.down == 1 and nxt.up == 1 and nxt.down > 1
             return conv_bias_act.conv2d_bias_act_fir(x, self.weight, b, nxt.resample_filter, conv2d_resample.lowpass_padding(nxt.resample_filter, nxt.down, nxt.padding),
-                                                     padding=self.padding, act=self.activation, gain=self.act_gain * gain, clamp=clamp, wgain=self.weight_gain)
+                                                     padding=self.padding, act=self.activation, gain=self.act_gain * gain, clamp=clamp, wgain=self.weight_gain,
+                                                     x_dact=x_dact)
         tail = Tail.make(self.activation, gain=self.act_gain * gain, clamp=clamp, bias=b)
         if conv2d_gradfix.is_mixed(x, self.weight) and x.device.type == 'cuda':
             return conv2d_resample.conv2d_resample(x=x, w=self.weight, f=self.resample_filter, up=self.up, down=self.down, padding=self.padding,
-                                                   flip_weight=(self.up == 1), bias_act_tail=tail, wgain=self.weight_gain, prefiltered=prefiltered)
+                                                   flip_weight=(self.up == 1), bias_act_tail=tail, wgain=self.weight_gain, prefiltered=prefiltered,
+                                                   x_dact=x_dact)
         w = self.weight * self.weight_gain
         return conv2d_resample.conv2d_resample(x=x, w=w.to(x.dtype), f=self.resample_filter, up=self.up, down=self.down,
                                                padding=self.padding, flip_weight=(self.up == 1), bias_act_tail=tail, prefiltered=prefiltered)
```

Result: slower. 625.1 img/s (-1.2%).
